# nv-nguyen/gigapose

Measured on AMD Instinct MI355X. Metric: query-crops/sec (ViT feat + template NN + 4DoF regress), 162 templates, 1/2/4/8 GPU, higher is better.
Workload: dtype f32 (ViT linear layers + attention, matcher, IST convolutions: f32 operands split into f16 hi/lo, 3 x f16 MFMA per k-block, f32 accumulate -- error vs f64 below the f32 fmaf chain's, tests/test_gpu_split.py; everything else f32); 1 GPU; BASELINE configs[1]: dinov2_vitl14 random-init, 1 object(s) x 162 templates, batch=64 crops per GPU, k=5, full path ViT->match->IST->RANSAC->pose; numerics=split, global_batch=64, parallelism=single, streams=single stream, rccl_ranks=0

## Files before the change

gigapose_amd/ae_net.py:

```python
import torch
from torch import nn

from .vit import Dinov2ViT, VARIANTS

descriptor_sizes = {"dinov2_vits14": 384, "dinov2_vitb14": 768, "dinov2_vitl14": 1024}


def as_hip_backbone(model, model_name=None):
    if isinstance(model, Dinov2ViT):
        return model
    if model is None:
        return Dinov2ViT.from_name(model_name)
    if hasattr(model, "config") and hasattr(model, "embeddings"):
        return Dinov2ViT.from_hf(model)
    sd = model.state_dict()
    if "blocks.0.attn.qkv.weight" in sd:
        dim = sd["cls_token"].shape[-1]
        depth = 1 + max(int(k.split(".")[1]) for k in sd if k.startswith("blocks."))
        vit = Dinov2ViT(dim, depth, dim // 64)
        vit.load_state_dict(sd, strict=False)
        return vit.eval()
    raise TypeError(f"cannot convert {type(model).__name__} into the HIP DINOv2 backbone")


class AENet(nn.Module):
    def __init__(self, model_name, dinov2_model, descriptor_size, max_batch_size, patch_size=14, **kwargs):
        super().__init__()
        if patch_size != 14:
            raise NotImplementedError("kernels are specialised for patch_size 14 @ 224x224")
        self.model_name = model_name
        self.dinov2_model = as_hip_backbone(dinov2_model, model_name)
        self.descriptor_size = descriptor_size
        self.max_batch_size = max_batch_size
        self.patch_size = patch_size
        assert self.dinov2_model.dim == descriptor_size

    def compute_features(self, images):
        return self.dinov2_model.forward_features(images)

    @torch.no_grad()
    def forward_by_chunk(self, processed_rgbs, patch_dim=(2, 3)):
        outs = [self.dinov2_model.patch_features(processed_rgbs[s:s + self.max_batch_size], normalize=True)
                for s in range(0, processed_rgbs.shape[0], self.max_batch_size)]
        if not outs:
            return torch.empty(0, self.descriptor_size, 16, 16, device=processed_rgbs.device)
        return outs[0] if len(outs) == 1 else torch.cat(outs, dim=0)

    def forward(self, images):
        return self.forward_by_chunk(images)
```

gigapose_amd/csrc/gp_gemm.hip:

```cpp
#include "gp_common.h"

namespace {

enum {
    EPI_NONE = 0,
    EPI_BIAS_I = 1,
    EPI_BIAS_I_GELU = 2,
    EPI_BIAS_I_SCALE_RES = 3,
    EPI_BIAS_J = 4,
    EPI_BIAS_I_RELU = 5,
};

using GM = KMajor<2, 4, 2, 1, 16>;

__device__ __forceinline__ float gelu_erf(float x)
{
    return 0.5f * x * (1.0f + erff(x * 0.70710678118654752440f));
}

constexpr int kMaxSlots = 1024;
constexpr size_t kSkHeaderBytes = 8192;
constexpr size_t kSkPartialFloats = (size_t)GM::BM * GM::BN;
constexpr int kSpinLimit = 400000;

struct GemmArgs {
    const float* A; int lda;
    const float* B; int ldb;
    float* D; int ldd;
    int K;
    const float* bias; const float* scale;
    const float* res ; int ldr;
    int tiles_i, tiles_j;
    int group;
    int* flags;
    float* partial;
    int epoch;
    int* status;
};

__device__ __forceinline__ void tile_origin(const GemmArgs& a, int q, int& i0, int& j0)
{
    const int per_band = a.group * a.tiles_j;
    const int band = q / per_band, r = q - band * per_band;
    const int first_i = band * a.group;
    const int gsz = min(a.group, a.tiles_i - first_i);
    i0 = (first_i + r % gsz) * GM::BM;
    j0 = (r / gsz) * GM::BN;
}

template <int EPI>
__device__ __forceinline__ void gemm_epilogue(const GemmArgs& a, int i0, int j0, const f32x16 (&acc)[2][1])
{
    int tid_ = threadIdx.x;
    asm volatile("" : "+v"(tid_));
    const int lane = tid_ & 63, wave = tid_ >> 6;
    const int wm = wave / GM::WN_, wn = wave % GM::WN_;
    const float* __restrict__ bias = a.bias;
    const float* __restrict__ scale = a.scale;
    const float* res = a.res;
    float* D = a.D;
    const int j = j0 + wn * 32 + (lane & 31);
#pragma unroll
    for (int mi = 0; mi < 2; ++mi) {
#pragma unroll
        for (int r = 0; r < 16; ++r) {
            const int i = i0 + wm * 64 + mi * 32 + frag_row(r, lane);
            float v = acc[mi][0][r];
            if (EPI == EPI_BIAS_I || EPI == EPI_BIAS_I_GELU || EPI == EPI_BIAS_I_SCALE_RES || EPI == EPI_BIAS_I_RELU)
                v = v + bias[i];
            if (EPI == EPI_BIAS_J) v = v + bias[j];
            if (EPI == EPI_BIAS_I_GELU) v = gelu_erf(v);
            if (EPI == EPI_BIAS_I_RELU) v = fmaxf(v, 0.f);
            if (EPI == EPI_BIAS_I_SCALE_RES) v = res[(unsigned)i * (unsigned)a.ldr + (unsigned)j] + scale[i] * v;
            D[(unsigned)i * (unsigned)a.ldd + (unsigned)j] = v;
        }
        if (EPI == EPI_BIAS_I_SCALE_RES) __builtin_amdgcn_sched_barrier(0);
    }
}

template <int EPI>
__global__ __launch_bounds__(GM::NT, 8) void gemm_kmajor_kernel(const GemmArgs a)
{
    __shared__ float smem[GM::LDS_FLOATS];
    const int q = xcd_chunked_tile(blockIdx.x, a.tiles_i * a.tiles_j);
    if (q < 0) return;
    int i0, j0;
    tile_origin(a, q, i0, j0);
    f32x16 acc[2][1];
    GM::run(a.A + i0, a.lda, a.B + j0, a.ldb, a.K, smem, acc);
    gemm_epilogue<EPI>(a, i0, j0, acc);
}

template <int EPI>
__global__ __launch_bounds__(GM::NT, 8) void gemm_streamk_kernel(const GemmArgs a)
{
    __shared__ float smem[GM::LDS_FLOATS];
    const int tid = threadIdx.x;
    const int p = blockIdx.x, x = p & 7, n = p >> 3, slots_x = gridDim.x >> 3;
    const int T = a.tiles_i * a.tiles_j;
    const int per = (T + 7) >> 3;
    const int t_lo = x * per;
    const int n_t = min(T - t_lo, per);
    const int nslab = a.K / GM::KS_;
    const long long U = (long long)n_t * nslab;
    const long long u0 = U * n / slots_x, u1 = U * (n + 1) / slots_x;
    const int ta = (int)(u0 / nslab), sa = (int)(u0 % nslab);
    const int tb = (int)(u1 / nslab), sb = (int)(u1 % nslab);
    const int n_head = sb > 0 ? 1 : 0, n_rest = sa > 0 ? 1 : 0;
    const int first_whole = ta + n_rest;
    const int n_seg = n_head + (tb - first_whole) + n_rest;
    for (int seg = 0; seg < n_seg; ++seg) {
        const bool is_head = seg < n_head;
        const bool is_rest = n_rest && seg == n_seg - 1;
        const int t = is_head ? tb : (is_rest ? ta : first_whole + seg - n_head);
        const int k0 = is_rest ? sa * GM::KS_ : 0;
        const int k1 = is_head ? sb * GM::KS_ : a.K;
        int i0, j0;
        tile_origin(a, t_lo + t, i0, j0);
        f32x16 acc[2][1];
        if (is_rest) {
            if (tid == 0) {
                int spins = 0;
                while (__hip_atomic_load(a.flags + (p - 8), __ATOMIC_RELAXED, __HIP_MEMORY_SCOPE_AGENT) != a.epoch) {
                    __builtin_amdgcn_s_sleep(16);
                    if (++spins > kSpinLimit) {
                        __hip_atomic_store(a.flags + kMaxSlots, 1, __ATOMIC_RELAXED, __HIP_MEMORY_SCOPE_AGENT);
                        gp_raise(a.status, GP_ST_HANDOFF_CHAIN);
                        break;
                    }
                }
                __builtin_amdgcn_fence(__ATOMIC_ACQUIRE, "agent");
            }
            __syncthreads();
            const f32x4* w = reinterpret_cast<const f32x4*>(a.partial + (size_t)(p - 8) * kSkPartialFloats) + tid * 8;
#pragma unroll
            for (int mi = 0; mi < 2; ++mi)
#pragma unroll
                for (int r4 = 0; r4 < 4; ++r4) {
                    const f32x4 v = w[mi * 4 + r4];
                    acc[mi][0][r4 * 4 + 0] = v[0]; acc[mi][0][r4 * 4 + 1] = v[1];
                    acc[mi][0][r4 * 4 + 2] = v[2]; acc[mi][0][r4 * 4 + 3] = v[3];
                }
        } else {
#pragma unroll
            for (int mi = 0; mi < 2; ++mi)
#pragma unroll
                for (int r = 0; r < 16; ++r) acc[mi][0][r] = 0.f;
        }
        GM::run_acc(a.A + (size_t)k0 * a.lda + i0, a.lda, a.B + (size_t)k0 * a.ldb + j0, a.ldb, k1 - k0, smem, acc);
        if (is_head) {
            f32x4* w = reinterpret_cast<f32x4*>(a.partial + (size_t)p * kSkPartialFloats) + tid * 8;
#pragma unroll
            for (int mi = 0; mi < 2; ++mi)
#pragma unroll
                for (int r4 = 0; r4 < 4; ++r4) {
                    f32x4 v;
                    v[0] = acc[mi][0][r4 * 4 + 0]; v[1] = acc[mi][0][r4 * 4 + 1];
                    v[2] = acc[mi][0][r4 * 4 + 2]; v[3] = acc[mi][0][r4 * 4 + 3];
                    w[mi * 4 + r4] = v;
                }
            asm volatile("s_waitcnt vmcnt(0)" ::: "memory");
            __syncthreads();
            if (tid == 0) {
                __builtin_amdgcn_fence(__ATOMIC_RELEASE, "agent");
                asm volatile("s_waitcnt vmcnt(0)" ::: "memory");
                __hip_atomic_store(a.flags + p, a.epoch, __ATOMIC_RELAXED, __HIP_MEMORY_SCOPE_AGENT);
            }
        } else {
            gemm_epilogue<EPI>(a, i0, j0, acc);
        }
    }
}

static int g_streamk = 1;
static int g_group = 8;
static unsigned g_epoch = 0;

template <int EPI>
int launch(const float* A, int lda, const float* B, int ldb, float* D, int ldd, int I, int J, int K,
           const float* bias, const float* scale, const float* res, int ldr, float* sk_ws, hipStream_t st)
{
    GemmArgs a{A, lda, B, ldb, D, ldd, K, bias, scale, res, ldr, I / GM::BM, J / GM::BN, g_group, nullptr, nullptr, 0, gp_status_buffer()};
    const int T = a.tiles_i * a.tiles_j;
    if (g_streamk && sk_ws && T > kMaxSlots && (T < 4 * kMaxSlots || g_streamk == 2) && T % kMaxSlots != 0) {
        const int per = (T + 7) / 8, last = T - 7 * per;
        const int slots_x = last < kMaxSlots / 8 ? last : kMaxSlots / 8;
        if (slots_x > 0) {
            a.flags = reinterpret_cast<int*>(sk_ws);
            a.partial = reinterpret_cast<float*>(reinterpret_cast<char*>(sk_ws) + kSkHeaderBytes);
            if (++g_epoch == 0) ++g_epoch;
            a.epoch = (int)g_epoch;
            hipLaunchKernelGGL((gemm_streamk_kernel<EPI>), dim3(8 * slots_x), dim3(GM::NT), 0, st, a);
            return 0;
        }
    }
    hipLaunchKernelGGL((gemm_kmajor_kernel<EPI>), dim3(xcd_chunked_grid(T)), dim3(GM::NT), 0, st, a);
    return 0;
}

}

int gp_gemm_launch(const float* A, int lda, const float* B, int ldb, float* D, int ldd, int I, int J,
                   int K, int epilogue, const float* bias, const float* scale, const float* res, int ldr,
                   float* sk_ws, hipStream_t st)
{
    GP_REQUIRE(I > 0 && J > 0 && K > 0, "gp_gemm_kmajor: empty problem (I=%d J=%d K=%d)", I, J, K);
    GP_REQUIRE(I % 128 == 0 && J % 128 == 0 && K % 16 == 0,
               "gp_gemm_kmajor: I=%d, J=%d must be multiples of 128 and K=%d of 16 (pad the operands)", I, J, K);
    GP_REQUIRE(lda % 4 == 0 && ldb % 4 == 0 && lda >= I && ldb >= J && ldd >= J,
               "gp_gemm_kmajor: bad leading dimensions lda=%d ldb=%d ldd=%d", lda, ldb, ldd);
    GP_REQUIRE((long long)I * ldd < (1ll << 31) && (long long)I * (ldr > 0 ? ldr : 1) < (1ll << 31),
               "gp_gemm_kmajor: output larger than 2^31 elements");
    GP_REQUIRE(A && B && D, "gp_gemm_kmajor: null pointer");
    GP_REQUIRE(((uintptr_t)A % 16 == 0) && ((uintptr_t)B % 16 == 0), "gp_gemm_kmajor: operands must be 16-byte aligned");
    GP_REQUIRE(((uintptr_t)sk_ws % 16 == 0), "gp_gemm_kmajor: stream-K scratch must be 16-byte aligned");
    GpProfScope prof(GP_PROF_GEMM, 2.0 * I * J * K, st);
    switch (epilogue) {
        case EPI_NONE: launch<EPI_NONE>(A, lda, B, ldb, D, ldd, I, J, K, bias, scale, res, ldr, sk_ws, st); break;
        case EPI_BIAS_I:
            GP_REQUIRE(bias, "gp_gemm_kmajor: bias required");
            launch<EPI_BIAS_I>(A, lda, B, ldb, D, ldd, I, J, K, bias, scale, res, ldr, sk_ws, st);
            break;
        case EPI_BIAS_I_GELU:
            GP_REQUIRE(bias, "gp_gemm_kmajor: bias required");
            launch<EPI_BIAS_I_GELU>(A, lda, B, ldb, D, ldd, I, J, K, bias, scale, res, ldr, sk_ws, st);
            break;
        case EPI_BIAS_I_SCALE_RES:
            GP_REQUIRE(bias && scale && res && ldr >= J, "gp_gemm_kmajor: bias/scale/residual required");
            launch<EPI_BIAS_I_SCALE_RES>(A, lda, B, ldb, D, ldd, I, J, K, bias, scale, res, ldr, sk_ws, st);
            break;
        case EPI_BIAS_J:
            GP_REQUIRE(bias, "gp_gemm_kmajor: bias required");
            launch<EPI_BIAS_J>(A, lda, B, ldb, D, ldd, I, J, K, bias, scale, res, ldr, sk_ws, st);
            break;
        case EPI_BIAS_I_RELU:
            GP_REQUIRE(bias, "gp_gemm_kmajor: bias required");
            launch<EPI_BIAS_I_RELU>(A, lda, B, ldb, D, ldd, I, J, K, bias, scale, res, ldr, sk_ws, st);
            break;
        default: GP_REQUIRE(false, "gp_gemm_kmajor: unknown epilogue %d", epilogue);
    }
    GP_CHECK_LAUNCH("gp_gemm_kmajor");
    return GP_OK;
}

size_t gp_gemm_streamk_bytes() { return kSkHeaderBytes + sizeof(float) * kSkPartialFloats * kMaxSlots; }

int gp_gemm_streamk_reset_launch(float* sk_ws, hipStream_t st)
{
    return hipMemsetAsync(sk_ws, 0, kSkHeaderBytes, st) == hipSuccess ? GP_OK : GP_ELAUNCH;
}

extern "C" int gp_gemm_kmajor(const float* A, int lda, const float* B, int ldb, float* D, int ldd, int I,
                              int J, int K, int epilogue, const float* bias, const float* scale,
                              const float* residual, int ldr, void* stream)
{
    return gp_gemm_launch(A, lda, B, ldb, D, ldd, I, J, K, epilogue, bias, scale, residual, ldr, nullptr,
                          (hipStream_t)stream);
}

extern "C" size_t gp_gemm_streamk_workspace_bytes(void) { return gp_gemm_streamk_bytes(); }

extern "C" int gp_gemm_streamk_reset(float* scratch, void* stream)
{
    GP_REQUIRE(scratch, "gp_gemm_streamk_reset: null scratch");
    return gp_gemm_streamk_reset_launch(scratch, (hipStream_t)stream);
}

#ifdef GP_PROBES
extern "C" void gp_gemm_set_streamk(int mode) { g_streamk = mode; }
extern "C" void gp_gemm_set_group(int g) { g_group = g > 0 ? g : 1; }

extern "C" int gp_gemm_streamk_error(const float* scratch, void* stream)
{
    int e = -1;
    if (hipMemcpyAsync(&e, reinterpret_cast<const int*>(scratch) + 1024, sizeof(int), hipMemcpyDeviceToHost,
                       (hipStream_t)stream) != hipSuccess ||
        hipStreamSynchronize((hipStream_t)stream) != hipSuccess)
        return -1;
    return e;
}
#endif

extern "C" int gp_gemm_kmajor_sk(const float* A, int lda, const float* B, int ldb, float* D, int ldd, int I,
                                 int J, int K, int epilogue, const float* bias, const float* scale,
                                 const float* residual, int ldr, float* scratch, size_t scratch_bytes, void* stream)
{
    GP_REQUIRE(scratch && scratch_bytes >= gp_gemm_streamk_bytes(), "gp_gemm_kmajor_sk: scratch too small");
    return gp_gemm_launch(A, lda, B, ldb, D, ldd, I, J, K, epilogue, bias, scale, residual, ldr, scratch,
                          (hipStream_t)stream);
}
```

gigapose_amd/csrc/gp_match.hip:

```cpp
#include "gp_common.h"

namespace {

__global__ __launch_bounds__(256) void l2norm_cp_kernel(const float* __restrict__ x,
                                                         float* __restrict__ out, int C)
{
    const size_t base = (size_t)blockIdx.x * C * GP_P + threadIdx.x;
    float ss = 0.f;
    for (int c = 0; c < C; ++c) {
        const float v = x[base + (size_t)c * GP_P];
        ss = __builtin_fmaf(v, v, ss);
    }
    const float d = fmaxf(__builtin_sqrtf(ss), 1e-12f);
    const int c0 = blockIdx.y * 32;
    for (int c = c0; c < c0 + 32 && c < C; ++c) out[base + (size_t)c * GP_P] = x[base + (size_t)c * GP_P] / d;
}

using MM = KMajor<4, 2, 2, 4, 16>;
static_assert(MM::BM == 256 && MM::BN == 256 && MM::NT == 512, "matcher tile must be 256x256");

struct alignas(16) MatchSmem {
    float stage[MM::LDS_FLOATS];
    float qmask[GP_P];
    float smask[GP_P];
    float rowv[2][GP_P];
    int rowi[2][GP_P];
    float colv[4][GP_P];
    int coli[4][GP_P];
    float sc_t2s[GP_P];
    int id_t2s[GP_P];
    float sc_s2t[GP_P];
    int id_s2t[GP_P];
    float contrib[GP_P];
    float maskv[GP_P];
};

template <int CNT>
__device__ __forceinline__ void rowmax_exchange(float (&rv)[32], int (&ri)[32], int lane)
{
    const bool hi = (lane & CNT) != 0;
#pragma unroll
    for (int j = 0; j < CNT; ++j) {
        const float sv = hi ? rv[j] : rv[j + CNT];
        const int si = hi ? ri[j] : ri[j + CNT];
        const float mv = hi ? rv[j + CNT] : rv[j];
        const int mj = hi ? ri[j + CNT] : ri[j];
        const float ov = __shfl_xor(sv, CNT);
        const int oi = __shfl_xor(si, CNT);
        const bool take = (ov > mv) | ((ov == mv) & (oi < mj));
        rv[j] = take ? ov : mv;
        ri[j] = take ? oi : mj;
    }
}

constexpr int kDeadPatch = 0x7fff;
#include "gp_match_rects.h"
struct MatchWaveTile {
    int r0, mi_n, c0, ni_n, rslot, cslot, active;
};
__device__ __forceinline__ MatchWaveTile match_wave_tile_grid(int wave)
{
    return MatchWaveTile{2 * (wave >> 1), 2, 4 * (wave & 1), 4, wave & 1, wave >> 1, 1};
}
__device__ __forceinline__ MatchWaveTile match_wave_tile_unpack(unsigned w)
{
    return MatchWaveTile{(int)(w & 15u), (int)((w >> 4) & 3u), (int)((w >> 6) & 15u), (int)((w >> 10) & 7u), (int)((w >> 13) & 3u), (int)((w >> 15) & 3u),
                         (int)((w >> 17) & 1u)};
}
template <bool PERM = false, class SM>
__device__ __forceinline__ void match_epilogue(SM& sm, f32x16 (&acc)[2][4], int b, int n, int N, float thr, float patch_thr,
                                               uint8_t* __restrict__ idx_t2s, float* __restrict__ score_t2s,
                                               float* __restrict__ mask_all, float* __restrict__ sim_avg,
                                               unsigned long long* trace = nullptr,
                                               int src2tar = 0,
                                               int compact = 1,
                                               MatchWaveTile wt = MatchWaveTile{0, 0, 0, 0, 0, 0, 0})
{
    const int tid = threadIdx.x, lane = tid & 63, wave = __builtin_amdgcn_readfirstlane(tid >> 6);
    if constexpr (!PERM) wt = match_wave_tile_grid(wave);
    const int s_lane = 32 * wt.c0 + (lane & 31);
    const int t_lane = 32 * wt.r0 + 4 * (lane >> 5);
    float sm_s[4];
    int s_idx[4];
#pragma unroll
    for (int ni = 0; ni < 4; ++ni) {
        sm_s[ni] = 0.f;
        s_idx[ni] = kDeadPatch;
        if (!PERM || ni < wt.ni_n) {
            if constexpr (PERM) {
                sm_s[ni] = sm.smask_p[s_lane + 32 * ni];
                s_idx[ni] = sm.s_of[s_lane + 32 * ni];
            } else {
                sm_s[ni] = sm.smask[s_lane + 32 * ni];
                s_idx[ni] = s_lane + 32 * ni;
            }
        }
    }
#pragma unroll
    for (int mi = 0; mi < 2; ++mi) {
        if (PERM && mi >= wt.mi_n) continue;
#pragma unroll
        for (int r = 0; r < 16; ++r) {
            float tm;
            if constexpr (PERM) tm = sm.qmask_p[t_lane + 32 * mi + (r & 3) + 8 * (r >> 2)];
            else tm = sm.qmask[t_lane + 32 * mi + (r & 3) + 8 * (r >> 2)];
#pragma unroll
            for (int ni = 0; ni < 4; ++ni) {
                float v = acc[mi][ni][r] * sm_s[ni];
                v = v * tm;
                acc[mi][ni][r] = (v < thr) ? 0.f : v;
            }
        }
    }

    float rv[32];
    int ri[32];
#pragma unroll
    for (int mi = 0; mi < 2; ++mi)
#pragma unroll
        for (int r = 0; r < 16; ++r) {
            float bv = acc[mi][0][r];
            int bi = s_idx[0];
#pragma unroll
            for (int ni = 1; ni < 4; ++ni) {
                const float x = acc[mi][ni][r];
                const bool take = PERM ? ((x > bv) | ((x == bv) & (s_idx[ni] < bi))) : (x > bv);
                bv = take ? x : bv;
                bi = take ? s_idx[ni] : bi;
            }
            rv[mi * 16 + r] = bv;
            ri[mi * 16 + r] = bi;
        }
    rowmax_exchange<16>(rv, ri, lane);
    rowmax_exchange<8>(rv, ri, lane);
    rowmax_exchange<4>(rv, ri, lane);
    rowmax_exchange<2>(rv, ri, lane);
    rowmax_exchange<1>(rv, ri, lane);
    {
        const int j = lane & 31;
        int t = t_lane + 32 * (j >> 4) + (j & 3) + 8 * ((j & 15) >> 2);
        const bool mine = !PERM || (wt.active && (j >> 4) < wt.mi_n);
        if constexpr (PERM) t = mine ? sm.t_of[t] : kDeadPatch;
        if (mine && (!PERM || t != kDeadPatch)) {
            sm.rowv[wt.rslot][t] = rv[0];
            sm.rowi[wt.rslot][t] = ri[0];
        }
    }

    int tp[32];
    if constexpr (PERM) {
#pragma unroll
        for (int mi = 0; mi < 2; ++mi)
#pragma unroll
            for (int r4 = 0; r4 < 4; ++r4) {
                typedef short s16x4 __attribute__((ext_vector_type(4)));
                const s16x4 q4 = *reinterpret_cast<const s16x4*>(&sm.t_of[t_lane + 32 * mi + 8 * r4]);
#pragma unroll
                for (int e = 0; e < 4; ++e) tp[mi * 16 + 4 * r4 + e] = (int)q4[e];
            }
    }
#pragma unroll
    for (int ni = 0; ni < 4; ++ni) {
        if (PERM && (ni >= wt.ni_n || !wt.active)) continue;
        float bv = acc[0][ni][0];
        int bi = PERM ? tp[0] : t_lane;
#pragma unroll
        for (int mi = 0; mi < 2; ++mi) {
            if (PERM && mi >= wt.mi_n) continue;
#pragma unroll
            for (int r = 0; r < 16; ++r) {
                const float x = acc[mi][ni][r];
                if constexpr (PERM) {
                    const int tq = tp[mi * 16 + r];
                    const bool take = (x > bv) | ((x == bv) & ((x > 0.f) | (compact == 0)) & (tq < bi));
                    bv = take ? x : bv;
                    bi = take ? tq : bi;
                } else {
                    const int row = t_lane + 32 * mi + (r & 3) + 8 * (r >> 2);
                    if (x > bv) { bv = x; bi = row; }
                }
            }
        }
        const float ov = __shfl_xor(bv, 32);
        const int oi = __shfl_xor(bi, 32);
        if (ov > bv || (ov == bv && oi < bi)) { bv = ov; bi = oi; }
        if (lane < 32 && (!PERM || s_idx[ni] != kDeadPatch)) {
            sm.colv[wt.cslot][s_idx[ni]] = bv;
            sm.coli[wt.cslot][s_idx[ni]] = bi;
        }
    }
    __syncthreads();
    if (trace && tid == 0) trace[3] = wall_clock64();

    if (tid < GP_P) {
        float bv = sm.rowv[0][tid];
        int bi = sm.rowi[0][tid];
#pragma unroll
        for (int w = 1; w < ((PERM && compact) ? 4 : 2); ++w) {
            const float v1 = sm.rowv[w][tid];
            const int i1 = sm.rowi[w][tid];
            if (v1 > bv || (PERM && v1 == bv && i1 < bi)) { bv = v1; bi = i1; }
        }
        if (PERM && compact && bv == 0.f) bi = 0;
        sm.sc_t2s[tid] = bv;
        sm.id_t2s[tid] = bi;
    } else {
        const int s = tid - GP_P;
        float bv = sm.colv[0][s];
        int bi = sm.coli[0][s];
#pragma unroll
        for (int w = 1; w < 4; ++w) {
            const float vw = sm.colv[w][s];
            const int iw = sm.coli[w][s];
            if (vw > bv || (PERM && vw == bv && iw < bi)) { bv = vw; bi = iw; }
        }
        if (PERM && compact && bv == 0.f) bi = 0;
        sm.sc_s2t[s] = bv;
        sm.id_s2t[s] = bi;
    }
    __syncthreads();
    if (trace && tid == 0) trace[4] = wall_clock64();

    if (tid < GP_P) {
        const int t = tid;
        const float* sc_a = src2tar ? sm.sc_s2t : sm.sc_t2s;
        const int* id_a = src2tar ? sm.id_s2t : sm.id_t2s;
        const float* sc_b = src2tar ? sm.sc_t2s : sm.sc_s2t;
        const int* id_b = src2tar ? sm.id_t2s : sm.id_s2t;
        const int js = id_a[t];
        const float sc = sc_a[t];
        const bool mask_sim = sc >= thr;
        bool mask_cycle = true;
        if (patch_thr > 0.f) {
            const int t2 = id_b[js];
            const float dx = (float)(t2 % GP_G) - (float)(t % GP_G);
            const float dy = (float)(t2 / GP_G) - (float)(t / GP_G);
            const float dist = __builtin_sqrtf(dx * dx + dy * dy);
            const bool mask_dist = dist <= patch_thr;
            const bool mask_sim2 = sc_b[js] >= thr;
            mask_cycle = mask_dist && mask_sim2;
        }
        float nz = sm.qmask[t] * sm.smask[js];
        nz = nz * (float)(id_b[t] != 0);
        nz = nz * (float)(js != 0);
        const float m = (float)(mask_sim && mask_cycle) * nz;
        const size_t o = ((size_t)b * N + n) * GP_P + t;
        idx_t2s[o] = (uint8_t)js;
        score_t2s[o] = sc;
        mask_all[o] = m;
        sm.contrib[t] = sc * m;
        sm.maskv[t] = m;
    }
    __syncthreads();
    if (trace && tid == 0) trace[5] = wall_clock64();
    if (tid == 0) {
        float a = 0.f, cnt = 0.f;
#pragma unroll 1
        for (int t0 = 0; t0 < GP_P; t0 += 32) {
            f32x4 c[8], m[8];
#pragma unroll
            for (int u = 0; u < 8; ++u) {
                c[u] = *reinterpret_cast<const f32x4*>(&sm.contrib[t0 + 4 * u]);
                m[u] = *reinterpret_cast<const f32x4*>(&sm.maskv[t0 + 4 * u]);
            }
#pragma unroll
            for (int u = 0; u < 8; ++u)
#pragma unroll
                for (int e = 0; e < 4; ++e) {
                    a = a + c[u][e];
                    cnt = cnt + m[u][e];
                }
        }
        sim_avg[(size_t)b * N + n] = (cnt > 0.f) ? a / 256.0f : 0.f;
        if (trace) trace[6] = wall_clock64();
    }
}

__global__ __launch_bounds__(512, 2) void match_tiles_kernel(
    const float* __restrict__ query,
    const float* __restrict__ bank,
    const float* __restrict__ qmask,
    const float* __restrict__ bmask,
    const int* __restrict__ labels,
    int B, int O, int N, int C, float thr, float patch_thr, int* __restrict__ status,
    uint8_t* __restrict__ idx_t2s,
    float* __restrict__ score_t2s,
    float* __restrict__ mask_all,
    float* __restrict__ sim_avg,
    int src2tar)
{
    __shared__ MatchSmem sm;
    const int q = xcd_chunked_tile(blockIdx.x, B * N);
    if (q < 0) return;
    const int band = q / (8 * N), r8 = q - band * (8 * N);
    const int gsz = min(8, B - band * 8);
    const int b = band * 8 + r8 % gsz, n = r8 / gsz;
    const int tid = threadIdx.x;
    int lab = labels[b];
    if ((unsigned)lab >= (unsigned)O) {
        if (tid == 0) gp_raise(status, GP_ST_LABEL_RANGE);
        lab = 0;
    }
    const size_t on = (size_t)lab * N + n;
    const float* A = query + (size_t)b * C * GP_P;
    const float* Bm = bank + on * (size_t)C * GP_P;

    if (tid < GP_P) sm.qmask[tid] = qmask[(size_t)b * GP_P + tid];
    else sm.smask[tid - GP_P] = bmask[on * GP_P + (tid - GP_P)];

    f32x16 acc[2][4];
    MM::run(A, GP_P, Bm, GP_P, C, sm.stage, acc);

    match_epilogue(sm, acc, b, n, N, thr, patch_thr, idx_t2s, score_t2s, mask_all, sim_avg, nullptr, src2tar);
}

typedef _Float16 h16x8 __attribute__((ext_vector_type(8)));
constexpr float kFeatScale = 32.0f;
constexpr int MS_BK = 32, MS_PLANE = 256 * MS_BK;

struct alignas(16) MatchSplitSmem {
    _Float16 stage[2 * 4 * MS_PLANE];
    float qmask[GP_P];
    float smask[GP_P];
    float qmask_p[GP_P];
    float smask_p[GP_P];
    short t_of[GP_P];
    short s_of[GP_P];
    int cnt[8];
    float rowv[4][GP_P];
    int rowi[4][GP_P];
    float colv[4][GP_P];
    int coli[4][GP_P];
    float sc_t2s[GP_P];
    int id_t2s[GP_P];
    float sc_s2t[GP_P];
    int id_s2t[GP_P];
    float contrib[GP_P];
    float maskv[GP_P];
};

typedef unsigned int mu32x4 __attribute__((ext_vector_type(4)));
constexpr unsigned kMatchOob = 0x80000000u;

struct MatchSplitRsrc {
    __amdgpu_buffer_rsrc_t qh, ql, bh, bl;
    unsigned va0, va1, vb0, vb1;
};

template <bool BANK_LO, int MI, int NI>
__device__ __forceinline__ void match_split_kloop(MatchSplitSmem& sm, f32x16 (&acc)[2][4], const MatchSplitRsrc& rs, int ns, int tid,
                                                  int lane, int r0, int c0, int grp)
{
    constexpr int P_AHI = 0, P_ALO = MS_PLANE, P_BHI = 2 * MS_PLANE, P_BLO = 3 * MS_PLANE, MS_BUF = 4 * MS_PLANE;
    const int wofs = (tid >> 2) * MS_BK + (((tid & 3) ^ (((tid >> 2) >> 2) & 3)) << 3);
    mu32x4 rg[8];
    auto gload = [&](int slab) {
        const unsigned so = (unsigned)slab * (MS_BK * 2u);
        rg[0] = __builtin_amdgcn_raw_buffer_load_b128(rs.qh, rs.va0, so, 0);
        rg[2] = __builtin_amdgcn_raw_buffer_load_b128(rs.ql, rs.va0, so, 0);
        rg[1] = __builtin_amdgcn_raw_buffer_load_b128(rs.qh, rs.va1, so, 0);
        rg[3] = __builtin_amdgcn_raw_buffer_load_b128(rs.ql, rs.va1, so, 0);
        rg[4] = __builtin_amdgcn_raw_buffer_load_b128(rs.bh, rs.vb0, so, 0);
        rg[5] = __builtin_amdgcn_raw_buffer_load_b128(rs.bh, rs.vb1, so, 0);
        if (BANK_LO) {
            rg[6] = __builtin_amdgcn_raw_buffer_load_b128(rs.bl, rs.vb0, so, 0);
            rg[7] = __builtin_amdgcn_raw_buffer_load_b128(rs.bl, rs.vb1, so, 0);
        }
    };
    auto stage = [&](int buf) {
        _Float16* L = sm.stage + buf * MS_BUF + wofs;
        *reinterpret_cast<mu32x4*>(L + P_AHI) = rg[0];
        *reinterpret_cast<mu32x4*>(L + P_ALO) = rg[2];
        *reinterpret_cast<mu32x4*>(L + P_AHI + 128 * MS_BK) = rg[1];
        *reinterpret_cast<mu32x4*>(L + P_ALO + 128 * MS_BK) = rg[3];
        *reinterpret_cast<mu32x4*>(L + P_BHI) = rg[4];
        *reinterpret_cast<mu32x4*>(L + P_BHI + 128 * MS_BK) = rg[5];
        if (BANK_LO) {
            *reinterpret_cast<mu32x4*>(L + P_BLO) = rg[6];
            *reinterpret_cast<mu32x4*>(L + P_BLO + 128 * MS_BK) = rg[7];
        }
    };
    const int ar_ = 32 * r0 + (lane & 31), br_ = 32 * c0 + (lane & 31), kh_ = lane >> 5;
    const int arow = ar_ * MS_BK, brow = br_ * MS_BK;
    const int ak0 = ((kh_ ^ ((ar_ >> 2) & 3)) << 3), ak1 = (((kh_ + 2) ^ ((ar_ >> 2) & 3)) << 3);
    const int bk0 = ((kh_ ^ ((br_ >> 2) & 3)) << 3), bk1 = (((kh_ + 2) ^ ((br_ >> 2) & 3)) << 3);
    gload(0);
    stage(0);
    __builtin_amdgcn_sched_barrier(0);
    if (ns > 1) gload(1);
    __syncthreads();

#define M_MFMA(A_, B_, mi, ni) acc[mi][ni] = __builtin_amdgcn_mfma_f32_32x32x16_f16(A_[mi], B_[ni], acc[mi][ni], 0, 0, 0)
#define M_ALL(A_, B_)                                       \
    _Pragma("unroll") for (int ni = 0; ni < NI; ++ni)       \
        _Pragma("unroll") for (int mi = 0; mi < MI; ++mi) M_MFMA(A_, B_, mi, ni)
    auto c_phase = [&](int s) __attribute__((always_inline)) {
        const _Float16* L = sm.stage + (s & 1) * MS_BUF;
        __builtin_amdgcn_s_setprio(1);
        h16x8 ah[MI], al[MI], bh[NI], bl[NI], ch[MI], cl[MI], dh[NI], dl[NI];
#pragma unroll
        for (int mi = 0; mi < MI; ++mi) ah[mi] = *reinterpret_cast<const h16x8*>(L + P_AHI + arow + mi * 32 * MS_BK + ak0);
#pragma unroll
        for (int ni = 0; ni < NI; ++ni) bh[ni] = *reinterpret_cast<const h16x8*>(L + P_BHI + brow + ni * 32 * MS_BK + bk0);
        if (BANK_LO) {
#pragma unroll
            for (int ni = 0; ni < NI; ++ni) bl[ni] = *reinterpret_cast<const h16x8*>(L + P_BLO + brow + ni * 32 * MS_BK + bk0);
        }
#pragma unroll
        for (int mi = 0; mi < MI; ++mi) al[mi] = *reinterpret_cast<const h16x8*>(L + P_ALO + arow + mi * 32 * MS_BK + ak0);
        M_ALL(ah, bh);
        if (BANK_LO) { M_ALL(ah, bl); }
#pragma unroll
        for (int mi = 0; mi < MI; ++mi) ch[mi] = *reinterpret_cast<const h16x8*>(L + P_AHI + arow + mi * 32 * MS_BK + ak1);
#pragma unroll
        for (int ni = 0; ni < NI; ++ni) dh[ni] = *reinterpret_cast<const h16x8*>(L + P_BHI + brow + ni * 32 * MS_BK + bk1);
        M_ALL(al, bh);
        if (BANK_LO) {
#pragma unroll
            for (int ni = 0; ni < NI; ++ni) dl[ni] = *reinterpret_cast<const h16x8*>(L + P_BLO + brow + ni * 32 * MS_BK + bk1);
        }
#pragma unroll
        for (int mi = 0; mi < MI; ++mi) cl[mi] = *reinterpret_cast<const h16x8*>(L + P_ALO + arow + mi * 32 * MS_BK + ak1);
        M_ALL(ch, dh);
        if (BANK_LO) { M_ALL(ch, dl); }
        M_ALL(cl, dh);
        __builtin_amdgcn_s_setprio(0);
    };
    auto m_phase = [&](int slab) __attribute__((always_inline)) {
        if (slab < ns) stage(slab & 1);
        __builtin_amdgcn_sched_barrier(0);
        gload(min(slab + 1, ns - 1));
    };
    if (grp) m_phase(1);
    for (int s = 0; s < ns; ++s) {
        c_phase(s);
        if (grp && s + 1 < ns) __syncthreads();
        m_phase(s + 1 + grp);
        if (!grp && s + 1 < ns) __syncthreads();
    }
#undef M_ALL
#undef M_MFMA
}

#ifndef GP_MATCH_BAND
#define GP_MATCH_BAND 8
#endif
constexpr int kSplitBand = GP_MATCH_BAND;
template <bool BANK_LO, bool TRACE = false>
__global__ __launch_bounds__(512, 2) void match_tiles_split_kernel(
    const _Float16* __restrict__ q_hi, const _Float16* __restrict__ q_lo,
    const _Float16* __restrict__ b_hi, const _Float16* __restrict__ b_lo,
    const float* __restrict__ qmask, const float* __restrict__ bmask, const int* __restrict__ labels, int B, int O, int N, int C,
    float thr, float patch_thr, int* __restrict__ status, uint8_t* __restrict__ idx_t2s, float* __restrict__ score_t2s,
    float* __restrict__ mask_all, float* __restrict__ sim_avg, unsigned long long* __restrict__ trace_all, int compact, int src2tar)
{
    __shared__ MatchSplitSmem sm;
    const unsigned long long w_in = TRACE ? wall_clock64() : 0;
    const int q = xcd_chunked_tile(blockIdx.x, B * N);
    if (q < 0) return;
    unsigned long long* trace = TRACE ? trace_all + (size_t)q * 8 : nullptr;
    if (TRACE && threadIdx.x == 0) {
        unsigned hw;
        asm volatile("s_getreg_b32 %0, hwreg(HW_REG_HW_ID)" : "=s"(hw));
        unsigned xcc;
        asm volatile("s_getreg_b32 %0, hwreg(HW_REG_XCC_ID)" : "=s"(xcc));
        trace[0] = w_in;
        trace[7] = ((unsigned long long)(xcc & 0xf) << 32) | hw;
    }
    const int band = q / (kSplitBand * N), r8 = q - band * (kSplitBand * N);
    const int gsz = min(kSplitBand, B - band * kSplitBand);
    const int b = band * kSplitBand + r8 % gsz, n = r8 / gsz;
    const int tid = threadIdx.x, lane = tid & 63;
    const int wave = __builtin_amdgcn_readfirstlane(tid >> 6);
    const int grp = wave >> 2;
    int lab = labels[b];
    if ((unsigned)lab >= (unsigned)O) {
        if (tid == 0) gp_raise(status, GP_ST_LABEL_RANGE);
        lab = 0;
    }
    const size_t on = (size_t)lab * N + n;

    const int pidx = tid & 255;
    const float mv = tid < GP_P ? qmask[(size_t)b * GP_P + pidx] : bmask[on * GP_P + pidx];
    const bool live = compact ? (mv != 0.f) : true;
    const unsigned long long bal = __ballot(live);
    const int before = __popcll(bal & ((1ull << lane) - 1ull));
    if (lane == 0) sm.cnt[wave] = __popcll(bal);
    if (tid < GP_P) {
        sm.qmask[pidx] = mv;
        sm.qmask_p[pidx] = 0.f;
        sm.t_of[pidx] = (short)kDeadPatch;
#pragma unroll
        for (int w = 0; w < 4; ++w) { sm.rowv[w][pidx] = 0.f; sm.rowi[w][pidx] = 0; }
    } else {
        sm.smask[pidx] = mv;
        sm.smask_p[pidx] = 0.f;
        sm.s_of[pidx] = (short)kDeadPatch;
#pragma unroll
        for (int w = 0; w < 4; ++w) { sm.colv[w][pidx] = 0.f; sm.coli[w][pidx] = 0; }
    }
    __syncthreads();
    int rank = before;
    for (int w = 4 * grp; w < wave; ++w) rank += sm.cnt[w];
    if (live) {
        if (tid < GP_P) {
            sm.t_of[rank] = (short)pidx;
            sm.qmask_p[rank] = mv;
        } else {
            sm.s_of[rank] = (short)pidx;
            sm.smask_p[rank] = mv;
        }
    }
    __syncthreads();
    const int live_t = sm.cnt[0] + sm.cnt[1] + sm.cnt[2] + sm.cnt[3], live_s = sm.cnt[4] + sm.cnt[5] + sm.cnt[6] + sm.cnt[7];
    const int nrb = __builtin_amdgcn_readfirstlane((live_t + 31) >> 5), ncb = __builtin_amdgcn_readfirstlane((live_s + 31) >> 5);
    const MatchWaveTile wt = match_wave_tile_unpack((unsigned)__builtin_amdgcn_readfirstlane((int)kMatchRect[nrb][ncb][wave]));

    const unsigned plane_bytes = (unsigned)GP_P * (unsigned)C * 2u;
    MatchSplitRsrc rs;
    rs.qh = __builtin_amdgcn_make_buffer_rsrc((void*)(q_hi + (size_t)b * GP_P * C), 0, plane_bytes, 0x00020000);
    rs.ql = __builtin_amdgcn_make_buffer_rsrc((void*)(q_lo + (size_t)b * GP_P * C), 0, plane_bytes, 0x00020000);
    rs.bh = __builtin_amdgcn_make_buffer_rsrc((void*)(b_hi + on * GP_P * C), 0, plane_bytes, 0x00020000);
    rs.bl = __builtin_amdgcn_make_buffer_rsrc((void*)((BANK_LO ? b_lo : b_hi) + on * GP_P * C), 0, plane_bytes, 0x00020000);
    {
        const int r0 = tid >> 2, r1 = r0 + 128;
        const unsigned ck = (unsigned)(tid & 3) * 16u, rowb = (unsigned)C * 2u;
        const int t0 = sm.t_of[r0], t1 = sm.t_of[r1], s0 = sm.s_of[r0], s1 = sm.s_of[r1];
        rs.va0 = t0 != kDeadPatch ? (unsigned)t0 * rowb + ck : kMatchOob;
        rs.va1 = t1 != kDeadPatch ? (unsigned)t1 * rowb + ck : kMatchOob;
        rs.vb0 = s0 != kDeadPatch ? (unsigned)s0 * rowb + ck : kMatchOob;
        rs.vb1 = s1 != kDeadPatch ? (unsigned)s1 * rowb + ck : kMatchOob;
    }

    f32x16 acc[2][4];
#pragma unroll
    for (int mi = 0; mi < 2; ++mi)
#pragma unroll
        for (int ni = 0; ni < 4; ++ni)
#pragma unroll
            for (int r = 0; r < 16; ++r) acc[mi][ni][r] = 0.f;
    const int ns = C / MS_BK;
    if (TRACE && tid == 0) trace[1] = wall_clock64();
    if (nrb > 0 && ncb > 0) {
        const int sel = wt.mi_n * 8 + wt.ni_n;
#define M_CASE(MI_, NI_) case MI_ * 8 + NI_: match_split_kloop<BANK_LO, MI_, NI_>(sm, acc, rs, ns, tid, lane, wt.r0, wt.c0, grp); break
        switch (sel) {
            M_CASE(1, 1); M_CASE(1, 2); M_CASE(1, 3); M_CASE(1, 4);
            M_CASE(2, 1); M_CASE(2, 2); M_CASE(2, 3);
            default: match_split_kloop<BANK_LO, 2, 4>(sm, acc, rs, ns, tid, lane, wt.r0, wt.c0, grp); break;
        }
#undef M_CASE
    }
    __syncthreads();
    if (TRACE && tid == 0) trace[2] = wall_clock64();

    constexpr float inv = 1.0f / (kFeatScale * kFeatScale);
#pragma unroll
    for (int mi = 0; mi < 2; ++mi)
#pragma unroll
        for (int ni = 0; ni < 4; ++ni)
#pragma unroll
            for (int r = 0; r < 16; ++r) acc[mi][ni][r] *= inv;
    match_epilogue<true>(sm, acc, b, n, N, thr, patch_thr, idx_t2s, score_t2s, mask_all, sim_avg, trace, src2tar, compact, wt);
}

__global__ __launch_bounds__(256) void l2norm_split_kernel(const float* __restrict__ x, _Float16* __restrict__ hi,
                                                            _Float16* __restrict__ lo, int C, int Cp,
                                                            const float* __restrict__ mask_img = nullptr, int mh = 0, int mw = 0,
                                                            float* __restrict__ patch_mask = nullptr)
{
    __shared__ float t[32][GP_P + 1];
    __shared__ float dn[GP_P];
    const int row = blockIdx.x, p = threadIdx.x;
    if (patch_mask && blockIdx.y == 0)
        patch_mask[(size_t)row * GP_P + p] = mask_img[(size_t)row * mh * mw + (size_t)((p >> 4) * (mh / GP_G)) * mw + (p & 15) * (mw / GP_G)];
    const float* xr = x + (size_t)row * C * GP_P;
    float ss = 0.f;
    int c = 0;
    for (; c + 16 <= C; c += 16) {
        float v[16];
#pragma unroll
        for (int u = 0; u < 16; ++u) v[u] = xr[(size_t)(c + u) * GP_P + p];
#pragma unroll
        for (int u = 0; u < 16; ++u) ss = __builtin_fmaf(v[u], v[u], ss);
    }
    for (; c < C; ++c) {
        const float v = xr[(size_t)c * GP_P + p];
        ss = __builtin_fmaf(v, v, ss);
    }
    dn[p] = fmaxf(__builtin_sqrtf(ss), 1e-12f);
    const int ngrp = Cp / 32, g0 = ngrp * blockIdx.y / gridDim.y, g1 = ngrp * (blockIdx.y + 1) / gridDim.y;
    for (int grp = g0; grp < g1; ++grp) {
        const int c0 = grp * 32;
        __syncthreads();
        for (int r = 0; r < 32; ++r) t[r][p] = (c0 + r < C) ? xr[(size_t)(c0 + r) * GP_P + p] : 0.f;
        __syncthreads();
#pragma unroll
        for (int u = 0; u < 4; ++u) {
            const int item = p + 256 * u, pp = item >> 2, g = item & 3;
            h16x8 h, l;
#pragma unroll
            for (int e = 0; e < 8; ++e) {
                const float v = (t[g * 8 + e][pp] / dn[pp]) * kFeatScale;
                const _Float16 hh = (_Float16)v;
                h[e] = hh;
                l[e] = (_Float16)(v - (float)hh);
            }
            const size_t o = ((size_t)row * GP_P + pp) * Cp + c0 + g * 8;
            *reinterpret_cast<h16x8*>(hi + o) = h;
            *reinterpret_cast<h16x8*>(lo + o) = l;
        }
    }
}

__global__ __launch_bounds__(64) void topk_kernel(const float* __restrict__ sim_avg, int N, int k,
                                                   int* __restrict__ ids, float* __restrict__ scores)
{
    extern __shared__ unsigned char taken[];
    const int b = blockIdx.x, lane = threadIdx.x;
    for (int n = lane; n < N; n += 64) taken[n] = 0;
    __syncthreads();
    const float* v = sim_avg + (size_t)b * N;
    for (int j = 0; j < k; ++j) {
        float bv = 0.f;
        int bi = 0x7fffffff;
        for (int n = lane; n < N; n += 64) {
            if (taken[n]) continue;
            const float x = v[n];
            if (bi == 0x7fffffff || x > bv) { bv = x; bi = n; }
        }
#pragma unroll
        for (int off = 32; off >= 1; off >>= 1) {
            const float ov = __shfl_xor(bv, off);
            const int oi = __shfl_xor(bi, off);
            if (oi != 0x7fffffff && (bi == 0x7fffffff || ov > bv || (ov == bv && oi < bi))) { bv = ov; bi = oi; }
        }
        if (lane == 0) {
            ids[(size_t)b * k + j] = bi;
            scores[(size_t)b * k + j] = bv;
            taken[bi] = 1;
        }
        __syncthreads();
    }
}

__global__ __launch_bounds__(256) void gather_records_kernel(
    const int* __restrict__ ids, const uint8_t* __restrict__ idx_t2s,
    const float* __restrict__ score_t2s, const float* __restrict__ mask_all, int N, int k,
    uint8_t* __restrict__ rec_idx, float* __restrict__ rec_score, float* __restrict__ rec_mask)
{
    const int bk = blockIdx.x, b = bk / k, t = threadIdx.x;
    const size_t src = ((size_t)b * N + ids[bk]) * GP_P + t;
    const size_t dst = (size_t)bk * GP_P + t;
    rec_idx[dst] = idx_t2s[src];
    rec_score[dst] = score_t2s[src];
    rec_mask[dst] = mask_all[src];
}

__global__ __launch_bounds__(256) void format_points_kernel(const uint8_t* __restrict__ rec_idx,
                                                             const float* __restrict__ rec_mask,
                                                             long long* __restrict__ tar_pts,
                                                             long long* __restrict__ src_pts)
{
    const size_t i = (size_t)blockIdx.x * GP_P + threadIdx.x;
    const int t = threadIdx.x;
    const bool valid = rec_mask[i] != 0.f;
    const int js = rec_idx[i];
    tar_pts[2 * i + 0] = valid ? (t % GP_G) : -1;
    tar_pts[2 * i + 1] = valid ? (t / GP_G) : -1;
    src_pts[2 * i + 0] = valid ? (js % GP_G) : -1;
    src_pts[2 * i + 1] = valid ? (js / GP_G) : -1;
}

__global__ __launch_bounds__(256) void select_topk_kernel(const float* __restrict__ sim_avg, const uint8_t* __restrict__ idx_t2s,
                                                           const float* __restrict__ score_t2s, const float* __restrict__ mask_all, int N, int k,
                                                           long long* __restrict__ ids64, float* __restrict__ scores,
                                                           float* __restrict__ rec_score, long long* __restrict__ tar_pts,
                                                           long long* __restrict__ src_pts)
{
    extern __shared__ unsigned char taken[];
    int* win = reinterpret_cast<int*>(taken + ((N + 3) & ~3));
    const int b = blockIdx.x, t = threadIdx.x, lane = t & 63;
    for (int n = t; n < N; n += 256) taken[n] = 0;
    __syncthreads();
    const float* v = sim_avg + (size_t)b * N;
    if (t < 64) {
        for (int j = 0; j < k; ++j) {
            float bv = 0.f;
            int bi = 0x7fffffff;
            for (int n = lane; n < N; n += 64) {
                if (taken[n]) continue;
                const float x = v[n];
                if (bi == 0x7fffffff || x > bv) { bv = x; bi = n; }
            }
#pragma unroll
            for (int off = 32; off >= 1; off >>= 1) {
                const float ov = __shfl_xor(bv, off);
                const int oi = __shfl_xor(bi, off);
                if (oi != 0x7fffffff && (bi == 0x7fffffff || ov > bv || (ov == bv && oi < bi))) { bv = ov; bi = oi; }
            }
            if (lane == 0) {
                ids64[(size_t)b * k + j] = bi;
                scores[(size_t)b * k + j] = bv;
                taken[bi] = 1;
                win[j] = bi;
            }
            __builtin_amdgcn_wave_barrier();
            __builtin_amdgcn_fence(__ATOMIC_ACQ_REL, "workgroup");
        }
    }
    __syncthreads();
    for (int j = 0; j < k; ++j) {
        const size_t src = ((size_t)b * N + win[j]) * GP_P + t;
        const size_t i = ((size_t)b * k + j) * GP_P + t;
        const bool valid = mask_all[src] != 0.f;
        const int js = idx_t2s[src];
        rec_score[i] = score_t2s[src];
        tar_pts[2 * i + 0] = valid ? (t % GP_G) : -1;
        tar_pts[2 * i + 1] = valid ? (t / GP_G) : -1;
        src_pts[2 * i + 0] = valid ? (js % GP_G) : -1;
        src_pts[2 * i + 1] = valid ? (js / GP_G) : -1;
    }
}

}

extern "C" {

int gp_l2norm_cp(const float* x, float* out, int rows, int C, void* stream)
{
    GP_REQUIRE(rows >= 0 && C > 0, "gp_l2norm_cp: bad arguments (rows=%d C=%d)", rows, C);
    if (rows == 0) return GP_OK;
    GP_REQUIRE(x && out, "gp_l2norm_cp: null pointer");
    hipLaunchKernelGGL(l2norm_cp_kernel, dim3(rows, (C + 31) / 32), dim3(256), 0, (hipStream_t)stream, x, out, C);
    GP_CHECK_LAUNCH("gp_l2norm_cp");
    return GP_OK;
}

int gp_match_tiles_dir(const float* query, const float* bank, const float* qmask, const float* bmask,
                       const int* labels, int B, int O, int N, int C, float sim_threshold,
                       float patch_threshold, int search_direction, uint8_t* idx_t2s, float* score_t2s, float* mask_all,
                       float* sim_avg, void* stream)
{
    GP_REQUIRE(search_direction == 0 || search_direction == 1, "gp_match_tiles: search_direction must be 0 (tar2src) or 1 (src2tar)");
    GP_REQUIRE(B >= 0 && O > 0 && N > 0, "gp_match_tiles: bad sizes B=%d O=%d N=%d", B, O, N);
    GP_REQUIRE(C > 0 && C % 16 == 0, "gp_match_tiles: C=%d must be a positive multiple of 16", C);
    if (B == 0) return GP_OK;
    GP_REQUIRE(query && bank && qmask && bmask && labels && idx_t2s && score_t2s && mask_all && sim_avg,
               "gp_match_tiles: null pointer");
    GpProfScope prof(GP_PROF_MATCH, 2.0 * B * N * 256.0 * 256.0 * C, (hipStream_t)stream);
    hipLaunchKernelGGL(match_tiles_kernel, dim3(xcd_chunked_grid(B * N)), dim3(512), 0,
                       (hipStream_t)stream, query, bank, qmask, bmask, labels, B, O, N, C, sim_threshold,
                       patch_threshold, gp_status_buffer(), idx_t2s, score_t2s, mask_all, sim_avg, search_direction);
    GP_CHECK_LAUNCH("gp_match_tiles");
    return GP_OK;
}

int gp_l2norm_split_mask(const float* x, void* hi, void* lo, int rows, int C, const float* mask_img, int mask_h, int mask_w,
                         float* patch_mask, void* stream)
{
    GP_REQUIRE(rows >= 0 && C > 0, "gp_l2norm_split: bad arguments (rows=%d C=%d)", rows, C);
    if (rows == 0) return GP_OK;
    GP_REQUIRE(x && hi && lo, "gp_l2norm_split: null pointer");
    GP_REQUIRE(!patch_mask || (mask_img && mask_h > 0 && mask_w > 0 && mask_h % GP_G == 0 && mask_w % GP_G == 0),
               "gp_l2norm_split_mask: the mask image must be (rows, H, W) f32 with H, W multiples of 16 (got %d x %d)", mask_h, mask_w);
    const int ngrp = (C + 31) / 32;
    hipLaunchKernelGGL(l2norm_split_kernel, dim3(rows, ngrp < 4 ? ngrp : 4), dim3(256), 0, (hipStream_t)stream, x, (_Float16*)hi,
                       (_Float16*)lo, C, ngrp * 32, mask_img, mask_h, mask_w, patch_mask);
    GP_CHECK_LAUNCH("gp_l2norm_split");
    return GP_OK;
}

static int g_match_compact = 1;

static int match_tiles_split_launch(const void* q_hi, const void* q_lo, const void* b_hi, const void* b_lo, const float* qmask,
                                    const float* bmask, const int* labels, int B, int O, int N, int C, float sim_threshold,
                                    float patch_threshold, uint8_t* idx_t2s, float* score_t2s, float* mask_all, float* sim_avg,
                                    unsigned long long* trace, void* stream, int search_direction = 0)
{
    GP_REQUIRE(search_direction == 0 || search_direction == 1, "gp_match_tiles_split: search_direction must be 0 (tar2src) or 1 (src2tar)");
    const int compact = (g_match_compact && sim_threshold >= 0.f) ? 1 : 0;
    GP_REQUIRE(B >= 0 && O > 0 && N > 0, "gp_match_tiles_split: bad sizes B=%d O=%d N=%d", B, O, N);
    GP_REQUIRE(C > 0 && C % 32 == 0, "gp_match_tiles_split: C=%d must be a positive multiple of 32", C);
    if (B == 0) return GP_OK;
    GP_REQUIRE(q_hi && q_lo && b_hi && qmask && bmask && labels && idx_t2s && score_t2s && mask_all && sim_avg,
               "gp_match_tiles_split: null pointer");
    GP_REQUIRE((long long)GP_P * C * 2 < (1ll << 31), "gp_match_tiles_split: C too large");
    GpProfScope prof(GP_PROF_MATCH_SPLIT, 2.0 * B * N * 256.0 * 256.0 * C, (hipStream_t)stream);
#define GP_MATCH_SPLIT_LAUNCH(LO, TR)                                                                                             \
    hipLaunchKernelGGL((match_tiles_split_kernel<LO, TR>), dim3(xcd_chunked_grid(B * N)), dim3(512), 0, (hipStream_t)stream,      \
                       (const _Float16*)q_hi, (const _Float16*)q_lo, (const _Float16*)b_hi, (const _Float16*)b_lo, qmask, bmask,  \
                       labels, B, O, N, C, sim_threshold, patch_threshold, gp_status_buffer(), idx_t2s, score_t2s, mask_all,      \
                       sim_avg, trace, compact, search_direction)
    if (trace) {
        GP_REQUIRE(b_lo, "gp_match_tiles_split_trace: the probe build takes the two-plane bank");
        GP_MATCH_SPLIT_LAUNCH(true, true);
    } else if (b_lo) {
        GP_MATCH_SPLIT_LAUNCH(true, false);
    } else {
        GP_MATCH_SPLIT_LAUNCH(false, false);
    }
#undef GP_MATCH_SPLIT_LAUNCH
    GP_CHECK_LAUNCH("gp_match_tiles_split");
    return GP_OK;
}

int gp_match_tiles_split_dir(const void* q_hi, const void* q_lo, const void* b_hi, const void* b_lo, const float* qmask,
                             const float* bmask, const int* labels, int B, int O, int N, int C, float sim_threshold,
                             float patch_threshold, int search_direction, uint8_t* idx_t2s, float* score_t2s, float* mask_all,
                             float* sim_avg, void* stream)
{
    return match_tiles_split_launch(q_hi, q_lo, b_hi, b_lo, qmask, bmask, labels, B, O, N, C, sim_threshold, patch_threshold,
                                    idx_t2s, score_t2s, mask_all, sim_avg, nullptr, stream, search_direction);
}

#ifdef GP_PROBES
int gp_match_tiles_split_trace(const void* q_hi, const void* q_lo, const void* b_hi, const void* b_lo, const float* qmask,
                               const float* bmask, const int* labels, int B, int O, int N, int C, float sim_threshold,
                               float patch_threshold, uint8_t* idx_t2s, float* score_t2s, float* mask_all, float* sim_avg,
                               unsigned long long* trace, void* stream)
{
    GP_REQUIRE(trace, "gp_match_tiles_split_trace: null trace buffer");
    return match_tiles_split_launch(q_hi, q_lo, b_hi, b_lo, qmask, bmask, labels, B, O, N, C, sim_threshold, patch_threshold,
                                    idx_t2s, score_t2s, mask_all, sim_avg, trace, stream);
}

int gp_match_split_set_compact(int on)
{
    g_match_compact = on ? 1 : 0;
    return GP_OK;
}
#endif

int gp_topk(const float* sim_avg, int B, int N, int k, int* ids, float* scores, void* stream)
{
    GP_REQUIRE(k >= 1 && k <= N, "gp_topk: selected index k out of range (k=%d, N=%d)", k, N);
    if (B == 0) return GP_OK;
    GP_REQUIRE(sim_avg && ids && scores, "gp_topk: null pointer");
    hipLaunchKernelGGL(topk_kernel, dim3(B), dim3(64), (size_t)N, (hipStream_t)stream, sim_avg, N, k, ids, scores);
    GP_CHECK_LAUNCH("gp_topk");
    return GP_OK;
}

int gp_select_topk(const float* sim_avg, const uint8_t* idx_t2s, const float* score_t2s, const float* mask_all, int B, int N, int k,
                   long long* ids, float* scores, float* rec_score, long long* tar_pts, long long* src_pts, void* stream)
{
    GP_REQUIRE(k >= 1 && k <= N, "gp_select_topk: selected index k out of range (k=%d, N=%d)", k, N);
    if (B == 0) return GP_OK;
    GP_REQUIRE(sim_avg && idx_t2s && score_t2s && mask_all && ids && scores && rec_score && tar_pts && src_pts, "gp_select_topk: null pointer");
    hipLaunchKernelGGL(select_topk_kernel, dim3(B), dim3(256), (size_t)((N + 3) & ~3) + sizeof(int) * (size_t)k, (hipStream_t)stream, sim_avg,
                       idx_t2s, score_t2s, mask_all, N, k, ids, scores, rec_score, tar_pts, src_pts);
    GP_CHECK_LAUNCH("gp_select_topk");
    return GP_OK;
}

int gp_gather_records(const int* ids, const uint8_t* idx_t2s, const float* score_t2s,
                      const float* mask_all, int B, int N, int k, uint8_t* rec_idx, float* rec_score,
                      float* rec_mask, void* stream)
{
    GP_REQUIRE(k >= 1 && N >= 1, "gp_gather_records: bad sizes");
    if (B == 0) return GP_OK;
    GP_REQUIRE(ids && idx_t2s && score_t2s && mask_all && rec_idx && rec_score && rec_mask,
               "gp_gather_records: null pointer");
    hipLaunchKernelGGL(gather_records_kernel, dim3(B * k), dim3(256), 0, (hipStream_t)stream, ids,
                       idx_t2s, score_t2s, mask_all, N, k, rec_idx, rec_score, rec_mask);
    GP_CHECK_LAUNCH("gp_gather_records");
    return GP_OK;
}

int gp_format_points(const uint8_t* rec_idx, const float* rec_mask, int rows, long long* tar_pts,
                     long long* src_pts, void* stream)
{
    if (rows <= 0) return GP_OK;
    GP_REQUIRE(rec_idx && rec_mask && tar_pts && src_pts, "gp_format_points: null pointer");
    hipLaunchKernelGGL(format_points_kernel, dim3(rows), dim3(256), 0, (hipStream_t)stream, rec_idx,
                       rec_mask, tar_pts, src_pts);
    GP_CHECK_LAUNCH("gp_format_points");
    return GP_OK;
}

}
```

gigapose_amd/csrc/gp_vit.hip:

```cpp
#include "gp_common.h"

int gp_gemm_launch(const float* A, int lda, const float* B, int ldb, float* D, int ldd, int I, int J,
                   int K, int epilogue, const float* bias, const float* scale, const float* res, int ldr,
                   float* sk_ws, hipStream_t st);
int gp_gemm_split_launch(const float* act, int ld_act, const void* whi, const void* wlo, float* D, int ldd, int I, int J,
                         int K, int act_is_b, int epilogue, const float* bias, const float* scale, const float* res, int ldr,
                         hipStream_t st);
bool gp_gemm_split256_usable(int I, int J, int K);
int gp_gemm_split256_launch(const float* act, int ld_act, const void* whi, const void* wlo, float* D, int ldd, int I, int J,
                            int K, int act_is_b, int epilogue, const float* bias, const float* scale, const float* res, int ldr,
                            float* scratch, hipStream_t st);
size_t gp_gemm_streamk_bytes();
int gp_gemm_streamk_reset_launch(float* sk_ws, hipStream_t st);
bool gp_gemm_split256_usable(int I, int J, int K);
bool gp_gemm_planes256_usable(int I, int J, int J_valid, int K);
int gp_gemm_planes256_launch(const void* ahi, const void* alo, const void* bhi, const void* blo, float* D, int ldd, void* ohi,
                             void* olo, int ldo, int I, int J, int J_valid, int K, int epilogue, const float* bias, const float* scale,
                             const float* res, int ldr, float out_scale, float* scratch, hipStream_t st, unsigned long long* trace = nullptr,
                             const GpPlaneOut* po = nullptr);

namespace {

constexpr int PATCH = 14, IMG = 224, KPE = 588, KPE_PAD = 592, T_TOK = 257;

__global__ __launch_bounds__(256) void im2col_kernel(const float* __restrict__ img, float* __restrict__ col, int B)
{
    const int k = blockIdx.x, b = blockIdx.y, p = threadIdx.x;
    float v = 0.f;
    if (k < KPE) {
        const int ci = k / 196, dy = (k % 196) / PATCH, dx = k % PATCH;
        const int py = p >> 4, px = p & 15;
        v = img[(((size_t)b * 3 + ci) * IMG + (py * PATCH + dy)) * IMG + px * PATCH + dx];
    }
    col[(size_t)k * (B * GP_P) + (size_t)b * GP_P + p] = v;
}

__global__ __launch_bounds__(320) void embed_kernel(const float* __restrict__ pe ,
                                                     const float* __restrict__ cls_pos ,
                                                     const float* __restrict__ pos_t ,
                                                     float* __restrict__ X, int B, int Mpad)
{
    const int c = blockIdx.x, b = blockIdx.y, t = threadIdx.x;
    if (b == B) {
        for (int m = B * T_TOK + t; m < Mpad; m += 320) X[(size_t)c * Mpad + m] = 0.f;
        return;
    }
    if (t >= T_TOK) return;
    float v;
    if (t == 0) v = cls_pos[c];
    else v = pe[(size_t)c * (B * GP_P) + (size_t)b * GP_P + (t - 1)] + pos_t[(size_t)c * GP_P + (t - 1)];
    X[(size_t)c * Mpad + (size_t)b * T_TOK + t] = v;
}

__global__ __launch_bounds__(1024) void layernorm_wide_kernel(const float* __restrict__ X, float* __restrict__ Y,
                                                               const float* __restrict__ gamma,
                                                               const float* __restrict__ beta, int C, int Mpad,
                                                               float eps)
{
    __shared__ float red[16][64];
    const int tok = threadIdx.x & 63, sl = threadIdx.x >> 6;
    const int per = C >> 4, c0 = sl * per;
    const float* x = X + (size_t)c0 * Mpad + (size_t)blockIdx.x * 64 + tok;
    float* y = Y + (size_t)c0 * Mpad + (size_t)blockIdx.x * 64 + tok;
    float s = 0.f;
#pragma unroll 8
    for (int i = 0; i < per; ++i) s += x[(size_t)i * Mpad];
    red[sl][tok] = s;
    __syncthreads();
    float tot = 0.f;
#pragma unroll
    for (int j = 0; j < 16; ++j) tot += red[j][tok];
    const float mean = tot / (float)C;
    __syncthreads();
    float q = 0.f;
#pragma unroll 8
    for (int i = 0; i < per; ++i) {
        const float d = x[(size_t)i * Mpad] - mean;
        q = __builtin_fmaf(d, d, q);
    }
    red[sl][tok] = q;
    __syncthreads();
    tot = 0.f;
#pragma unroll
    for (int j = 0; j < 16; ++j) tot += red[j][tok];
    const float rstd = 1.0f / __builtin_sqrtf(tot / (float)C + eps);
#pragma unroll 8
    for (int i = 0; i < per; ++i)
        y[(size_t)i * Mpad] = (x[(size_t)i * Mpad] - mean) * rstd * gamma[c0 + i] + beta[c0 + i];
}

int launch_layernorm(const float* X, float* Y, const float* g, const float* b, int C, int Mpad, float eps,
                     hipStream_t st)
{
    GpProfScope prof(GP_PROF_LN, 8.0 * C * Mpad, st);
    hipLaunchKernelGGL(layernorm_wide_kernel, dim3(Mpad / 64), dim3(1024), 0, st, X, Y, g, b, C, Mpad, eps);
    return 0;
}


typedef _Float16 v16x8 __attribute__((ext_vector_type(8)));
typedef _Float16 v16x4 __attribute__((ext_vector_type(4)));
typedef unsigned int au32x4 __attribute__((ext_vector_type(4)));
typedef float f32x2 __attribute__((ext_vector_type(2)));
constexpr float kPlaneScale = 8.0f;

__global__ __launch_bounds__(1024) void layernorm_planes_kernel(const float* __restrict__ X, _Float16* __restrict__ Yhi,
                                                                 _Float16* __restrict__ Ylo, const float* __restrict__ gamma,
                                                                 const float* __restrict__ beta, int C, int Mpad, float eps,
                                                                 int* __restrict__ status, float plane_scale, float* __restrict__ amax)
{
    __shared__ float red[16][64];
    const int tok = threadIdx.x & 63, sl = threadIdx.x >> 6;
    const int per = C >> 4, c0 = sl * per;
    const float* x = X + (size_t)c0 * Mpad + (size_t)blockIdx.x * 64 + tok;
    int bad = 0;
    float vmax = 0.f;
    float s = 0.f;
#pragma unroll 8
    for (int i = 0; i < per; ++i) s += x[(size_t)i * Mpad];
    red[sl][tok] = s;
    __syncthreads();
    float tot = 0.f;
#pragma unroll
    for (int j = 0; j < 16; ++j) tot += red[j][tok];
    const float mean = tot / (float)C;
    __syncthreads();
    float q = 0.f;
#pragma unroll 8
    for (int i = 0; i < per; ++i) {
        const float d = x[(size_t)i * Mpad] - mean;
        q = __builtin_fmaf(d, d, q);
    }
    red[sl][tok] = q;
    __syncthreads();
    tot = 0.f;
#pragma unroll
    for (int j = 0; j < 16; ++j) tot += red[j][tok];
    const float rstd = 1.0f / __builtin_sqrtf(tot / (float)C + eps);
    __shared__ unsigned int tile[2][128 * 65];
    const float* xb = X + (size_t)blockIdx.x * 64 + tok;
    const int t2 = 8 * (sl & 7) + (tok & 7), g2 = 8 * (sl >> 3) + (tok >> 3);
    const size_t row = ((size_t)blockIdx.x * 64 + t2) * C + 8 * g2;
    const int nchunk = C >> 7;
    for (int k = 0; k < nchunk; ++k) {
        unsigned int* T = tile[k & 1];
#pragma unroll
        for (int e = 0; e < 8; ++e) {
            const int cl = 8 * sl + e, c = 128 * k + cl;
            const float y = (xb[(size_t)c * Mpad] - mean) * rstd * gamma[c] + beta[c];
            const float v = y * plane_scale;
            const _Float16 hh = (_Float16)v;
            const _Float16 ll = (_Float16)(v - (float)hh);
            bad |= !(fabsf(v) <= kSplitPlaneLimit);
            vmax = __builtin_elementwise_maximum(vmax, __builtin_fabsf(v));
            T[cl * 65 + tok] = (unsigned int)__builtin_bit_cast(unsigned short, hh) |
                               ((unsigned int)__builtin_bit_cast(unsigned short, ll) << 16);
        }
        __syncthreads();
        v16x8 h, l;
#pragma unroll
        for (int e = 0; e < 8; ++e) {
            const unsigned int w = T[(8 * g2 + e) * 65 + t2];
            h[e] = __builtin_bit_cast(_Float16, (unsigned short)(w & 0xffffu));
            l[e] = __builtin_bit_cast(_Float16, (unsigned short)(w >> 16));
        }
        *reinterpret_cast<v16x8*>(Yhi + row + 128 * k) = h;
        *reinterpret_cast<v16x8*>(Ylo + row + 128 * k) = l;
    }
    if (bad) gp_raise(status, GP_ST_SPLIT_RANGE);
    if (amax) gp_record_amax(amax, vmax, 1.0f / plane_scale);
}

template <int NK, int TOK = 32>
__global__ __launch_bounds__(512) void layernorm_planes_reg_kernel(const float* __restrict__ X, _Float16* __restrict__ Yhi,
                                                                    _Float16* __restrict__ Ylo, const float* __restrict__ gamma,
                                                                    const float* __restrict__ beta, int Mpad, float eps,
                                                                    int* __restrict__ status, float plane_scale, float* __restrict__ amax)
{
    constexpr int C = 128 * NK, SL = 512 / TOK, CH = 8 * SL, NC = C / CH;
    constexpr int TP = CH + 4;
    static_assert(C % CH == 0 && (TOK == 32 || TOK == 16), "layernorm_planes_reg_kernel: C must be a multiple of the chunk width");
    __shared__ float red[SL][TOK];
    __shared__ __attribute__((aligned(16))) unsigned int tile[2][TOK * TP];
    __shared__ __attribute__((aligned(16))) float gb[2][C];
    const int tok = threadIdx.x & (TOK - 1), sl = threadIdx.x / TOK;
    const size_t tok0 = (size_t)blockIdx.x * TOK;
    float xv[NC][8];
    float s = 0.f;
#pragma unroll
    for (int k = 0; k < NC; ++k)
#pragma unroll
        for (int e = 0; e < 8; ++e) {
            xv[k][e] = X[(size_t)(CH * k + 8 * sl + e) * Mpad + tok0 + tok];
            s += xv[k][e];
        }
    for (int c = threadIdx.x; c < C; c += 512) {
        gb[0][c] = gamma[c];
        gb[1][c] = beta[c];
    }
    red[sl][tok] = s;
    __syncthreads();
    float tot = 0.f;
#pragma unroll
    for (int j = 0; j < SL; ++j) tot += red[j][tok];
    const float mean = tot / (float)C;
    __syncthreads();
    float q = 0.f;
#pragma unroll
    for (int k = 0; k < NC; ++k)
#pragma unroll
        for (int e = 0; e < 8; ++e) {
            const float d = xv[k][e] - mean;
            q = __builtin_fmaf(d, d, q);
        }
    red[sl][tok] = q;
    __syncthreads();
    tot = 0.f;
#pragma unroll
    for (int j = 0; j < SL; ++j) tot += red[j][tok];
    const float rstd = 1.0f / __builtin_sqrtf(tot / (float)C + eps);
    const int g2 = threadIdx.x & (SL - 1), t2 = threadIdx.x / SL;
    const size_t row = (tok0 + t2) * C + 8 * g2;
    int bad = 0;
    float vmax = 0.f;
#pragma unroll
    for (int k = 0; k < NC; ++k) {
        unsigned int* T = tile[k & 1];
        const int c = CH * k + 8 * sl;
        const f32x4 g0 = *reinterpret_cast<const f32x4*>(gb[0] + c), g1 = *reinterpret_cast<const f32x4*>(gb[0] + c + 4);
        const f32x4 b0 = *reinterpret_cast<const f32x4*>(gb[1] + c), b1 = *reinterpret_cast<const f32x4*>(gb[1] + c + 4);
        unsigned int w[8];
#pragma unroll
        for (int e = 0; e < 8; ++e) {
            const float y = (xv[k][e] - mean) * rstd * (e < 4 ? g0[e] : g1[e - 4]) + (e < 4 ? b0[e] : b1[e - 4]);
            const float v = y * plane_scale;
            const _Float16 hh = (_Float16)v;
            const _Float16 ll = (_Float16)(v - (float)hh);
            bad |= !(fabsf(v) <= kSplitPlaneLimit);
            if (amax) vmax = __builtin_elementwise_maximum(vmax, __builtin_fabsf(v));
            w[e] = (unsigned int)__builtin_bit_cast(unsigned short, hh) | ((unsigned int)__builtin_bit_cast(unsigned short, ll) << 16);
        }
        typedef unsigned int u4 __attribute__((ext_vector_type(4)));
        u4 w0 = {w[0], w[1], w[2], w[3]}, w1 = {w[4], w[5], w[6], w[7]};
        *reinterpret_cast<u4*>(T + tok * TP + 8 * sl) = w0;
        *reinterpret_cast<u4*>(T + tok * TP + 8 * sl + 4) = w1;
        __syncthreads();
        const u4 r0 = *reinterpret_cast<const u4*>(T + t2 * TP + 8 * g2), r1 = *reinterpret_cast<const u4*>(T + t2 * TP + 8 * g2 + 4);
        v16x8 h, l;
#pragma unroll
        for (int e = 0; e < 4; ++e) {
            h[e] = __builtin_bit_cast(_Float16, (unsigned short)(r0[e] & 0xffffu));
            l[e] = __builtin_bit_cast(_Float16, (unsigned short)(r0[e] >> 16));
            h[4 + e] = __builtin_bit_cast(_Float16, (unsigned short)(r1[e] & 0xffffu));
            l[4 + e] = __builtin_bit_cast(_Float16, (unsigned short)(r1[e] >> 16));
        }
        *reinterpret_cast<v16x8*>(Yhi + row + CH * k) = h;
        *reinterpret_cast<v16x8*>(Ylo + row + CH * k) = l;
    }
    if (bad) gp_raise(status, GP_ST_SPLIT_RANGE);
    if (amax) gp_record_amax(amax, vmax, 1.0f / plane_scale);
}


static int g_ln_planes_reg = 1;
#ifdef GP_PROBES
extern "C" void gp_vit_set_ln_reg(int on) { g_ln_planes_reg = (on >= 0 && on <= 2) ? on : 1; }
#endif

int launch_layernorm_planes(const float* X, _Float16* hi, _Float16* lo, const float* g, const float* b, int C, int Mpad, float eps,
                            hipStream_t st, float plane_scale = kPlaneScale, float* amax = nullptr)
{
    GpProfScope prof(GP_PROF_LN, 8.0 * C * Mpad, st);
    if (g_ln_planes_reg && C == 1024 && Mpad % 32 == 0 && Mpad / 32 <= 128 && g_ln_planes_reg != 2)
        hipLaunchKernelGGL((layernorm_planes_reg_kernel<8, 16>), dim3(Mpad / 16), dim3(512), 0, st, X, hi, lo, g, b, Mpad, eps, gp_status_buffer(), plane_scale, amax);
    else if (g_ln_planes_reg && C == 1024 && Mpad % 32 == 0)
        hipLaunchKernelGGL(layernorm_planes_reg_kernel<8>, dim3(Mpad / 32), dim3(512), 0, st, X, hi, lo, g, b, Mpad, eps, gp_status_buffer(), plane_scale, amax);
    else if (g_ln_planes_reg && C == 768 && Mpad % 32 == 0)
        hipLaunchKernelGGL(layernorm_planes_reg_kernel<6>, dim3(Mpad / 32), dim3(512), 0, st, X, hi, lo, g, b, Mpad, eps, gp_status_buffer(), plane_scale, amax);
    else
        hipLaunchKernelGGL(layernorm_planes_kernel, dim3(Mpad / 64), dim3(1024), 0, st, X, hi, lo, g, b, C, Mpad, eps, gp_status_buffer(), plane_scale, amax);
    return 0;
}

constexpr int NKT = 9;

__device__ __forceinline__ void attention_body(const float* __restrict__ Qp, const float* __restrict__ Kp,
                                               const float* __restrict__ Vp, float* __restrict__ Op, int q0, int C,
                                               int Mpad, float scale)
{
    const int lane = threadIdx.x, half = lane >> 5, l31 = lane & 31;
    const int tq = q0 + l31;
    const int tq_c = tq < T_TOK ? tq : T_TOK - 1;
    f32x16 o0, o1;
#pragma unroll
    for (int r = 0; r < 16; ++r) { o0[r] = 0.f; o1[r] = 0.f; }
    float m_run = -INFINITY, l_part = 0.f;

#pragma unroll 1
    for (int ch = 0; ch < 3; ++ch) {
        f32x16 s[3];
        int tk_c[3];
#pragma unroll
        for (int t = 0; t < 3; ++t) {
#pragma unroll
            for (int r = 0; r < 16; ++r) s[t][r] = 0.f;
            const int tk = (ch * 3 + t) * 32 + l31;
            tk_c[t] = tk < T_TOK ? tk : T_TOK - 1;
        }
#pragma unroll 8
        for (int kk = 0; kk < 32; ++kk) {
            const size_t drow = (size_t)(2 * kk + half) * Mpad;
            const float qv = Qp[drow + tq_c];
#pragma unroll
            for (int t = 0; t < 3; ++t) {
                const float kv = Kp[drow + tk_c[t]];
                s[t] = __builtin_amdgcn_mfma_f32_32x32x2f32(kv, qv, s[t], 0, 0, 0);
            }
        }
        float cmax = -INFINITY;
#pragma unroll
        for (int t = 0; t < 3; ++t)
#pragma unroll
            for (int r = 0; r < 16; ++r) {
                const int tk = (ch * 3 + t) * 32 + frag_row(r, lane);
                const float v = (tk < T_TOK) ? s[t][r] * scale : -INFINITY;
                s[t][r] = v;
                cmax = fmaxf(cmax, v);
            }
        cmax = fmaxf(cmax, __shfl_xor(cmax, 32));
        const float m_new = fmaxf(m_run, cmax);
        const float alpha = expf(m_run - m_new);
        float psum = 0.f;
#pragma unroll
        for (int t = 0; t < 3; ++t)
#pragma unroll
            for (int r = 0; r < 16; ++r) {
                const float p = expf(s[t][r] - m_new);
                s[t][r] = p;
                psum += p;
            }
        l_part = l_part * alpha + psum;
#pragma unroll
        for (int r = 0; r < 16; ++r) { o0[r] *= alpha; o1[r] *= alpha; }
        m_run = m_new;
#pragma unroll
        for (int t = 0; t < 3; ++t)
#pragma unroll
            for (int r = 0; r < 16; ++r) {
                int tk = (ch * 3 + t) * 32 + frag_row(r, lane);
                tk = tk < T_TOK ? tk : T_TOK - 1;
                const float* vrow = Vp + (size_t)tk * C + l31;
                const float v0 = vrow[0], v1 = vrow[32];
                o0 = __builtin_amdgcn_mfma_f32_32x32x2f32(v0, s[t][r], o0, 0, 0, 0);
                o1 = __builtin_amdgcn_mfma_f32_32x32x2f32(v1, s[t][r], o1, 0, 0, 0);
            }
    }
    const float inv = 1.0f / (l_part + __shfl_xor(l_part, 32));
    if (tq < T_TOK) {
#pragma unroll
        for (int r = 0; r < 16; ++r) {
            const int d = frag_row(r, lane);
            Op[(size_t)d * Mpad + tq] = o0[r] * inv;
            Op[(size_t)(32 + d) * Mpad + tq] = o1[r] * inv;
        }
    }
}

__global__ __launch_bounds__(64, 4) void attention_kernel(const float* __restrict__ QK ,
                                                          const float* __restrict__ Vt ,
                                                          float* __restrict__ O , int B, int H, int C,
                                                          int Mpad, float scale)
{
    const int q = xcd_chunked_tile(blockIdx.x, B * H * NKT);
    if (q < 0) return;
    const int qb = q % NKT, bh = q / NKT, h = bh % H, b = bh / H;
    const float* Qp = QK + (size_t)(h * 64) * Mpad + (size_t)b * T_TOK;
    const float* Kp = QK + (size_t)(C + h * 64) * Mpad + (size_t)b * T_TOK;
    const float* Vp = Vt + (size_t)b * T_TOK * C + h * 64;
    float* Op = O + (size_t)(h * 64) * Mpad + (size_t)b * T_TOK;
    attention_body(Qp, Kp, Vp, Op, qb * 32, C, Mpad, scale);
}

int launch_attention_f32(const float* QK, const float* Vt, float* O, int B, int heads, int C, int Mpad, hipStream_t st)
{
    GpProfScope prof(GP_PROF_ATTN, 4.0 * B * heads * 257.0 * 257.0 * 64.0, st);
    hipLaunchKernelGGL(attention_kernel, dim3(xcd_chunked_grid(B * heads * NKT)), dim3(64), 0, st, QK, Vt, O, B, heads, C, Mpad, 0.125f);
    return 0;
}

constexpr int AKS = 72;
constexpr int AVS = 292;
constexpr int AKEYS = 288;

__device__ __forceinline__ float exp_neg(float x)
{
    x = fmaxf(x, -10000.0f);
    const float t = x * 1.4426950216293335f;
    float e = __builtin_fmaf(x, 1.4426950216293335f, -t);
    e = __builtin_fmaf(x, 1.925963033500011e-08f, e);
    const float r = __builtin_amdgcn_exp2f(t);
    return __builtin_fmaf(r, e * 0.6931471824645996f, r);
}

typedef const __attribute__((address_space(3))) v16x8* lds_v16x8p;
typedef const __attribute__((address_space(3))) v16x4* lds_v16x4p;
__device__ __forceinline__ unsigned lds_addr(const _Float16* p)
{
    return (unsigned)(size_t)(const __attribute__((address_space(3))) _Float16*)p;
}

constexpr int ATH = 512;

typedef _Float16 av16x2 __attribute__((ext_vector_type(2)));
__device__ __forceinline__ unsigned attn_hi_pair(float v0, float v1)
{
    av16x2 h;
    h[0] = (_Float16)v0;
    h[1] = (_Float16)v1;
    return __builtin_bit_cast(unsigned, h);
}
__device__ __forceinline__ unsigned attn_lo_pair(float v0, float v1, unsigned hi)
{
    unsigned lo;
    asm("v_fma_mixlo_f16 %0, %1, 1.0, -%3 op_sel:[0,0,0] op_sel_hi:[0,0,1]\n\t"
        "v_fma_mixhi_f16 %0, %2, 1.0, -%3 op_sel:[0,0,1] op_sel_hi:[0,0,1]\n\t"
        "s_nop 1"
        : "=&v"(lo)
        : "v"(v0), "v"(v1), "v"(hi));
    return lo;
}
__device__ __forceinline__ float attn_max3(float a, float b, float c)
{
    return __builtin_elementwise_maximum(__builtin_elementwise_maximum(a, b), c);
}

__global__ __launch_bounds__(ATH) void attention_split_kernel(const _Float16* __restrict__ QKVhi, const _Float16* __restrict__ QKVlo,
                                                               _Float16* __restrict__ Ohi, _Float16* __restrict__ Olo, int B, int H,
                                                               int C, int Mpad, float inv_s2)
{
    __shared__ __attribute__((aligned(16))) _Float16 sm[2 * AKEYS * AKS + 2 * 64 * AVS];
    __shared__ __attribute__((aligned(16))) float xq[64], xs[T_TOK + 3], xred[2][8], xo[8][64];
    _Float16* sKh = sm;
    _Float16* sKl = sKh + AKEYS * AKS;
    _Float16* sVh = sKl + AKEYS * AKS;
    _Float16* sVl = sVh + 64 * AVS;
    const int bh = xcd_chunked_tile(blockIdx.x, B * H);
    if (bh < 0) return;
    const int h = bh % H, b = bh / H;
    const int tid = threadIdx.x, lane = tid & 63, wave = tid >> 6, half = lane >> 5, l31 = lane & 31;
    const size_t ld = 3 * (size_t)C, tok0 = (size_t)b * T_TOK;

    const int pl = tid >> 8, t8 = tid & 255;
    const _Float16* Ksrc = (pl ? QKVlo : QKVhi) + tok0 * ld + C + h * 64;
    _Float16* sKp = pl ? sKl : sKh;
    unsigned* sVp = reinterpret_cast<unsigned*>(pl ? sVl : sVh);
    const bool odd = (lane & 8) != 0;
    au32x4 kvA[3], vvA[3], kvB[3], vvB[3];
    auto load_chunk = [&](int c3, au32x4 (&kv)[3], au32x4 (&vv)[3]) __attribute__((always_inline)) {
#pragma unroll
        for (int u = 0; u < 3; ++u) {
            const int c = t8 + 256 * (3 * c3 + u), key = c >> 3, ch8 = c & 7;
            kv[u] = au32x4{0u, 0u, 0u, 0u};
            vv[u] = au32x4{0u, 0u, 0u, 0u};
            if (key < T_TOK) {
                const _Float16* src = Ksrc + (size_t)key * ld + 8 * ch8;
                kv[u] = *reinterpret_cast<const au32x4*>(src);
                vv[u] = *reinterpret_cast<const au32x4*>(src + C);
            }
        }
    };
    auto store_chunk = [&](int c3, au32x4 (&kv)[3], au32x4 (&vv)[3]) __attribute__((always_inline)) {
#pragma unroll
        for (int u = 0; u < 3; ++u) {
            const int c = t8 + 256 * (3 * c3 + u), key = c >> 3, ch8 = c & 7;
            const unsigned r0 = __shfl_xor(odd ? vv[u][0] : vv[u][2], 8), r1 = __shfl_xor(odd ? vv[u][1] : vv[u][3], 8);
            if (key < T_TOK + 1) {
                *reinterpret_cast<au32x4*>(sKp + key * AKS + 8 * ch8) = kv[u];
                const unsigned e0 = odd ? r0 : vv[u][0], e1 = odd ? r1 : vv[u][1];
                const unsigned o0 = odd ? vv[u][2] : r0, o1 = odd ? vv[u][3] : r1;
                unsigned* dst = sVp + ((8 * ch8 + (odd ? 4 : 0)) * AVS + (key & ~1)) / 2;
                dst[0 * (AVS / 2)] = (e0 & 0xffffu) | (o0 << 16);
                dst[1 * (AVS / 2)] = (e0 >> 16) | (o0 & 0xffff0000u);
                dst[2 * (AVS / 2)] = (e1 & 0xffffu) | (o1 << 16);
                dst[3 * (AVS / 2)] = (e1 >> 16) | (o1 & 0xffff0000u);
            }
        }
    };
    load_chunk(0, kvA, vvA);
    load_chunk(1, kvB, vvB);
    for (int c = tid; c < 2 * (AKEYS - T_TOK - 1) * 8; c += ATH) {
        const int plane = c >= (AKEYS - T_TOK - 1) * 8 ? 1 : 0, r = c - plane * (AKEYS - T_TOK - 1) * 8;
        *reinterpret_cast<au32x4*>((plane ? sKl : sKh) + (T_TOK + 1 + (r >> 3)) * AKS + 8 * (r & 7)) = au32x4{0u, 0u, 0u, 0u};
    }
    {
        constexpr int ZW = (AVS - T_TOK - 1) / 2;
        for (int c = tid; c < 2 * 64 * ZW; c += ATH) {
            const int plane = c >= 64 * ZW ? 1 : 0, r = c - plane * 64 * ZW;
            reinterpret_cast<unsigned*>(plane ? sVl : sVh)[((r / ZW) * AVS + T_TOK + 1) / 2 + r % ZW] = 0u;
        }
    }
    const int tq = wave * 32 + l31;
    const size_t qo = (tok0 + tq) * ld + h * 64 + 8 * half;
    if (tid < 64) {
        const size_t q256 = (tok0 + (T_TOK - 1)) * ld + h * 64 + tid;
        xq[tid] = (float)QKVhi[q256] + (float)QKVlo[q256];
    }
    store_chunk(0, kvA, vvA);
    load_chunk(2, kvA, vvA);
    store_chunk(1, kvB, vvB);
    store_chunk(2, kvA, vvA);
    __syncthreads();

    f32x16 o0, o1;
#pragma unroll
    for (int r = 0; r < 16; ++r) { o0[r] = 0.f; o1[r] = 0.f; }
    float m_run = -INFINITY, l_part = 0.f;
    const float s_scale = (0.125f * inv_s2) * 1.4426950408889634f;

#pragma unroll 1
    for (int ch = 0; ch < 3; ++ch) {
        f32x16 s[3];
        v16x8 qh[4], ql[4];
#pragma unroll
        for (int kb = 0; kb < 4; ++kb) {
            qh[kb] = *reinterpret_cast<const v16x8*>(QKVhi + qo + 16 * kb);
            ql[kb] = *reinterpret_cast<const v16x8*>(QKVlo + qo + 16 * kb);
        }
        unsigned akh = lds_addr(sKh) + 2u * ((ch * 96 + l31) * AKS + 8 * half), akl = akh + 2u * (AKEYS * AKS);
        unsigned avh = lds_addr(sVh) + 2u * (l31 * AVS + ch * 96 + 4 * half), avl = avh + 2u * (64 * AVS);
        asm volatile("" : "+v"(akh), "+v"(akl), "+v"(avh), "+v"(avl));
#pragma unroll
        for (int t = 0; t < 3; ++t) {
#pragma unroll
            for (int r = 0; r < 16; ++r) s[t][r] = 0.f;
#pragma unroll
            for (int kb = 0; kb < 4; ++kb) {
                const v16x8 kh = *(lds_v16x8p)(size_t)(akh + 2u * (t * 32 * AKS + 16 * kb));
                const v16x8 kl = *(lds_v16x8p)(size_t)(akl + 2u * (t * 32 * AKS + 16 * kb));
                s[t] = __builtin_amdgcn_mfma_f32_32x32x16_f16(kh, qh[kb], s[t], 0, 0, 0);
                s[t] = __builtin_amdgcn_mfma_f32_32x32x16_f16(kh, ql[kb], s[t], 0, 0, 0);
                s[t] = __builtin_amdgcn_mfma_f32_32x32x16_f16(kl, qh[kb], s[t], 0, 0, 0);
            }
        }
        float cmax = -INFINITY;
        if (ch == 2) {
#pragma unroll
            for (int r = 0; r < 16; ++r) s[2][r] = (256 + frag_row(r, lane) < T_TOK) ? s[2][r] : -INFINITY;
        }
#pragma unroll
        for (int t = 0; t < 3; ++t)
#pragma unroll
            for (int r = 0; r < 16; r += 2) cmax = attn_max3(cmax, s[t][r], s[t][r + 1]);
        cmax = fmaxf(cmax, __shfl_xor(cmax, 32)) * s_scale;
        const float mb = fmaxf(m_run, cmax - 15.0f);
        const float alpha = __builtin_amdgcn_exp2f(m_run - mb);
        const float nmb = -mb;
        float psum = 0.f;
#pragma unroll
        for (int t = 0; t < 3; ++t)
#pragma unroll
            for (int r = 0; r < 16; ++r) {
                const float pp = __builtin_amdgcn_exp2f(__builtin_fmaf(s[t][r], s_scale, nmb));
                s[t][r] = pp;
                psum += pp;
            }
        l_part = l_part * alpha + psum;
#pragma unroll
        for (int r = 0; r < 16; ++r) { o0[r] *= alpha; o1[r] *= alpha; }
        m_run = mb;
#pragma unroll
        for (int t = 0; t < 3; ++t)
#pragma unroll
            for (int m = 0; m < 2; ++m) {
                au32x4 phu, plu;
#pragma unroll
                for (int e = 0; e < 8; e += 2) {
                    const float px = s[t][8 * m + e], py = s[t][8 * m + e + 1];
                    const unsigned hp = attn_hi_pair(px, py);
                    phu[e >> 1] = hp;
                    plu[e >> 1] = attn_lo_pair(px, py, hp);
                }
                const v16x8 ph = __builtin_bit_cast(v16x8, phu), pl = __builtin_bit_cast(v16x8, plu);
#pragma unroll
                for (int dh = 0; dh < 2; ++dh) {
                    const unsigned vo = 2u * (32 * dh * AVS + t * 32 + 16 * m);
                    const v16x4 a0 = *(lds_v16x4p)(size_t)(avh + vo), a1 = *(lds_v16x4p)(size_t)(avh + vo + 16u);
                    const v16x4 b0 = *(lds_v16x4p)(size_t)(avl + vo), b1 = *(lds_v16x4p)(size_t)(avl + vo + 16u);
                    v16x8 vh, vl;
#pragma unroll
                    for (int e = 0; e < 4; ++e) { vh[e] = a0[e]; vh[4 + e] = a1[e]; vl[e] = b0[e]; vl[4 + e] = b1[e]; }
                    if (dh == 0) {
                        o0 = __builtin_amdgcn_mfma_f32_32x32x16_f16(vh, ph, o0, 0, 0, 0);
                        o0 = __builtin_amdgcn_mfma_f32_32x32x16_f16(vh, pl, o0, 0, 0, 0);
                        o0 = __builtin_amdgcn_mfma_f32_32x32x16_f16(vl, ph, o0, 0, 0, 0);
                    } else {
                        o1 = __builtin_amdgcn_mfma_f32_32x32x16_f16(vh, ph, o1, 0, 0, 0);
                        o1 = __builtin_amdgcn_mfma_f32_32x32x16_f16(vh, pl, o1, 0, 0, 0);
                        o1 = __builtin_amdgcn_mfma_f32_32x32x16_f16(vl, ph, o1, 0, 0, 0);
                    }
                }
            }
    }
    const float sc = 1.0f / (l_part + __shfl_xor(l_part, 32));
    {
        const size_t row = (tok0 + tq) * C + h * 64;
#pragma unroll
        for (int dh = 0; dh < 2; ++dh)
#pragma unroll
            for (int r4 = 0; r4 < 4; ++r4) {
                typedef unsigned int au32x2 __attribute__((ext_vector_type(2)));
                au32x2 hv, lv;
#pragma unroll
                for (int e = 0; e < 4; e += 2) {
                    float v0 = (dh ? o1[4 * r4 + e] : o0[4 * r4 + e]) * sc, v1 = (dh ? o1[4 * r4 + e + 1] : o0[4 * r4 + e + 1]) * sc;
                    asm volatile("" : "+v"(v0), "+v"(v1));
                    const unsigned hp = attn_hi_pair(v0, v1);
                    hv[e >> 1] = hp;
                    lv[e >> 1] = attn_lo_pair(v0, v1, hp);
                }
                const size_t o = row + 32 * dh + frag_row(4 * r4, lane);
                *reinterpret_cast<au32x2*>(Ohi + o) = hv;
                *reinterpret_cast<au32x2*>(Olo + o) = lv;
            }
    }
    {
        float sv = -INFINITY;
        if (tid < T_TOK) {
            const _Float16* kh = sKh + tid * AKS;
            const _Float16* kl = sKl + tid * AKS;
            float a = 0.f;
#pragma unroll
            for (int c8 = 0; c8 < 8; ++c8) {
                const v16x8 h8 = *reinterpret_cast<const v16x8*>(kh + 8 * c8), l8 = *reinterpret_cast<const v16x8*>(kl + 8 * c8);
#pragma unroll
                for (int e = 0; e < 8; ++e) {
                    a = __builtin_fmaf((float)h8[e], xq[8 * c8 + e], a);
                    a = __builtin_fmaf((float)l8[e], xq[8 * c8 + e], a);
                }
            }
            sv = a * (0.125f * inv_s2);
        }
        float mx = sv;
#pragma unroll
        for (int off = 32; off >= 1; off >>= 1) mx = fmaxf(mx, __shfl_xor(mx, off));
        if (lane == 0) xred[0][wave] = mx;
        __syncthreads();
        mx = xred[0][0];
#pragma unroll
        for (int w = 1; w < 8; ++w) mx = fmaxf(mx, xred[0][w]);
        const float pr = tid < T_TOK ? exp_neg(sv - mx) : 0.f;
        if (tid < T_TOK) xs[tid] = pr;
        float ps = pr;
#pragma unroll
        for (int off = 32; off >= 1; off >>= 1) ps += __shfl_xor(ps, off);
        if (lane == 0) xred[1][wave] = ps;
        __syncthreads();
        {
            const _Float16* vh = sVh + lane * AVS + 32 * wave;
            const _Float16* vl = sVl + lane * AVS + 32 * wave;
            v16x4 h4[8], l4[8];
            f32x4 p4[8];
#pragma unroll
            for (int u = 0; u < 8; ++u) {
                h4[u] = *reinterpret_cast<const v16x4*>(vh + 4 * u);
                l4[u] = *reinterpret_cast<const v16x4*>(vl + 4 * u);
                p4[u] = *reinterpret_cast<const f32x4*>(xs + 32 * wave + 4 * u);
            }
            float a = 0.f;
#pragma unroll
            for (int u = 0; u < 8; ++u)
#pragma unroll
                for (int e = 0; e < 4; ++e) {
                    a = __builtin_fmaf((float)h4[u][e], p4[u][e], a);
                    a = __builtin_fmaf((float)l4[u][e], p4[u][e], a);
                }
            if (wave == 0) {
                a = __builtin_fmaf((float)sVh[lane * AVS + T_TOK - 1], xs[T_TOK - 1], a);
                a = __builtin_fmaf((float)sVl[lane * AVS + T_TOK - 1], xs[T_TOK - 1], a);
            }
            xo[wave][lane] = a;
        }
        __syncthreads();
        if (tid < 64) {
            float l = xred[1][0], a = xo[0][tid];
#pragma unroll
            for (int w = 1; w < 8; ++w) { l += xred[1][w]; a += xo[w][tid]; }
            float v = a * (1.0f / l);
            asm volatile("" : "+v"(v));
            const _Float16 hh = (_Float16)v;
            const size_t o = (tok0 + (T_TOK - 1)) * C + h * 64 + tid;
            Ohi[o] = hh;
            Olo[o] = (_Float16)(v - (float)hh);
        }
    }
}

static bool g_vit_planes = true;
#ifdef GP_PROBES
extern "C" void gp_vit_set_planes(int on) { g_vit_planes = on != 0; }
#endif

__global__ __launch_bounds__(256) void features_kernel(const float* __restrict__ X, float* __restrict__ out,
                                                        int C, int Mpad, int normalize, int* __restrict__ status)
{
    const int b = blockIdx.x, p = threadIdx.x;
    const int c0 = (int)((long long)C * blockIdx.y / gridDim.y), c1 = (int)((long long)C * (blockIdx.y + 1) / gridDim.y);
    const float* x = X + (size_t)b * T_TOK + 1 + p;
    float d = 1.f;
    if (normalize) {
        float ss = 0.f;
        int c = 0;
        for (; c + 16 <= C; c += 16) {
            float v[16];
#pragma unroll
            for (int u = 0; u < 16; ++u) v[u] = x[(size_t)(c + u) * Mpad];
#pragma unroll
            for (int u = 0; u < 16; ++u) ss = __builtin_fmaf(v[u], v[u], ss);
        }
        for (; c < C; ++c) {
            const float v = x[(size_t)c * Mpad];
            ss = __builtin_fmaf(v, v, ss);
        }
        d = fmaxf(__builtin_sqrtf(ss), 1e-12f);
        if (blockIdx.y == 0 && !(ss <= 3.0e38f)) gp_raise(status, GP_ST_SPLIT_RANGE);
    }
    float* o = out + (size_t)b * C * GP_P + p;
    for (int c = c0; c < c1; ++c) o[(size_t)c * GP_P] = normalize ? x[(size_t)c * Mpad] / d : x[(size_t)c * Mpad];
}

int launch_features(const float* X, float* out, int B, int C, int Mpad, int normalize, hipStream_t st)
{
    hipLaunchKernelGGL(features_kernel, dim3(B, B >= 64 ? 4 : (B >= 16 ? 16 : 32)), dim3(256), 0, st, X, out, C, Mpad, normalize,
                       gp_status_buffer());
    return 0;
}

inline int round_up(int x, int m) { return (x + m - 1) / m * m; }

}

enum { W_PATCH_WT = 0, W_PATCH_B, W_CLS_POS, W_POS_T, W_HEADER = 4 };
enum { L_LN1_G = 0, L_LN1_B, L_QK_WT, L_QK_B, L_V_WT, L_V_B, L_PROJ_WT, L_PROJ_B, L_LS1, L_LN2_G, L_LN2_B,
       L_FC1_WT, L_FC1_B, L_FC2_WT, L_FC2_B, L_LS2, L_PER_LAYER = 16 };

extern "C" {

size_t gp_vit_workspace_bytes(int B, int dim, int mlp_dim)
{
    if (B <= 0 || dim <= 0 || mlp_dim <= 0) return 0;
    const size_t Mpad = (size_t)round_up(B * T_TOK, 256);
    size_t f = (size_t)mlp_dim * Mpad;
    const size_t pe_need = (size_t)KPE_PAD * B * GP_P + (size_t)dim * B * GP_P;
    if (pe_need > f) f = pe_need;
    return sizeof(float) * ((size_t)5 * dim * Mpad + f) + gp_gemm_streamk_bytes();
}

enum { S_QK_HI = 0, S_QK_LO, S_V_HI, S_V_LO, S_PROJ_HI, S_PROJ_LO, S_FC1_HI, S_FC1_LO, S_FC2_HI, S_FC2_LO, S_PER_LAYER = 10 };
int gp_vit_forward_split2(const float* images, int B, int dim, int depth, int heads, int mlp_dim, float ln_eps,
                          const float* const* weights, int n_weights, const void* const* split, int n_split,
                          float* workspace, size_t workspace_bytes, float* out_features, int normalize,
                          int stop_after_layers, const float* plane_scales, float* plane_amax, void* stream);

int gp_attention_split_scaled(const void* qkv_hi, const void* qkv_lo, void* out_hi, void* out_lo, int B, int heads, int dim, int Mpad,
                              float qkv_scale, void* stream);
int gp_attention_split_scaled(const void* qkv_hi, const void* qkv_lo, void* out_hi, void* out_lo, int B, int heads, int dim, int Mpad,
                              float qkv_scale, void* stream)
{
    GP_REQUIRE(qkv_scale > 0.f, "gp_attention_split: bad plane scale");
    GP_REQUIRE(qkv_hi && qkv_lo && out_hi && out_lo && B > 0 && heads > 0 && dim == heads * 64 && Mpad >= B * T_TOK,
               "gp_attention_split: bad arguments");
    hipLaunchKernelGGL(attention_split_kernel, dim3(xcd_chunked_grid(B * heads)), dim3(ATH), 0, (hipStream_t)stream,
                       (const _Float16*)qkv_hi, (const _Float16*)qkv_lo, (_Float16*)out_hi, (_Float16*)out_lo, B, heads, dim, Mpad, 1.0f / (qkv_scale * qkv_scale));
    GP_CHECK_LAUNCH("gp_attention_split");
    return GP_OK;
}

int gp_layernorm_planes(const float* X, void* out_hi, void* out_lo, const float* gamma, const float* beta, int C, int Mpad, float eps,
                        void* stream)
{
    GP_REQUIRE(X && out_hi && out_lo && gamma && beta && C > 0 && C % 128 == 0 && Mpad > 0 && Mpad % 64 == 0, "gp_layernorm_planes: bad arguments");
    launch_layernorm_planes(X, (_Float16*)out_hi, (_Float16*)out_lo, gamma, beta, C, Mpad, eps, (hipStream_t)stream);
    GP_CHECK_LAUNCH("gp_layernorm_planes");
    return GP_OK;
}

#ifdef GP_PROBES
int gp_vit_attention_f32(const float* qk, const float* vt, float* out, int B, int heads, int dim, int Mpad, void* stream)
{
    GP_REQUIRE(qk && vt && out && B > 0 && heads > 0 && dim == heads * 64 && Mpad > 0 && Mpad % 256 == 0 && (long long)Mpad >= (long long)B * T_TOK,
               "gp_vit_attention_f32: bad arguments");
    launch_attention_f32(qk, vt, out, B, heads, dim, Mpad, (hipStream_t)stream);
    GP_CHECK_LAUNCH("gp_vit_attention_f32");
    return GP_OK;
}

int gp_vit_layernorm_f32(const float* X, float* Y, const float* gamma, const float* beta, int C, int Mpad, float eps, void* stream)
{
    GP_REQUIRE(X && Y && gamma && beta && C > 0 && C % 16 == 0 && Mpad > 0 && Mpad % 64 == 0, "gp_vit_layernorm_f32: bad arguments");
    launch_layernorm(X, Y, gamma, beta, C, Mpad, eps, (hipStream_t)stream);
    GP_CHECK_LAUNCH("gp_vit_layernorm_f32");
    return GP_OK;
}

int gp_vit_features(const float* X, float* out, int B, int C, int Mpad, int normalize, void* stream)
{
    GP_REQUIRE(X && out && B > 0 && C > 0 && Mpad > 0 && (long long)Mpad >= (long long)B * T_TOK, "gp_vit_features: bad arguments");
    launch_features(X, out, B, C, Mpad, normalize, (hipStream_t)stream);
    GP_CHECK_LAUNCH("gp_vit_features");
    return GP_OK;
}
#endif

int gp_vit_forward(const float* images, int B, int dim, int depth, int heads, int mlp_dim, float ln_eps,
                   const float* const* weights, int n_weights, float* workspace, size_t workspace_bytes,
                   float* out_features, int normalize, int stop_after_layers, void* stream)
{
    return gp_vit_forward_split2(images, B, dim, depth, heads, mlp_dim, ln_eps, weights, n_weights, nullptr, 0, workspace,
                                 workspace_bytes, out_features, normalize, stop_after_layers, nullptr, nullptr, stream);
}

int gp_vit_forward_split2(const float* images, int B, int dim, int depth, int heads, int mlp_dim, float ln_eps,
                          const float* const* weights, int n_weights, const void* const* split, int n_split,
                          float* workspace, size_t workspace_bytes, float* out_features, int normalize,
                          int stop_after_layers, const float* plane_scales, float* plane_amax, void* stream)
{
    hipStream_t st = (hipStream_t)stream;
    enum { PS_LN1 = 0, PS_QKV, PS_LN2, PS_GELU, PS_PER_LAYER = 4 };
    if (plane_scales)
        for (int i = 0; i < depth * PS_PER_LAYER; ++i) {
            int ex = 0;
            GP_REQUIRE(plane_scales[i] > 0.f && frexpf(plane_scales[i], &ex) == 0.5f && plane_scales[i] <= 64.f && plane_scales[i] >= 1.0f / 1024.0f,
                       "gp_vit_forward_split2: plane scale %d = %g is not a power of two in [2^-10, 64]", i, (double)plane_scales[i]);
        }
    GP_REQUIRE(B >= 0 && dim > 0 && depth > 0 && heads > 0, "gp_vit_forward: bad config");
    if (B == 0) return GP_OK;
    GP_REQUIRE(dim == heads * 64, "gp_vit_forward: head dim must be 64 (dim=%d heads=%d)", dim, heads);
    GP_REQUIRE(dim % 128 == 0 && mlp_dim % 128 == 0, "gp_vit_forward: dim/mlp_dim must be multiples of 128");
    GP_REQUIRE(n_weights == W_HEADER + depth * L_PER_LAYER, "gp_vit_forward: expected %d weight pointers, got %d",
               W_HEADER + depth * L_PER_LAYER, n_weights);
    GP_REQUIRE(images && weights && workspace && out_features, "gp_vit_forward: null pointer");
    GP_REQUIRE(workspace_bytes >= gp_vit_workspace_bytes(B, dim, mlp_dim), "gp_vit_forward: workspace too small");
    for (int i = 0; i < n_weights; ++i) GP_REQUIRE(weights[i], "gp_vit_forward: weight pointer %d is null", i);
    GP_REQUIRE(split == nullptr || n_split == depth * S_PER_LAYER || n_split == 2 * depth * S_PER_LAYER,
               "gp_vit_forward_split: expected %d (or %d) split planes, got %d", depth * S_PER_LAYER, 2 * depth * S_PER_LAYER, n_split);
    const int sp_stride = (split && n_split == 2 * depth * S_PER_LAYER) ? 2 * S_PER_LAYER : S_PER_LAYER;
    const bool have_x64 = split && sp_stride >= 2 * S_PER_LAYER;
    if (split) {
        GP_REQUIRE(dim % 32 == 0 && mlp_dim % 32 == 0, "gp_vit_forward_split: dim / mlp_dim must be multiples of 32");
        for (int i = 0; i < n_split; ++i) GP_REQUIRE(split[i], "gp_vit_forward_split: split plane %d is null", i);
    }

    const int C = dim, Mpad = round_up(B * T_TOK, 256), BP = B * GP_P;
    float* X = workspace;
    float* Hn = X + (size_t)C * Mpad;
    float* QK = Hn + (size_t)C * Mpad;
    float* Vt = QK + (size_t)2 * C * Mpad;
    float* F = Vt + (size_t)C * Mpad;
    size_t f_floats = (size_t)mlp_dim * Mpad;
    if ((size_t)KPE_PAD * B * GP_P + (size_t)dim * B * GP_P > f_floats) f_floats = (size_t)KPE_PAD * B * GP_P + (size_t)dim * B * GP_P;
    float* SK = F + f_floats;
    float* col = F;
    float* pe = F + (size_t)KPE_PAD * BP;
    int rc;

    if ((rc = gp_gemm_streamk_reset_launch(SK, st))) return rc;
    hipLaunchKernelGGL(im2col_kernel, dim3(KPE_PAD, B), dim3(256), 0, st, images, col, B);
    GP_CHECK_LAUNCH("gp_vit_forward/im2col");
    if ((rc = gp_gemm_launch(weights[W_PATCH_WT], C, col, BP, pe, BP, C, BP, KPE_PAD, 1 ,
                             weights[W_PATCH_B], nullptr, nullptr, 0, SK, st)))
        return rc;
    hipLaunchKernelGGL(embed_kernel, dim3(C, B + 1), dim3(320), 0, st, pe, weights[W_CLS_POS], weights[W_POS_T],
                       X, B, Mpad);
    GP_CHECK_LAUNCH("gp_vit_forward/embed");

    const int nl = (stop_after_layers >= 0 && stop_after_layers < depth) ? stop_after_layers : depth;
    const int Mtok = B * T_TOK;
    const bool planes = have_x64 && g_vit_planes && gp_gemm_planes256_usable(2 * C, Mpad, Mtok, C) &&
                        gp_gemm_planes256_usable(C, Mpad, Mtok, C) && gp_gemm_planes256_usable(mlp_dim, Mpad, Mtok, C) &&
                        gp_gemm_planes256_usable(C, Mpad, Mtok, mlp_dim);
    if (planes) {
        _Float16* Hhi = reinterpret_cast<_Float16*>(Hn);
        _Float16* Hlo = Hhi + (size_t)C * Mpad;
        _Float16* Fhi = reinterpret_cast<_Float16*>(F);
        _Float16* Flo = Fhi + (size_t)mlp_dim * Mpad;
        const float ps_default[PS_PER_LAYER] = {kPlaneScale, kPlaneScale, kPlaneScale, kPlaneScale};
        for (int l = 0; l < nl; ++l) {
            const float* const* w = weights + W_HEADER + l * L_PER_LAYER;
            const void* const* sq = split + l * sp_stride + S_PER_LAYER;
            const float* ps = plane_scales ? plane_scales + l * PS_PER_LAYER : ps_default;
            float* am = plane_amax ? plane_amax + l * PS_PER_LAYER : nullptr;
            const float os_ln1 = 1.0f / (ps[PS_LN1] * 64.0f), os_qkv = 1.0f / (ps[PS_QKV] * 64.0f), os_ln2 = 1.0f / (ps[PS_LN2] * 64.0f),
                        os_gelu = 1.0f / (ps[PS_GELU] * 64.0f);
            const GpPlaneOut po_qkv{ps[PS_QKV], am ? am + PS_QKV : nullptr}, po_gelu{ps[PS_GELU], am ? am + PS_GELU : nullptr};
            launch_layernorm_planes(X, Hhi, Hlo, w[L_LN1_G], w[L_LN1_B], C, Mpad, ln_eps, st, ps[PS_LN1], am ? am + PS_LN1 : nullptr);
            GP_CHECK_LAUNCH("gp_vit_forward/layernorm_planes");
            _Float16* Ahi = reinterpret_cast<_Float16*>(QK);
            _Float16* Alo = Ahi + (size_t)3 * C * Mpad;
            const bool fused_qkv = (const char*)sq[S_V_HI] == (const char*)sq[S_QK_HI] + (size_t)2 * C * C * 2 &&
                                   (const char*)sq[S_V_LO] == (const char*)sq[S_QK_LO] + (size_t)2 * C * C * 2 && w[L_V_B] == w[L_QK_B] + 2 * C &&
                                   gp_gemm_planes256_usable(3 * C, Mpad, Mtok, C);
            if (fused_qkv) {
                if ((rc = gp_gemm_planes256_launch(sq[S_QK_HI], sq[S_QK_LO], Hhi, Hlo, nullptr, 0, Ahi, Alo, 3 * C, 3 * C, Mpad, Mtok, C,
                                                   7 , w[L_QK_B], nullptr, nullptr, 0, os_ln1, SK, st, nullptr, &po_qkv)))
                    return rc;
            } else {
                if ((rc = gp_gemm_planes256_launch(sq[S_QK_HI], sq[S_QK_LO], Hhi, Hlo, nullptr, 0, Ahi, Alo, 3 * C, 2 * C, Mpad, Mtok, C,
                                                   7 , w[L_QK_B], nullptr, nullptr, 0, os_ln1, SK, st, nullptr, &po_qkv)))
                    return rc;
                if ((rc = gp_gemm_planes256_launch(sq[S_V_HI], sq[S_V_LO], Hhi, Hlo, nullptr, 0, Ahi + 2 * C, Alo + 2 * C, 3 * C, C, Mpad, Mtok, C,
                                                   7 , w[L_V_B], nullptr, nullptr, 0, os_ln1, SK, st, nullptr, &po_qkv)))
                    return rc;
            }
            {
                GpProfScope prof(GP_PROF_ATTN, 4.0 * B * heads * 257.0 * 257.0 * 64.0, st);
                hipLaunchKernelGGL(attention_split_kernel, dim3(xcd_chunked_grid(B * heads)), dim3(ATH), 0, st, Ahi, Alo, Hhi, Hlo, B,
                                   heads, C, Mpad, 1.0f / (ps[PS_QKV] * ps[PS_QKV]));
            }
            GP_CHECK_LAUNCH("gp_vit_forward/attention_split");
            if ((rc = gp_gemm_planes256_launch(sq[S_PROJ_HI], sq[S_PROJ_LO], Hhi, Hlo, X, Mpad, nullptr, nullptr, 0, C, Mpad, Mtok, C,
                                               3 , w[L_PROJ_B], w[L_LS1], X, Mpad, os_qkv, SK, st)))
                return rc;
            launch_layernorm_planes(X, Hhi, Hlo, w[L_LN2_G], w[L_LN2_B], C, Mpad, ln_eps, st, ps[PS_LN2], am ? am + PS_LN2 : nullptr);
            GP_CHECK_LAUNCH("gp_vit_forward/layernorm_planes");
            if ((rc = gp_gemm_planes256_launch(sq[S_FC1_HI], sq[S_FC1_LO], Hhi, Hlo, nullptr, 0, Fhi, Flo, mlp_dim, mlp_dim, Mpad, Mtok, C,
                                               6 , w[L_FC1_B], nullptr, nullptr, 0, os_ln2, SK, st, nullptr, &po_gelu)))
                return rc;
            if ((rc = gp_gemm_planes256_launch(sq[S_FC2_HI], sq[S_FC2_LO], Fhi, Flo, X, Mpad, nullptr, nullptr, 0, C, Mpad, Mtok, mlp_dim,
                                               3 , w[L_FC2_B], w[L_LS2], X, Mpad, os_gelu, SK, st)))
                return rc;
        }
    }
    for (int l = planes ? nl : 0; l < nl; ++l) {
        const float* const* w = weights + W_HEADER + l * L_PER_LAYER;
        launch_layernorm(X, Hn, w[L_LN1_G], w[L_LN1_B], C, Mpad, ln_eps, st);
        GP_CHECK_LAUNCH("gp_vit_forward/layernorm");
        const void* const* sp = split ? split + l * sp_stride : nullptr;
        const void* const* sq = (sp && have_x64) ? sp + S_PER_LAYER : nullptr;
        auto sgemm = [&](const float* act, int ld_act, int which, float* D, int ldd, int I, int J, int K, int act_is_b, int epi,
                         const float* bias, const float* scale, const float* res, int ldr) -> int {
            if (sq && gp_gemm_split256_usable(I, J, K))
                return gp_gemm_split256_launch(act, ld_act, sq[which], sq[which + 1], D, ldd, I, J, K, act_is_b, epi, bias, scale, res,
                                               ldr, SK, st);
            return gp_gemm_split_launch(act, ld_act, sp[which], sp[which + 1], D, ldd, I, J, K, act_is_b, epi, bias, scale, res, ldr, st);
        };
        if (sp) rc = sgemm(Hn, Mpad, S_QK_HI, QK, Mpad, 2 * C, Mpad, C, 1, 1, w[L_QK_B], nullptr, nullptr, 0);
        else rc = gp_gemm_launch(w[L_QK_WT], 2 * C, Hn, Mpad, QK, Mpad, 2 * C, Mpad, C, 1, w[L_QK_B], nullptr, nullptr, 0, SK, st);
        if (rc) return rc;
        if (sp) rc = sgemm(Hn, Mpad, S_V_HI, Vt, C, Mpad, C, C, 0, 4 , w[L_V_B], nullptr, nullptr, 0);
        else rc = gp_gemm_launch(Hn, Mpad, w[L_V_WT], C, Vt, C, Mpad, C, C, 4 , w[L_V_B], nullptr, nullptr, 0, SK, st);
        if (rc) return rc;
        launch_attention_f32(QK, Vt, Hn, B, heads, C, Mpad, st);
        GP_CHECK_LAUNCH("gp_vit_forward/attention");
        if (sp) rc = sgemm(Hn, Mpad, S_PROJ_HI, X, Mpad, C, Mpad, C, 1, 3, w[L_PROJ_B], w[L_LS1], X, Mpad);
        else rc = gp_gemm_launch(w[L_PROJ_WT], C, Hn, Mpad, X, Mpad, C, Mpad, C, 3, w[L_PROJ_B], w[L_LS1], X, Mpad, SK, st);
        if (rc) return rc;
        launch_layernorm(X, Hn, w[L_LN2_G], w[L_LN2_B], C, Mpad, ln_eps, st);
        GP_CHECK_LAUNCH("gp_vit_forward/layernorm");
        if (sp) rc = sgemm(Hn, Mpad, S_FC1_HI, F, Mpad, mlp_dim, Mpad, C, 1, 2 , w[L_FC1_B], nullptr, nullptr, 0);
        else rc = gp_gemm_launch(w[L_FC1_WT], mlp_dim, Hn, Mpad, F, Mpad, mlp_dim, Mpad, C, 2 , w[L_FC1_B], nullptr,
                                 nullptr, 0, SK, st);
        if (rc) return rc;
        if (sp) rc = sgemm(F, Mpad, S_FC2_HI, X, Mpad, C, Mpad, mlp_dim, 1, 3, w[L_FC2_B], w[L_LS2], X, Mpad);
        else rc = gp_gemm_launch(w[L_FC2_WT], C, F, Mpad, X, Mpad, C, Mpad, mlp_dim, 3, w[L_FC2_B], w[L_LS2], X, Mpad, SK, st);
        if (rc) return rc;
    }
    launch_features(X, out_features, B, C, Mpad, normalize, st);
    GP_CHECK_LAUNCH("gp_vit_forward/features");
    return GP_OK;
}

}
```

gigapose_amd/gigaPose.py:

```python
import os
import ctypes
import os.path as osp
import time

import numpy as np
import pandas as pd
import torch
from torch import nn

from . import _lib
from .matching import MatchBank
from .poses import ObjectPoseRecovery
from .tensor_collection import PandasTensorCollection

try:
    import pytorch_lightning as pl

    _Base = pl.LightningModule
except Exception:
    class _Base(nn.Module):
        global_rank = 0
        logger = None

        @property
        def device(self):
            try:
                return next(self.parameters()).device
            except StopIteration:
                return torch.device("cpu")


def stable_argsort_desc(score):
    return torch.sort(score, dim=1, descending=True, stable=True).indices


def rank_hypotheses(pred, sort=True):
    isc = pred.ransac_scores.contiguous()
    B, k, num_patches = isc.shape
    dev = isc.device
    if not isc.is_cuda or isc.dtype != torch.int64:
        raise _lib.GigaPoseHipError(f"rank_hypotheses needs the int64 device tensor gp_ransac writes, got {isc.dtype} on {isc.device}")
    score = torch.empty(B, k, dtype=torch.float32, device=dev)
    order = torch.empty(B, k, dtype=torch.int64, device=dev)
    names = list(pred.tensors) if sort else []
    srcs = [pred.tensors[n].contiguous() for n in names]
    for v in srcs:
        if v.shape[:2] != (B, k):
            raise ValueError(f"per-hypothesis tensors must be (B, k, ...), got {tuple(v.shape)}")
    dsts = [torch.empty_like(v) for v in srcs]
    for s0 in range(0, max(len(srcs), 1), 16):
        a, b = srcs[s0:s0 + 16], dsts[s0:s0 + 16]
        n = len(a)
        src_t = (ctypes.c_void_p * max(n, 1))(*[v.data_ptr() for v in a])
        dst_t = (ctypes.c_void_p * max(n, 1))(*[v.data_ptr() for v in b])
        rb_t = (ctypes.c_int * max(n, 1))(*[v[0, 0].numel() * v.element_size() if B else 1 for v in a])
        _lib.call("gp_rank_hypotheses", _lib.ptr(isc), _lib.i(B), _lib.i(k), _lib.i(num_patches), _lib.i(1 if sort else 0),
                  _lib.ptr(score), _lib.ptr(order), _lib.i(n), src_t, dst_t, rb_t, _lib.stream_ptr())
    for name, v in zip(names, dsts):
        pred.register_tensor(name, v)
    pred.register_tensor("scores", score)
    return order


class GigaPose(_Base):
    def __init__(self, model_name, ae_net, ist_net, training_loss, testing_metric, optim_config, log_interval,
                 log_dir, max_num_dets_per_forward=None, test_setting="localization", **kwargs):
        super().__init__()
        numerics = kwargs.pop("numerics", None)
        accumulate = kwargs.pop("accumulate_crops", None)
        ownership = kwargs.pop("image_ownership", None)
        self.model_name = model_name
        self.ae_net = ae_net
        self.ist_net = ist_net
        self.training_loss = training_loss
        self.testing_metric = testing_metric
        self.max_num_dets_per_forward = max_num_dets_per_forward
        self.test_setting = test_setting
        self.log_interval = log_interval
        self.log_dir = log_dir
        os.makedirs(osp.join(self.log_dir, "predictions"), exist_ok=True)
        self.optim_config = optim_config
        self.template_datas = {}
        self.match_banks = {}
        self.pose_recovery = {}
        self.run_id = None
        self.template_datasets = None
        self.test_dataset_name = None
        self.last_predictions = None
        self.template_shard = None
        env = os.environ.get("GIGAPOSE_OVERLAP_IST", "auto").strip().lower()
        self.overlap_ist = "auto" if env == "auto" else env in ("1", "true", "on")
        self._side_stream = None
        self.accumulate_crops = int(os.environ.get("GIGAPOSE_ACCUMULATE_CROPS", "64")) if accumulate is None else int(accumulate)
        self._pending = []
        self._pending_crops = 0
        self._in_flight = None
        self._feat_shapes = {}
        self._sharded_flow = None
        self.image_ownership = (os.environ.get("GIGAPOSE_IMAGE_OWNERSHIP") or None) if ownership is None else (ownership or None)
        if self.image_ownership not in (None, "round_robin"):
            raise ValueError("image_ownership must be None or 'round_robin'")
        if numerics is not None:
            self.set_numerics(numerics)

    def set_numerics(self, mode):
        if mode not in _lib.NUMERICS:
            raise ValueError(f"numerics must be one of {_lib.NUMERICS}")
        self.ae_net.dinov2_model.set_numerics(mode)
        self.testing_metric.numerics = mode
        self.ist_net.backbone.set_numerics(mode)
        self.template_datas, self.match_banks, self.pose_recovery = {}, {}, {}
        return self

    def _widen_split_range(self, bits):
        import warnings

        changed = []
        vit = getattr(self.ae_net, "dinov2_model", None)
        if bits & 4 and vit is not None and getattr(vit, "numerics", None) == "split" and getattr(vit, "split_gemm", "128") != "128":
            vit.set_split_gemm("128")
            changed.append("ViT linear layers -> 128 x 128 two-accumulator kernels (Dinov2ViT.set_split_gemm('128'))")
        ist = getattr(self.ist_net, "backbone", None)
        if bits & 16 and ist is not None and getattr(ist, "numerics", None) == "split" and getattr(ist, "conv_kernel", "128") != "128":
            ist.conv_kernel = "128"
            ist.invalidate()
            changed.append("IST convolutions -> 128 x 128 two-accumulator kernel (ResNet.conv_kernel = '128')")
        if changed:
            warnings.warn("split numerics: an activation left the range of the f16 planes (|x| >= 8190); falling back for this model: "
                          + "; ".join(changed) + ".  Template banks are rebuilt.", RuntimeWarning)
            names = [n for n in self.template_datas if n in (self.template_datasets or {})]
            self.template_datas, self.match_banks, self.pose_recovery = {}, {}, {}
            for name in names:
                self.set_template_data(name)
        return bool(changed)

    def _calibrate_planes(self, images):
        vit = getattr(self.ae_net, "dinov2_model", None)
        if vit is None or not hasattr(vit, "calibrate_plane_scales"):
            return False
        sharded = self.template_shard is not None
        group = self.template_shard[2] if sharded else None
        changed = False
        for x in ([images] if torch.is_tensor(images) else images):
            changed = vit.calibrate_plane_scales(x.to(self.device), group=group, sync_ranks=sharded) or changed
        _lib.raise_status(_lib.take_status() & ~_lib.SPLIT_RANGE_BITS)
        return changed

    def _needs_calibration(self):
        vit = getattr(self.ae_net, "dinov2_model", None)
        return (vit is not None and getattr(vit, "numerics", None) == "split" and getattr(vit, "split_gemm", "128") != "128"
                and hasattr(vit, "calibrate_plane_scales") and vit.plane_amax is None)

    def _recover_range(self, bits, images):
        import warnings

        if bits & 4 and images is not None:
            vit = self.ae_net.dinov2_model
            if getattr(vit, "numerics", None) == "split" and getattr(vit, "split_gemm", "128") != "128" and self._calibrate_planes(images):
                warnings.warn("split numerics: a ViT activation left the range of its f16 planes; plane scales re-calibrated on the offending "
                              f"inputs: {vit.plane_scale_report()} (tensor: (max |x|, scale)); all GEMMs stay on the 256 x 256 kernels.", RuntimeWarning)
                return "recalibrated"
        return "widened" if self._widen_split_range(bits) else False

    def _collect_status(self):
        bits = _lib.take_status()
        if self.template_shard is not None:
            import torch.distributed as dist

            _, world, group = self.template_shard
            if world > 1:
                dev = self.device if dist.get_backend(group) != "gloo" else torch.device("cpu")
                flags = torch.tensor([(bits >> b) & 1 for b in range(16)], dtype=torch.int32, device=dev)
                dist.all_reduce(flags, op=dist.ReduceOp.MAX, group=group)
                bits = sum(int(f) << b for b, f in enumerate(flags.tolist()))
        return bits

    def enable_template_sharding(self, group=None):
        import torch.distributed as dist

        self.template_shard = (dist.get_rank(group), dist.get_world_size(group), group)

    @torch.no_grad()
    def set_template_data(self, dataset_name):
        t0 = time.time()
        template_dataset = self.template_datasets[dataset_name]
        dev = self.device
        if torch.device(dev).type == "cuda":
            _lib.status_word(dev)
        if self._needs_calibration() and len(template_dataset):
            self._calibrate_planes(template_dataset[idx].rgb for idx in range(len(template_dataset)))
        cols = {n: [] for n in ["mask", "K", "M", "poses", "ae_features", "ist_features"]}
        lo, hi = 0, None
        if self.template_shard is not None:
            from .sharding import ShardedMatcher, shard_bounds

            rank, world, group = self.template_shard
        for idx in range(len(template_dataset)):
            item = template_dataset[idx]
            templates = item.rgb.to(dev)
            if self.template_shard is not None:
                lo, hi = shard_bounds(templates.shape[0], world, rank)
            cols["ae_features"].append(self.ae_net(templates)[lo:hi].contiguous())
            cols["ist_features"].append(self.ist_net.forward_by_chunk(templates))
            for n in ["mask", "K", "M", "poses"]:
                cols[n].append(getattr(item, n).to(dev))
        data = {n: torch.stack(v, dim=0) for n, v in cols.items()}
        self.template_datas[dataset_name] = PandasTensorCollection(infos=pd.DataFrame(), **data)
        if self.template_shard is None:
            self.match_banks[dataset_name] = MatchBank(data["ae_features"], data["mask"], self.testing_metric.numerics,
                                                       self.testing_metric.bank_dtype)
        else:
            shard = MatchBank(data["ae_features"], data["mask"][:, lo:hi].contiguous(), self.testing_metric.numerics,
                              self.testing_metric.bank_dtype)
            self.match_banks[dataset_name] = ShardedMatcher(self.testing_metric, shard, lo, group)
        self.pose_recovery[dataset_name] = ObjectPoseRecovery(template_K=data["K"], template_Ms=data["M"],
                                                              template_poses=data["poses"])
        torch.cuda.synchronize()
        bits = self._collect_status()
        if bits & _lib.SPLIT_RANGE_BITS:
            how = self._recover_range(bits, (template_dataset[idx].rgb for idx in range(len(template_dataset))))
            if how == "widened" and dataset_name in self.template_datas:
                return
            if how:
                self.template_datas.pop(dataset_name, None)
                return self.set_template_data(dataset_name)
        _lib.raise_status(bits)
        self.onboarding_time = (time.time() - t0) / max(1, len(template_dataset))

    @torch.no_grad()
    def predict(self, tar_img, tar_mask, tar_K, tar_M, labels, dataset_name, sort_pred_by_inliers=True, exchange_aux=None, live_rows=None):
        bank = self.match_banks[dataset_name]
        template_data = self.template_datas[dataset_name]
        n_obj = template_data.ist_features.shape[0]
        if not labels.is_cuda and labels.numel() and (int(labels.min()) < 1 or int(labels.max()) > n_obj):
            raise IndexError(f"detection label outside 1..{n_obj} (the reference indexes ae_features[label - 1], gigaPose.py:520)")
        if tar_img.is_cuda:
            _lib.status_word(tar_img.device)
        if not labels.is_cuda and tar_img.is_cuda:
            labels0 = (labels.to(torch.int64) - 1).to(torch.int32).contiguous().pin_memory().to(tar_img.device, non_blocking=True)
        else:
            labels0 = (labels.to(tar_img.device) - 1).to(torch.int32).contiguous()
        side = None
        if tar_img.is_cuda and (self.overlap_ist is True or (self.overlap_ist == "auto" and tar_img.shape[0] <= 32)):
            main = torch.cuda.current_stream()
            if self._side_stream is None:
                self._side_stream = torch.cuda.Stream(device=tar_img.device)
            side = self._side_stream
            side.wait_stream(main)
            with torch.cuda.stream(side):
                tar_ist = self._backbone_rows("ist", self.ist_net.forward_by_chunk, tar_img, live_rows)
        tar_ae = self._backbone_rows("ae", self.ae_net, tar_img, live_rows)
        if self.template_shard is None:
            pred = self.testing_metric.test_bank(bank, tar_ae, tar_mask, labels0)
            if side is None:
                tar_ist = self._backbone_rows("ist", self.ist_net.forward_by_chunk, tar_img, live_rows)
        else:
            pending = bank.start_exchange(tar_ae, tar_mask, labels0, exchange_aux)
            if side is None:
                tar_ist = self._backbone_rows("ist", self.ist_net.forward_by_chunk, tar_img, live_rows)
            pred = bank.finish(pending)
        if side is not None:
            torch.cuda.current_stream().wait_stream(side)
            tar_ist.record_stream(torch.cuda.current_stream())
        rel_scale, rel_inplane = self.ist_net.regress_bank(template_data.ist_features, labels0, pred.id_src,
                                                           tar_ist, pred.src_pts, pred.tar_pts)
        pred.register_tensor("relScale", rel_scale)
        pred.register_tensor("relInplane", rel_inplane)
        pred = self.pose_recovery[dataset_name].forward_ransac(predictions=pred)
        rank_hypotheses(pred, sort_pred_by_inliers)
        poses = self.pose_recovery[dataset_name].forward_recovery(
            tar_label=labels, tar_K=tar_K, tar_M=tar_M, pred_src_views=pred.id_src, pred_M=pred.M, labels0=labels0)
        pred.register_tensor("pred_poses", poses)
        return pred

    def _backbone_rows(self, key, net, tar_img, live_rows):
        B = tar_img.shape[0]
        if live_rows is None or live_rows >= B:
            out = net(tar_img)
            self._feat_shapes[key] = (tuple(out.shape[1:]), out.dtype)
            return out
        if live_rows == 0 and key in self._feat_shapes:
            shape, dtype = self._feat_shapes[key]
            return torch.zeros((B,) + shape, dtype=dtype, device=tar_img.device)
        feat = net(tar_img[:max(live_rows, 1)])
        self._feat_shapes[key] = (tuple(feat.shape[1:]), feat.dtype)
        out = feat.new_zeros((B,) + tuple(feat.shape[1:]))
        if live_rows > 0:
            out[:live_rows] = feat[:live_rows]
        return out

    def eval_retrieval(self, batch, idx_batch, dataset_name, sort_pred_by_inliers=True):
        if dataset_name not in self.template_datas:
            self.set_template_data(dataset_name)
        labels_np = np.asarray(batch.infos.label).astype(np.int32)
        if self.template_shard is not None:
            from .sharding import require_same_batch

            require_same_batch(len(labels_np), batch.tar_img.device, self.template_shard[2])
        t0 = time.time()
        labels = torch.from_numpy(labels_np)
        predictions = self.predict(batch.tar_img, batch.tar_mask, batch.tar_K, batch.tar_M, labels, dataset_name,
                                   sort_pred_by_inliers)
        torch.cuda.synchronize()
        bits = self._collect_status()
        if bits & _lib.SPLIT_RANGE_BITS and self._recover_range(bits, batch.tar_img):
            return self.eval_retrieval(batch, idx_batch, dataset_name, sort_pred_by_inliers)
        _lib.raise_status(bits)
        predictions.infos = batch.infos
        total_time = time.time() - t0
        self.last_predictions = predictions
        save_path = osp.join(self.log_dir, "predictions", f"{idx_batch}.npz")
        if getattr(batch, "test_list", None) is not None:
            return self.filter_and_save(predictions, test_list=batch.test_list, time=total_time, save_path=save_path,
                                        keep_only_testing_instances=(self.test_setting == "localization"))
        return None, predictions

    def filter_and_save(self, predictions, test_list, time, save_path, keep_only_testing_instances=True):
        labels = np.asarray(predictions.infos.label).astype(np.int32)
        assert len(np.unique(labels)) == len(np.unique(test_list.infos.obj_id))
        top_scores = predictions.scores[:, 0].cpu().numpy()
        selected, detection_times = list(range(len(labels))), [0.0] * len(labels)
        if keep_only_testing_instances:
            selected, detection_times = [], []
            for row, obj_id in enumerate(test_list.infos.obj_id):
                num_inst = int(test_list.infos.inst_count[row])
                cand = np.flatnonzero(labels == obj_id)
                best = cand[np.argsort(-top_scores[cand], kind="stable")[:num_inst]]
                selected.extend(best.tolist())
                detection_times.extend([test_list.infos.detection_time[row]] * num_inst)
        predictions = predictions[selected]
        det_t = torch.from_numpy(np.asarray(detection_times, dtype=np.float64)).to(predictions.scores.device)
        predictions.register_tensor("detection_time", det_t)
        predictions.register_tensor("time", torch.ones_like(det_t) * time)
        np.savez(save_path,
                 scene_id=np.asarray(predictions.infos.scene_id).astype(np.int32),
                 im_id=np.asarray(predictions.infos.view_id).astype(np.int32),
                 object_id=np.asarray(predictions.infos.label).astype(np.int32),
                 time=predictions.time.cpu().numpy(), detection_time=predictions.detection_time.cpu().numpy(),
                 poses=predictions.pred_poses.cpu().numpy(), scores=predictions.scores.cpu().numpy())
        return selected, predictions

    @torch.no_grad()
    def test_step(self, batch, idx_batch):
        if self.image_ownership == "round_robin":
            rank, world = self._image_ranks()
            if idx_batch % world != rank:
                return 0
        if self.template_shard is not None and self._flushable(batch):
            self._flow().push(batch, idx_batch)
            return 0
        if not self._accumulating(batch):
            if self.template_shard is None:
                self.flush_pending()
            if self.accumulate_crops == 0 and self.template_shard is None and self._flushable(batch):
                if self.test_dataset_name not in self.template_datas:
                    self.set_template_data(self.test_dataset_name)
                t0 = time.time()
                job = self._run_flush([(batch, idx_batch, self._bind())], self.test_dataset_name)
                job["ev"][1].synchronize()
                job["wall_s"] = time.time() - t0
                self._finish_flush(job)
                return 0
            self.eval_retrieval(batch, idx_batch=idx_batch, dataset_name=self.test_dataset_name)
            return 0
        bound = self._bind()
        if self._pending and self._pending[-1][2] != bound:
            self.flush_pending()
        self._pending.append((batch, idx_batch, bound))
        self._pending_crops += len(batch.infos)
        if self._pending_crops >= self.accumulate_crops:
            self._launch_flush()
        return 0

    def _flushable(self, batch):
        return getattr(batch, "test_list", None) is not None and batch.tar_img.is_cuda

    def _accumulating(self, batch):
        return self.accumulate_crops > 0 and self.template_shard is None and self._flushable(batch)

    def _bind(self):
        return (self.test_dataset_name, self.log_dir, self.test_setting)

    def _flow(self):
        if self._sharded_flow is None:
            from .sharded_flow import ShardedFlow

            self._sharded_flow = ShardedFlow(self)
        return self._sharded_flow

    def _image_ranks(self):
        import torch.distributed as dist

        if self.template_shard is not None:
            return self.template_shard[0], self.template_shard[1]
        if dist.is_available() and dist.is_initialized():
            return dist.get_rank(), dist.get_world_size()
        return 0, 1

    @torch.no_grad()
    def _launch_flush(self):
        dataset_name = self._pending[0][2][0] if self._pending else self.test_dataset_name
        if dataset_name not in self.template_datas:
            self.set_template_data(dataset_name)
        take, n = [], 0
        while self._pending and (not take or n + len(self._pending[0][0].infos) <= max(self.accumulate_crops, 1)):
            take.append(self._pending.pop(0))
            n += len(take[-1][0].infos)
        self._pending_crops -= n
        job = self._run_flush(take, dataset_name)
        prev, self._in_flight = self._in_flight, job
        if prev is not None:
            self._finish_flush(prev)

    def _run_flush(self, images, dataset_name):
        batches = [im[0] for im in images]
        cat = (lambda name: batches[0].tensors[name]) if len(batches) == 1 else (lambda name: torch.cat([b.tensors[name] for b in batches], dim=0))
        labels_np = np.concatenate([np.asarray(b.infos.label).astype(np.int32) for b in batches])
        job = self._run_rows({n: cat(n) for n in ("tar_img", "tar_mask", "tar_K", "tar_M")}, labels_np, dataset_name)
        job["images"] = images
        return job

    def _run_rows(self, inputs, labels_np, dataset_name, aux=None, live_rows=None):
        dev = inputs["tar_img"].device
        n = len(labels_np)
        ev0, ev1 = torch.cuda.Event(enable_timing=True), torch.cuda.Event(enable_timing=True)
        ev0.record()
        recovery = self.pose_recovery[dataset_name]
        keep_asserts, recovery.check_asserts = recovery.check_asserts, ("deferred" if recovery.check_asserts else False)
        sharded = self.template_shard is not None
        aux_t = None
        if sharded:
            aux_t = torch.full((n,), int(aux or 0), dtype=torch.int32).pin_memory().to(dev, non_blocking=True)
        try:
            pred = self.predict(inputs["tar_img"], inputs["tar_mask"], inputs["tar_K"], inputs["tar_M"], torch.from_numpy(labels_np), dataset_name,
                                exchange_aux=aux_t, live_rows=live_rows)
        finally:
            recovery.check_asserts = keep_asserts
        word = _lib.status_word(dev)
        flag = recovery.deferred_flag if keep_asserts else None
        host = {"scores": torch.empty(pred.scores.shape, dtype=pred.scores.dtype, pin_memory=True),
                "pred_poses": torch.empty(pred.pred_poses.shape, dtype=pred.pred_poses.dtype, pin_memory=True),
                "bad_crop_M": torch.zeros(1, dtype=torch.int32, pin_memory=True)}
        host["scores"].copy_(pred.scores, non_blocking=True)
        host["pred_poses"].copy_(pred.pred_poses, non_blocking=True)
        if sharded:
            from .sharding import all_gather_rows

            words, _ = all_gather_rows(word.view(1, 1), self.template_shard[2])
            host["status"] = torch.zeros(words.shape[0], dtype=torch.int32, pin_memory=True)
            host["status"].copy_(words.reshape(-1), non_blocking=True)
            aux_all = self.match_banks[dataset_name].last_aux
            host["aux_all"] = torch.zeros(aux_all.shape[0], dtype=torch.int32, pin_memory=True)
            host["aux_all"].copy_(aux_all, non_blocking=True)
        else:
            host["status"] = torch.zeros(1, dtype=torch.int32, pin_memory=True)
            host["status"].copy_(word, non_blocking=True)
        word.zero_()
        if flag is not None:
            host["bad_crop_M"].copy_(flag, non_blocking=True)
        ev1.record()
        return dict(inputs=inputs, labels=labels_np, pred=pred, host=host, ev=(ev0, ev1), dataset_name=dataset_name, device=dev)

    def _clear_crop_flag(self, dataset_name):
        flag = self.pose_recovery[dataset_name]._flag
        if flag is not None:
            flag.zero_()

    def _finish_flush(self, job):
        job["ev"][1].synchronize()
        bits = int(job["host"]["status"][0])
        redone = False
        while bits & _lib.SPLIT_RANGE_BITS and self._recover_range(bits, [im[0].tar_img for im in job["images"]]):
            if not redone:
                nxt, self._in_flight = self._in_flight, None
                self._drain_device()
                redone = True
            wall = "wall_s" in job
            t0 = time.time()
            job = self._run_flush(job["images"], job["dataset_name"])
            job["ev"][1].synchronize()
            if wall:
                job["wall_s"] = time.time() - t0
            bits = int(job["host"]["status"][0])
        _lib.raise_status(bits)
        if redone and nxt is not None:
            self._in_flight = self._run_flush(nxt["images"], nxt["dataset_name"])
        if int(job["host"]["bad_crop_M"][0]) != 0:
            self._clear_crop_flag(job["dataset_name"])
            raise AssertionError("tar_M must be an isotropic scale + translation")
        total_ms = 1e3 * job["wall_s"] if "wall_s" in job else job["ev"][0].elapsed_time(job["ev"][1])
        scores, poses = job["host"]["scores"].numpy(), job["host"]["pred_poses"].numpy()
        n_all, a = len(job["labels"]), 0
        for batch, idx_batch, (_, log_dir, test_setting) in job["images"]:
            n = len(batch.infos)
            save_path = osp.join(log_dir, "predictions", f"{idx_batch}.npz")
            self._save_image(batch.infos, batch.test_list, scores[a:a + n], poses[a:a + n], 1e-3 * total_ms * n / max(n_all, 1), save_path,
                             test_setting == "localization")
            a += n
        pred = job["pred"]
        pred.infos = pd.concat([im[0].infos for im in job["images"]], axis=0, sort=False).reset_index(drop=True)
        self.last_predictions = pred

    @staticmethod
    def _drain_device():
        torch.cuda.synchronize()
        _lib.take_status()

    @staticmethod
    def _save_image(infos, test_list, scores, poses, time, save_path, keep_only_testing_instances):
        labels = np.asarray(infos.label).astype(np.int32)
        assert len(np.unique(labels)) == len(np.unique(test_list.infos.obj_id))
        selected, detection_times = list(range(len(labels))), [0.0] * len(labels)
        if keep_only_testing_instances:
            selected, detection_times = [], []
            for row, obj_id in enumerate(test_list.infos.obj_id):
                num_inst = int(test_list.infos.inst_count[row])
                cand = np.flatnonzero(labels == obj_id)
                best = cand[np.argsort(-scores[cand, 0], kind="stable")[:num_inst]]
                selected.extend(best.tolist())
                detection_times.extend([test_list.infos.detection_time[row]] * num_inst)
        det_t = np.asarray(detection_times, dtype=np.float64)
        sel = np.asarray(selected, dtype=np.int64)
        np.savez(save_path,
                 scene_id=np.asarray(infos.scene_id).astype(np.int32)[sel], im_id=np.asarray(infos.view_id).astype(np.int32)[sel],
                 object_id=labels[sel], time=np.ones_like(det_t) * time, detection_time=det_t,
                 poses=poses[sel], scores=scores[sel])
        return selected

    def flush_pending(self):
        if self.template_shard is not None:
            if self._sharded_flow is not None or self.test_dataset_name is not None:
                self._flow().drain()
            return
        while self._pending:
            self._launch_flush()
        if self._in_flight is not None:
            job, self._in_flight = self._in_flight, None
            self._finish_flush(job)
            if self._in_flight is not None:
                job, self._in_flight = self._in_flight, None
                self._finish_flush(job)

    def on_test_epoch_end(self):
        self.flush_pending()
        import torch.distributed as dist

        if dist.is_available() and dist.is_initialized():
            group = self.template_shard[2] if self.template_shard is not None else None
            if dist.get_world_size(group) > 1:
                dist.barrier(group=group)
        if self.global_rank != 0:
            return
        from .inout import save_predictions_from_batched_predictions

        save_predictions_from_batched_predictions(osp.join(self.log_dir, "predictions"),
                                                  dataset_name=self.test_dataset_name, model_name=self.model_name,
                                                  run_id=self.run_id, is_refined=False)
```

gigapose_amd/matching.py:

```python
import os

import pandas as pd
import torch

from . import _lib
from .tensor_collection import PandasTensorCollection

P = 256


def patch_grid_mask(mask224):
    assert mask224.shape[-1] % 16 == 0 and mask224.shape[-2] % 16 == 0
    sy, sx = mask224.shape[-2] // 16, mask224.shape[-1] // 16
    m = mask224[..., ::sy, ::sx].to(torch.float32)
    return m.reshape(*m.shape[:-2], P).contiguous()


default_numerics = _lib.default_numerics


def _l2norm_split(x, hi, lo, rows, C):
    _lib.call("gp_l2norm_split_mask", _lib.ptr(x), _lib.ptr(hi), _lib.ptr(lo), _lib.i(rows), _lib.i(C), _lib.ptr(None), _lib.i(0), _lib.i(0),
              _lib.ptr(None), _lib.stream_ptr())


def normalize_split(feats, mask224=None):
    rows, C = feats.shape[:2]
    x = feats.reshape(rows, C, P).contiguous().float()
    hi = torch.empty(rows, P, (C + 31) // 32 * 32, dtype=torch.float16, device=x.device)
    lo = torch.empty_like(hi)
    if mask224 is None:
        _l2norm_split(x, hi, lo, rows, C)
        return hi, lo
    fused = (mask224.dtype == torch.float32 and mask224.is_contiguous() and mask224.dim() == 3 and mask224.shape[0] == rows
             and mask224.shape[1] % 16 == 0 and mask224.shape[2] % 16 == 0)
    if not fused:
        _l2norm_split(x, hi, lo, rows, C)
        return hi, lo, patch_grid_mask(mask224)
    qmask = torch.empty(rows, P, dtype=torch.float32, device=x.device)
    _lib.call("gp_l2norm_split_mask", _lib.ptr(x), _lib.ptr(hi), _lib.ptr(lo), _lib.i(rows), _lib.i(C), _lib.ptr(mask224),
              _lib.i(mask224.shape[1]), _lib.i(mask224.shape[2]), _lib.ptr(qmask), _lib.stream_ptr())
    return hi, lo, qmask


class MatchBank:

    def __init__(self, ae_features, masks224, numerics=None, bank_dtype=None):
        self.numerics = numerics or default_numerics()
        self.bank_dtype = bank_dtype or os.environ.get("GIGAPOSE_BANK_DTYPE", "f32")
        if self.bank_dtype not in ("f32", "f16") or (self.bank_dtype == "f16" and self.numerics != "split"):
            raise ValueError("bank_dtype must be 'f32' or 'f16' ('f16' needs numerics='split')")
        O, N, C = ae_features.shape[:3]
        feats = ae_features.reshape(O * N, C, P).contiguous().float()
        self.features = self.hi = self.lo = None
        if self.numerics == "split":
            hi, lo = normalize_split(feats)
            self.hi = hi.view(O, N, P, -1)
            self.lo = lo.view(O, N, P, -1) if self.bank_dtype == "f32" else None
        else:
            self.features = torch.empty_like(feats)
            _lib.call("gp_l2norm_cp", _lib.ptr(feats), _lib.ptr(self.features), _lib.i(O * N), _lib.i(C),
                      _lib.stream_ptr())
            self.features = self.features.view(O, N, C, P)
        self.masks = patch_grid_mask(masks224)
        self.O, self.N, self.C = O, N, C


class LocalSimilarity(torch.nn.Module):
    def __init__(self, k, sim_threshold, patch_threshold, search_direction="tar2src",
                 image_size=224, patch_size=14, max_batch_size=32):
        super().__init__()
        if search_direction not in ("tar2src", "src2tar"):
            raise ValueError(f"search_direction must be 'tar2src' or 'src2tar', got {search_direction!r}")
        self.max_batch_size = max_batch_size
        self.k = k
        self.sim_threshold = sim_threshold
        self.patch_threshold = patch_threshold
        self.search_direction = search_direction
        self.num_patches = image_size // patch_size
        self.numerics = default_numerics()
        self.bank_dtype = None
        if self.num_patches != 16:
            raise NotImplementedError("kernels are specialised for a 16x16 patch grid (224/14)")

    def normalize(self, feats):
        if self.numerics == "split":
            return normalize_split(feats.reshape(feats.shape[0], feats.shape[1], P))
        rows, C = feats.shape[:2]
        x = feats.reshape(rows, C, P).contiguous().float()
        out = torch.empty_like(x)
        _lib.call("gp_l2norm_cp", _lib.ptr(x), _lib.ptr(out), _lib.i(rows), _lib.i(C), _lib.stream_ptr())
        return out

    def match_tiles(self, query, qmask, bank, labels0, search_direction=None, out=None):
        split = isinstance(query, (tuple, list))
        if split != (getattr(bank, "numerics", "chain") == "split"):
            raise ValueError(f"query numerics and bank numerics ({bank.numerics}) differ")
        B, C = (query[0].shape[0], query[0].shape[2]) if split else query.shape[:2]
        N = bank.N
        dev = qmask.device
        if out is not None:
            idx, sc, ma, avg = out
            want = [((B, N, P), torch.uint8), ((B, N, P), torch.float32), ((B, N, P), torch.float32), ((B, N), torch.float32)]
            if any(tuple(t.shape) != shp or t.dtype != dt or t.device != dev for t, (shp, dt) in zip(out, want)):
                raise ValueError("match_tiles: out must be (idx u8, score f32, mask f32) of shape (B, N, 256) and sim_avg f32 (B, N) on the masks' device")
        else:
            idx = torch.empty(B, N, P, dtype=torch.uint8, device=dev)
            sc = torch.empty(B, N, P, dtype=torch.float32, device=dev)
            ma = torch.empty(B, N, P, dtype=torch.float32, device=dev)
            avg = torch.empty(B, N, dtype=torch.float32, device=dev)
        direction = 1 if (search_direction or self.search_direction) == "src2tar" else 0
        if split:
            _lib.call("gp_match_tiles_split_dir", _lib.ptr(query[0]), _lib.ptr(query[1]), _lib.ptr(bank.hi), _lib.ptr(bank.lo),
                      _lib.ptr(qmask), _lib.ptr(bank.masks), _lib.ptr(labels0), _lib.i(B), _lib.i(bank.O), _lib.i(N),
                      _lib.i(C), _lib.f(self.sim_threshold), _lib.f(self.patch_threshold), _lib.i(direction), _lib.ptr(idx),
                      _lib.ptr(sc), _lib.ptr(ma), _lib.ptr(avg), _lib.stream_ptr())
            return idx, sc, ma, avg
        _lib.call("gp_match_tiles_dir", _lib.ptr(query), _lib.ptr(bank.features), _lib.ptr(qmask),
                  _lib.ptr(bank.masks), _lib.ptr(labels0), _lib.i(B), _lib.i(bank.O), _lib.i(N), _lib.i(C),
                  _lib.f(self.sim_threshold), _lib.f(self.patch_threshold), _lib.i(direction), _lib.ptr(idx), _lib.ptr(sc),
                  _lib.ptr(ma), _lib.ptr(avg), _lib.stream_ptr())
        return idx, sc, ma, avg

    def topk(self, sim_avg, k=None):
        k = self.k if k is None else k
        B, N = sim_avg.shape
        if k > N:
            raise RuntimeError("selected index k out of range")
        ids = torch.empty(B, k, dtype=torch.int32, device=sim_avg.device)
        scores = torch.empty(B, k, dtype=torch.float32, device=sim_avg.device)
        _lib.call("gp_topk", _lib.ptr(sim_avg), _lib.i(B), _lib.i(N), _lib.i(k), _lib.ptr(ids),
                  _lib.ptr(scores), _lib.stream_ptr())
        return ids, scores

    def gather_records(self, ids, idx, sc, ma):
        B, k = ids.shape
        N = idx.shape[1]
        dev = ids.device
        rec_idx = torch.empty(B, k, P, dtype=torch.uint8, device=dev)
        rec_score = torch.empty(B, k, P, dtype=torch.float32, device=dev)
        rec_mask = torch.empty(B, k, P, dtype=torch.float32, device=dev)
        _lib.call("gp_gather_records", _lib.ptr(ids), _lib.ptr(idx), _lib.ptr(sc), _lib.ptr(ma), _lib.i(B),
                  _lib.i(N), _lib.i(k), _lib.ptr(rec_idx), _lib.ptr(rec_score), _lib.ptr(rec_mask),
                  _lib.stream_ptr())
        return rec_idx, rec_score, rec_mask

    def format_points(self, rec_idx, rec_mask):
        B, k = rec_idx.shape[:2]
        tar_pts = torch.empty(B, k, P, 2, dtype=torch.int64, device=rec_idx.device)
        src_pts = torch.empty(B, k, P, 2, dtype=torch.int64, device=rec_idx.device)
        _lib.call("gp_format_points", _lib.ptr(rec_idx), _lib.ptr(rec_mask), _lib.i(B * k), _lib.ptr(tar_pts),
                  _lib.ptr(src_pts), _lib.stream_ptr())
        return tar_pts, src_pts

    def select_topk(self, sim_avg, idx, sc, ma, k=None):
        k = self.k if k is None else k
        B, N = sim_avg.shape
        if k > N:
            raise RuntimeError("selected index k out of range")
        dev = sim_avg.device
        ids = torch.empty(B, k, dtype=torch.int64, device=dev)
        scores = torch.empty(B, k, dtype=torch.float32, device=dev)
        rec_score = torch.empty(B, k, P, dtype=torch.float32, device=dev)
        tar_pts = torch.empty(B, k, P, 2, dtype=torch.int64, device=dev)
        src_pts = torch.empty(B, k, P, 2, dtype=torch.int64, device=dev)
        _lib.call("gp_select_topk", _lib.ptr(sim_avg), _lib.ptr(idx), _lib.ptr(sc), _lib.ptr(ma), _lib.i(B), _lib.i(N), _lib.i(k), _lib.ptr(ids),
                  _lib.ptr(scores), _lib.ptr(rec_score), _lib.ptr(tar_pts), _lib.ptr(src_pts), _lib.stream_ptr())
        return ids, scores, rec_score, tar_pts, src_pts

    def test_bank(self, bank, tar_feat, tar_mask, labels0):
        if self.numerics == "split":
            hi, lo, qmask = normalize_split(tar_feat.reshape(tar_feat.shape[0], tar_feat.shape[1], P), tar_mask)
            query = (hi, lo)
        else:
            query = self.normalize(tar_feat)
            qmask = patch_grid_mask(tar_mask)
        idx, sc, ma, avg = self.match_tiles(query, qmask, bank, labels0.to(torch.int32).contiguous())
        ids, score_src, rec_score, tar_pts, src_pts = self.select_topk(avg, idx, sc, ma)
        return PandasTensorCollection(infos=pd.DataFrame(), id_src=ids, score_src=score_src,
                                      score_pts=rec_score, tar_pts=tar_pts, src_pts=src_pts)

    def val(self, src_feat, tar_feat, src_mask, tar_mask):
        if self.patch_threshold <= 0:
            raise ValueError("patch_threshold must be greater than 0")
        B = tar_feat.shape[0]
        dev = tar_feat.device
        bank = MatchBank(src_feat.unsqueeze(1), src_mask.unsqueeze(1), self.numerics)
        labels0 = torch.arange(B, dtype=torch.int32, device=dev)
        idx, sc, ma, _ = self.match_tiles(self.normalize(tar_feat), patch_grid_mask(tar_mask), bank, labels0, "tar2src")
        tar_pts, src_pts = self.format_points(idx.contiguous(), ma.contiguous())
        return PandasTensorCollection(infos=pd.DataFrame(), src_pts=src_pts[:, 0], tar_pts=tar_pts[:, 0], score=sc[:, 0])

    def test(self, src_feats, tar_feat, src_masks, tar_mask, max_batch_size=None):
        if max_batch_size is None:
            max_batch_size = self.max_batch_size
        B = tar_feat.shape[0]
        outs = []
        for s in range(0, B, max_batch_size):
            e = min(B, s + max_batch_size)
            bank = MatchBank(src_feats[s:e], src_masks[s:e], self.numerics)
            labels0 = torch.arange(e - s, dtype=torch.int32, device=tar_feat.device)
            outs.append(self.test_bank(bank, tar_feat[s:e], tar_mask[s:e], labels0))
        out = outs[0]
        for o in outs[1:]:
            out.cat_df(o)
        return PandasTensorCollection(infos=pd.DataFrame(), **out.tensors)
```

gigapose_amd/vit.py:

```python
import ctypes
import math
import os

import torch
from torch import nn

from . import _lib

VARIANTS = {
    "dinov2_vits14": (384, 12, 6),
    "dinov2_vitb14": (768, 12, 12),
    "dinov2_vitl14": (1024, 24, 16),
}
T = 257
NUMERICS = ("chain", "split")


def split_planes(w):
    w = w.detach().float().contiguous()
    hi = w.half()
    lo = ((w - hi.float()) * 2048.0).half()
    return hi.contiguous(), lo.contiguous()


def split_planes_x64(w):
    w = w.detach().float().contiguous()
    hi = torch.empty(w.shape, dtype=torch.float16, device=w.device)
    lo = torch.empty_like(hi)
    _lib.call("gp_split256_weights", _lib.ptr(w), ctypes.c_size_t(w.numel()), _lib.ptr(hi), _lib.ptr(lo), _lib.stream_ptr())
    return hi, lo


class _Block(nn.Module):
    def __init__(self, dim, mlp_dim):
        super().__init__()
        self.norm1 = nn.LayerNorm(dim, eps=1e-6)
        self.attn = nn.Module()
        self.attn.qkv = nn.Linear(dim, 3 * dim)
        self.attn.proj = nn.Linear(dim, dim)
        self.ls1 = nn.Module()
        self.ls1.gamma = nn.Parameter(torch.ones(dim))
        self.norm2 = nn.LayerNorm(dim, eps=1e-6)
        self.mlp = nn.Module()
        self.mlp.fc1 = nn.Linear(dim, mlp_dim)
        self.mlp.fc2 = nn.Linear(mlp_dim, dim)
        self.ls2 = nn.Module()
        self.ls2.gamma = nn.Parameter(torch.ones(dim))


class Dinov2ViT(nn.Module):

    def __init__(self, dim=1024, depth=24, heads=16, mlp_ratio=4, num_pos=T):
        super().__init__()
        assert dim == heads * 64, "kernels are specialised for head dim 64"
        self.dim, self.depth, self.heads, self.mlp_dim = dim, depth, heads, dim * mlp_ratio
        self.cls_token = nn.Parameter(torch.zeros(1, 1, dim))
        self.pos_embed = nn.Parameter(torch.zeros(1, num_pos, dim))
        self.mask_token = nn.Parameter(torch.zeros(1, dim))
        self.patch_embed = nn.Module()
        self.patch_embed.proj = nn.Conv2d(3, dim, kernel_size=14, stride=14)
        self.blocks = nn.ModuleList([_Block(dim, self.mlp_dim) for _ in range(depth)])
        self.norm = nn.LayerNorm(dim, eps=1e-6)
        self._packed = None
        self._ws = None
        self.numerics = _lib.default_numerics()
        self.split_gemm = "256"
        self.plane_scales = None
        self.plane_amax = None
        self.plane_headroom = 4.0

    def set_split_gemm(self, mode):
        if mode not in ("256", "128"):
            raise ValueError("split_gemm must be '256' or '128'")
        if mode != self.split_gemm:
            self.split_gemm = mode
            self._packed = None
        return self

    def set_numerics(self, mode):
        if mode not in NUMERICS:
            raise ValueError(f"numerics must be one of {NUMERICS}")
        if mode != self.numerics:
            self.numerics = mode
            self._packed = None
        return self

    @classmethod
    def from_name(cls, name):
        dim, depth, heads = VARIANTS[name]
        return cls(dim, depth, heads)

    @classmethod
    def from_hf(cls, hf_model):
        cfg = hf_model.config
        m = cls(cfg.hidden_size, cfg.num_hidden_layers, cfg.num_attention_heads, int(cfg.mlp_ratio))
        sd = hf_model.state_dict()
        out = {
            "cls_token": sd["embeddings.cls_token"],
            "pos_embed": sd["embeddings.position_embeddings"],
            "mask_token": sd["embeddings.mask_token"],
            "patch_embed.proj.weight": sd["embeddings.patch_embeddings.projection.weight"],
            "patch_embed.proj.bias": sd["embeddings.patch_embeddings.projection.bias"],
            "norm.weight": sd["layernorm.weight"],
            "norm.bias": sd["layernorm.bias"],
        }
        for i in range(m.depth):
            p = f"encoder.layer.{i}."
            a = p + "attention.attention."
            out[f"blocks.{i}.norm1.weight"] = sd[p + "norm1.weight"]
            out[f"blocks.{i}.norm1.bias"] = sd[p + "norm1.bias"]
            out[f"blocks.{i}.attn.qkv.weight"] = torch.cat([sd[a + "query.weight"], sd[a + "key.weight"], sd[a + "value.weight"]])
            out[f"blocks.{i}.attn.qkv.bias"] = torch.cat([sd[a + "query.bias"], sd[a + "key.bias"], sd[a + "value.bias"]])
            out[f"blocks.{i}.attn.proj.weight"] = sd[p + "attention.output.dense.weight"]
            out[f"blocks.{i}.attn.proj.bias"] = sd[p + "attention.output.dense.bias"]
            out[f"blocks.{i}.ls1.gamma"] = sd[p + "layer_scale1.lambda1"]
            out[f"blocks.{i}.norm2.weight"] = sd[p + "norm2.weight"]
            out[f"blocks.{i}.norm2.bias"] = sd[p + "norm2.bias"]
            out[f"blocks.{i}.mlp.fc1.weight"] = sd[p + "mlp.fc1.weight"]
            out[f"blocks.{i}.mlp.fc1.bias"] = sd[p + "mlp.fc1.bias"]
            out[f"blocks.{i}.mlp.fc2.weight"] = sd[p + "mlp.fc2.weight"]
            out[f"blocks.{i}.mlp.fc2.bias"] = sd[p + "mlp.fc2.bias"]
            out[f"blocks.{i}.ls2.gamma"] = sd[p + "layer_scale2.lambda1"]
        m.load_state_dict(out)
        return m.eval()

    interpolate_offset = 0.1
    interpolate_antialias = False

    def resample_pos_embed(self, pe):
        pe = pe.float()
        n = int(round(math.sqrt(pe.shape[1] - 1)))
        if n * n != pe.shape[1] - 1:
            raise ValueError(f"pos_embed with {pe.shape[1]} entries is not 1 + a square grid")
        grid = pe[:, 1:].reshape(1, n, n, -1).permute(0, 3, 1, 2)
        if self.interpolate_offset:
            sf = float(16 + self.interpolate_offset) / n
            grid = nn.functional.interpolate(grid, scale_factor=(sf, sf), mode="bicubic", antialias=self.interpolate_antialias)
        else:
            grid = nn.functional.interpolate(grid, size=(16, 16), mode="bicubic", antialias=self.interpolate_antialias)
        if tuple(grid.shape[-2:]) != (16, 16):
            raise ValueError(f"pos_embed resampling produced {tuple(grid.shape[-2:])}, expected (16, 16)")
        return torch.cat([pe[:, :1], grid.permute(0, 2, 3, 1).reshape(1, 256, -1)], dim=1)

    def _load_from_state_dict(self, state_dict, prefix, *args, **kwargs):
        key = prefix + "pos_embed"
        if key in state_dict and state_dict[key].shape[1] != self.pos_embed.shape[1]:
            state_dict[key] = self.resample_pos_embed(state_dict[key])
        self._packed = None
        self.plane_scales = self.plane_amax = None
        return super()._load_from_state_dict(state_dict, prefix, *args, **kwargs)

    def _apply(self, fn, *a, **k):
        self._packed = None
        return super()._apply(fn, *a, **k)

    def invalidate(self):
        self._packed = None
        self.plane_scales = self.plane_amax = None

    @torch.no_grad()
    def _pack(self, device):
        def dev(t):
            return t.detach().to(device=device, dtype=torch.float32).contiguous()

        C = self.dim
        w = self.patch_embed.proj.weight.detach().float().reshape(C, 588).t()
        patch_wt = torch.zeros(592, C)
        patch_wt[:588] = w.cpu()
        tensors = [dev(patch_wt), dev(self.patch_embed.proj.bias),
                   dev((self.cls_token[0, 0] + self.pos_embed[0, 0])),
                   dev(self.pos_embed[0, 1:].t())]
        for blk in self.blocks:
            qkv_w, qkv_b = blk.attn.qkv.weight, blk.attn.qkv.bias
            qkv_bd = dev(qkv_b)
            tensors += [dev(blk.norm1.weight), dev(blk.norm1.bias),
                        dev(qkv_w[:2 * C].t()), qkv_bd[:2 * C],
                        dev(qkv_w[2 * C:].t()), qkv_bd[2 * C:],
                        dev(blk.attn.proj.weight.t()), dev(blk.attn.proj.bias), dev(blk.ls1.gamma),
                        dev(blk.norm2.weight), dev(blk.norm2.bias),
                        dev(blk.mlp.fc1.weight.t()), dev(blk.mlp.fc1.bias),
                        dev(blk.mlp.fc2.weight.t()), dev(blk.mlp.fc2.bias), dev(blk.ls2.gamma)]
        table = (ctypes.c_void_p * len(tensors))(*[t.data_ptr() for t in tensors])
        split, split_table = [], None
        if self.numerics == "split":
            for blk in self.blocks:
                qkv_w = blk.attn.qkv.weight.detach().to(device)
                ws = (qkv_w[:2 * C], qkv_w[2 * C:], blk.attn.proj.weight.to(device), blk.mlp.fc1.weight.to(device),
                      blk.mlp.fc2.weight.to(device))
                for w in ws:
                    split += list(split_planes(w))
                if self.split_gemm != "128":
                    qkv_hi, qkv_lo = split_planes_x64(qkv_w)
                    split += [qkv_hi[:2 * C], qkv_lo[:2 * C], qkv_hi[2 * C:], qkv_lo[2 * C:]]
                    for w in ws[2:]:
                        split += list(split_planes_x64(w))
            split_table = (ctypes.c_void_p * len(split))(*[t.data_ptr() for t in split])
        self._packed = (device, tensors, table, split, split_table)

    def _workspace(self, B, device):
        lib = _lib.lib()
        lib.gp_vit_workspace_bytes.restype = ctypes.c_size_t
        need = lib.gp_vit_workspace_bytes(_lib.i(B), _lib.i(self.dim), _lib.i(self.mlp_dim))
        if self._ws is None or self._ws.numel() * 4 < need or self._ws.device != device:
            self._ws = torch.empty((need + 3) // 4, dtype=torch.float32, device=device)
        return self._ws, need

    PLANE_TENSORS = ("ln1", "qkv", "ln2", "gelu")
    CALIBRATION_SCALE = 2.0 ** -4

    def reset_plane_scales(self):
        self.plane_scales, self.plane_amax = None, None

    @staticmethod
    def scale_for(amax, headroom):
        if not amax > 0.0:
            return 8.0
        return float(min(8.0, max(2.0 ** -10, 2.0 ** math.floor(math.log2(65504.0 / (amax * headroom))))))

    @torch.no_grad()
    def calibrate_plane_scales(self, images, group=None, chunk=64, sync_ranks=False):
        active = self.numerics == "split" and self.split_gemm != "128"
        if not sync_ranks and (not active or images.shape[0] == 0):
            return False
        device = images.device
        amax = torch.zeros(self.depth * 4, dtype=torch.float32, device=device)
        keep = self.plane_scales
        self.plane_scales = [self.CALIBRATION_SCALE] * (self.depth * 4)
        try:
            for s0 in range(0, images.shape[0] if active else 0, chunk):
                self.patch_features(images[s0:s0 + chunk], plane_amax=amax)
        finally:
            self.plane_scales = keep
        if sync_ranks:
            import torch.distributed as dist

            if dist.is_initialized() and dist.get_world_size(group) > 1:
                if dist.get_backend(group) == "gloo":
                    host = amax.cpu()
                    dist.all_reduce(host, op=dist.ReduceOp.MAX, group=group)
                    amax = host
                else:
                    dist.all_reduce(amax, op=dist.ReduceOp.MAX, group=group)
        if not active:
            return False
        seen = amax.double().cpu().numpy().reshape(self.depth, 4)
        if not bool((seen == seen).all()) or not bool((seen < float("inf")).all()):
            raise _lib.GigaPoseHipError("plane-scale calibration: a ViT activation is not finite (NaN / inf input or weights)")
        self.plane_amax = seen if self.plane_amax is None else __import__("numpy").maximum(self.plane_amax, seen)
        new = [self.scale_for(float(a), self.plane_headroom) for a in self.plane_amax.reshape(-1)]
        old = self.plane_scales or [8.0] * (self.depth * 4)
        changed = new != old
        self.plane_scales = None if all(v == 8.0 for v in new) else new
        return changed

    def adopt_plane_amax(self, amax):
        import numpy as np

        amax = np.asarray(amax, dtype=np.float64).reshape(self.depth, 4)
        if not np.isfinite(amax).all() or (amax < 0).any():
            raise ValueError("plane-scale calibration: the adopted maxima must be finite and non-negative")
        self.plane_amax = amax.copy() if self.plane_amax is None else np.maximum(self.plane_amax, amax)
        new = [self.scale_for(float(a), self.plane_headroom) for a in self.plane_amax.reshape(-1)]
        old = self.plane_scales or [8.0] * (self.depth * 4)
        self.plane_scales = None if all(v == 8.0 for v in new) else new
        return new != old

    def plane_scale_report(self):
        if self.plane_scales is None or self.plane_amax is None:
            return {}
        out = {}
        for l in range(self.depth):
            for t, name in enumerate(self.PLANE_TENSORS):
                if self.plane_scales[4 * l + t] != 8.0:
                    out[f"L{l}.{name}"] = (float(self.plane_amax[l, t]), self.plane_scales[4 * l + t])
        return out

    @torch.no_grad()
    def patch_features(self, images, normalize=True, stop_after_layers=-1, plane_amax=None):
        if images.shape[1:] != (3, 224, 224):
            raise ValueError(f"expected (B,3,224,224) crops, got {tuple(images.shape)}")
        device = images.device
        if device.type == "cuda":
            _lib.status_word(device)
        if self._packed is None or self._packed[0] != device:
            self._pack(device)
        B = images.shape[0]
        x = images.contiguous().float()
        out = torch.empty(B, self.dim, 16, 16, dtype=torch.float32, device=device)
        if B == 0:
            return out
        ws, need = self._workspace(B, device)
        _, tensors, table, split, split_table = self._packed
        scales = None
        if self.plane_scales is not None and self.numerics == "split":
            scales = (ctypes.c_float * len(self.plane_scales))(*self.plane_scales)
        _lib.call("gp_vit_forward_split2", _lib.ptr(x), _lib.i(B), _lib.i(self.dim), _lib.i(self.depth),
                  _lib.i(self.heads), _lib.i(self.mlp_dim), _lib.f(1e-6), table, _lib.i(len(tensors)),
                  split_table, _lib.i(len(split)), _lib.ptr(ws), ctypes.c_size_t(need), _lib.ptr(out),
                  _lib.i(1 if normalize else 0), _lib.i(stop_after_layers), scales, _lib.ptr(plane_amax), _lib.stream_ptr())
        return out

    @torch.no_grad()
    def forward_features(self, images):
        B = images.shape[0]
        self.patch_features(images, normalize=False)
        mpad = (B * T + 255) // 256 * 256
        xt = self._ws[: self.dim * mpad].view(self.dim, mpad)[:, : B * T]
        return {"x_prenorm": xt.t().reshape(B, T, self.dim).contiguous()}
```

include/gigapose_hip_probe.h:

```cpp
#ifndef GIGAPOSE_HIP_PROBE_H
#define GIGAPOSE_HIP_PROBE_H
#include "gigapose_hip.h"
#ifdef __cplusplus
extern "C" {
#endif

int gp_match_tiles_split_trace(const void* q_hi, const void* q_lo, const void* b_hi, const void* b_lo, const float* qmask,
                               const float* bmask, const int* labels, int B, int O, int N, int C, float sim_threshold,
                               float patch_threshold, uint8_t* idx_t2s, float* score_t2s, float* mask_all, float* sim_avg,
                               unsigned long long* trace, void* stream);
int gp_match_split_set_compact(int on);

void gp_gemm_set_streamk(int mode);
void gp_gemm_set_group(int g);
int gp_gemm_streamk_error(const float* scratch, void* stream);

int gp_gemm_split_set_trace(unsigned long long* dev_buf);
int gp_gemm_split_timing(const float* act, int ld_act, const void* whi, const void* wlo, float* D, int ldd, int I, int J, int K,
                         unsigned long long* out20 , void* stream);
int gp_gemm_split256_error(const float* scratch, void* stream);
int gp_gemm_planes256_set_dp(int mode);
int gp_gemm_planes256_set_par(int on);
int gp_gemm_planes256_set_half_tiles(int on);
int gp_gemm_planes256_trace(const void* a_hi, const void* a_lo, const void* b_hi, const void* b_lo, float* D, int ldd, void* out_hi,
                            void* out_lo, int ldo, int I, int J, int J_valid, int K, int epilogue, const float* bias, const float* scale,
                            const float* residual, int ldr, float out_scale, float* scratch, unsigned long long* trace, void* stream);
int gp_gemm_planes256_timing(const void* a_hi, const void* a_lo, const void* b_hi, const void* b_lo, float* D, int ldd, int I, int J,
                             int K, float* scratch, unsigned long long* out8, void* stream);

void gp_vit_set_ln_reg(int mode);
void gp_vit_set_planes(int on);
int gp_vit_attention_f32(const float* qk, const float* vt, float* out, int B, int heads, int dim, int Mpad, void* stream);
int gp_vit_layernorm_f32(const float* X, float* Y, const float* gamma, const float* beta, int C, int Mpad, float eps, void* stream);
int gp_vit_features(const float* X, float* out, int B, int C, int Mpad, int normalize, void* stream);

void gp_conv_set_direct(int on);
void gp_conv2d_planes_set_trace(unsigned long long* device_buf);
int gp_conv2d_planes_set_halo(int on);

#ifdef __cplusplus
}
#endif
#endif
```

Before: 1571 query-crops/sec.

## Emit matcher f16 planes from ViT and fuse embedding, LN tail and zeroing

The ViT forward can now write L2-normalised hi/lo f16 query planes straight into the matcher layout, so the separate l2norm split pass over the f32 features is skipped and only a small patch-mask kernel runs. The patch-embedding add of class token, position table and padding zeroing moves into a GEMM epilogue, which removes embed_kernel. The stream-K header reset is folded into im2col. LayerNorm launches only cover live tokens, and a few leftover tokens are folded into existing blocks to avoid a partial wave. This cuts launches and memory passes but adds epilogue complexity and layout coupling between the ViT and the matcher.

```diff
diff --git a/gigapose_amd/ae_net.py b/gigapose_amd/ae_net.py
--- a/gigapose_amd/ae_net.py
+++ b/gigapose_amd/ae_net.py
@@ -48,3 +48,11 @@
 
     def forward(self, images):
         return self.forward_by_chunk(images)
+
+    @torch.no_grad()
+    def forward_planes(self, processed_rgbs):
+        outs = [self.dinov2_model.patch_features(processed_rgbs[s:s + self.max_batch_size], matcher_planes=True)
+                for s in range(0, processed_rgbs.shape[0], self.max_batch_size)]
+        if not outs:
+            return torch.empty(2, 0, 256, self.descriptor_size, dtype=torch.float16, device=processed_rgbs.device)
+        return outs[0] if len(outs) == 1 else torch.cat(outs, dim=1)
diff --git a/gigapose_amd/csrc/gp_gemm.hip b/gigapose_amd/csrc/gp_gemm.hip
--- a/gigapose_amd/csrc/gp_gemm.hip
+++ b/gigapose_amd/csrc/gp_gemm.hip
@@ -9,6 +9,7 @@
     EPI_BIAS_I_SCALE_RES = 3,
     EPI_BIAS_J = 4,
     EPI_BIAS_I_RELU = 5,
+    EPI_EMBED = 8,
 };
 
 using GM = KMajor<2, 4, 2, 1, 16>;
@@ -21,6 +22,7 @@
 constexpr int kMaxSlots = 1024;
 constexpr size_t kSkHeaderBytes = 8192;
 constexpr size_t kSkPartialFloats = (size_t)GM::BM * GM::BN;
+constexpr int T_EMB = GP_P + 1;
 constexpr int kSpinLimit = 400000;
 
 struct GemmArgs {
@@ -66,15 +68,29 @@
         for (int r = 0; r < 16; ++r) {
             const int i = i0 + wm * 64 + mi * 32 + frag_row(r, lane);
             float v = acc[mi][0][r];
-            if (EPI == EPI_BIAS_I || EPI == EPI_BIAS_I_GELU || EPI == EPI_BIAS_I_SCALE_RES || EPI == EPI_BIAS_I_RELU)
+            if (EPI == EPI_BIAS_I || EPI == EPI_BIAS_I_GELU || EPI == EPI_BIAS_I_SCALE_RES || EPI == EPI_BIAS_I_RELU || EPI == EPI_EMBED)
                 v = v + bias[i];
             if (EPI == EPI_BIAS_J) v = v + bias[j];
             if (EPI == EPI_BIAS_I_GELU) v = gelu_erf(v);
             if (EPI == EPI_BIAS_I_RELU) v = fmaxf(v, 0.f);
             if (EPI == EPI_BIAS_I_SCALE_RES) v = res[(unsigned)i * (unsigned)a.ldr + (unsigned)j] + scale[i] * v;
-            D[(unsigned)i * (unsigned)a.ldd + (unsigned)j] = v;
+            if (EPI == EPI_EMBED) v = v + scale[(unsigned)i * GP_P + (unsigned)(j & (GP_P - 1))];
+            D[(unsigned)i * (unsigned)a.ldd + (unsigned)(EPI == EPI_EMBED ? j + (j >> 8) + 1 : j)] = v;
         }
         if (EPI == EPI_BIAS_I_SCALE_RES) __builtin_amdgcn_sched_barrier(0);
+    }
+    if (EPI == EPI_EMBED) {
+        static_assert(GM::BN == 128 && GM::BM <= GM::NT, "EPI_EMBED: one crop start per two j tiles, one class-token row per thread");
+        int t2 = threadIdx.x;
+        asm volatile("" : "+v"(t2));
+        if ((j0 & (GP_P - 1)) == 0 && t2 < GM::BM) D[(unsigned)(i0 + t2) * (unsigned)a.ldd + (unsigned)(j0 + (j0 >> 8))] = res[i0 + t2];
+        if (j0 + GM::BN == a.tiles_j * GM::BN) {
+            const int m0 = a.tiles_j * GM::BN / GP_P * T_EMB, npad = a.ldr - m0;
+            for (int idx = t2; idx < GM::BM * npad; idx += GM::NT) {
+                const int r = idx / npad;
+                D[(unsigned)(i0 + r) * (unsigned)a.ldd + (unsigned)(m0 + idx - r * npad)] = 0.f;
+            }
+        }
     }
 }
 
@@ -237,6 +253,11 @@
             GP_REQUIRE(bias, "gp_gemm_kmajor: bias required");
             launch<EPI_BIAS_I_RELU>(A, lda, B, ldb, D, ldd, I, J, K, bias, scale, res, ldr, sk_ws, st);
             break;
+        case EPI_EMBED:
+            GP_REQUIRE(bias && scale && res && J % GP_P == 0 && ldr == ldd && ldd >= J / GP_P * T_EMB && ldd - J / GP_P * T_EMB < GP_P,
+                       "gp_gemm_kmajor: bias / position table / class token and a (257 B + padding)-column output required");
+            launch<EPI_EMBED>(A, lda, B, ldb, D, ldd, I, J, K, bias, scale, res, ldr, sk_ws, st);
+            break;
         default: GP_REQUIRE(false, "gp_gemm_kmajor: unknown epilogue %d", epilogue);
     }
     GP_CHECK_LAUNCH("gp_gemm_kmajor");
@@ -244,6 +265,8 @@
 }
 
 size_t gp_gemm_streamk_bytes() { return kSkHeaderBytes + sizeof(float) * kSkPartialFloats * kMaxSlots; }
+
+size_t gp_gemm_streamk_header_bytes() { return kSkHeaderBytes; }
 
 int gp_gemm_streamk_reset_launch(float* sk_ws, hipStream_t st)
 {
diff --git a/gigapose_amd/csrc/gp_match.hip b/gigapose_amd/csrc/gp_match.hip
--- a/gigapose_amd/csrc/gp_match.hip
+++ b/gigapose_amd/csrc/gp_match.hip
@@ -613,6 +613,12 @@
     }
 }
 
+__global__ __launch_bounds__(256) void patch_mask_kernel(const float* __restrict__ mask_img, int mh, int mw, float* __restrict__ patch_mask)
+{
+    const int row = blockIdx.x, p = threadIdx.x;
+    patch_mask[(size_t)row * GP_P + p] = mask_img[(size_t)row * mh * mw + (size_t)((p >> 4) * (mh / GP_G)) * mw + (p & 15) * (mw / GP_G)];
+}
+
 __global__ __launch_bounds__(64) void topk_kernel(const float* __restrict__ sim_avg, int N, int k,
                                                    int* __restrict__ ids, float* __restrict__ scores)
 {
@@ -761,10 +767,15 @@
 {
     GP_REQUIRE(rows >= 0 && C > 0, "gp_l2norm_split: bad arguments (rows=%d C=%d)", rows, C);
     if (rows == 0) return GP_OK;
-    GP_REQUIRE(x && hi && lo, "gp_l2norm_split: null pointer");
+    GP_REQUIRE((x && hi && lo) || (!x && patch_mask), "gp_l2norm_split: null pointer");
     GP_REQUIRE(!patch_mask || (mask_img && mask_h > 0 && mask_w > 0 && mask_h % GP_G == 0 && mask_w % GP_G == 0),
                "gp_l2norm_split_mask: the mask image must be (rows, H, W) f32 with H, W multiples of 16 (got %d x %d)", mask_h, mask_w);
     const int ngrp = (C + 31) / 32;
+    if (!x) {
+        hipLaunchKernelGGL(patch_mask_kernel, dim3(rows), dim3(256), 0, (hipStream_t)stream, mask_img, mask_h, mask_w, patch_mask);
+        GP_CHECK_LAUNCH("gp_l2norm_split");
+        return GP_OK;
+    }
     hipLaunchKernelGGL(l2norm_split_kernel, dim3(rows, ngrp < 4 ? ngrp : 4), dim3(256), 0, (hipStream_t)stream, x, (_Float16*)hi,
                        (_Float16*)lo, C, ngrp * 32, mask_img, mask_h, mask_w, patch_mask);
     GP_CHECK_LAUNCH("gp_l2norm_split");
diff --git a/gigapose_amd/csrc/gp_vit.hip b/gigapose_amd/csrc/gp_vit.hip
--- a/gigapose_amd/csrc/gp_vit.hip
+++ b/gigapose_amd/csrc/gp_vit.hip
@@ -11,7 +11,7 @@
                             int K, int act_is_b, int epilogue, const float* bias, const float* scale, const float* res, int ldr,
                             float* scratch, hipStream_t st);
 size_t gp_gemm_streamk_bytes();
-int gp_gemm_streamk_reset_launch(float* sk_ws, hipStream_t st);
+size_t gp_gemm_streamk_header_bytes();
 bool gp_gemm_split256_usable(int I, int J, int K);
 bool gp_gemm_planes256_usable(int I, int J, int J_valid, int K);
 int gp_gemm_planes256_launch(const void* ahi, const void* alo, const void* bhi, const void* blo, float* D, int ldd, void* ohi,
@@ -23,9 +23,12 @@
 
 constexpr int PATCH = 14, IMG = 224, KPE = 588, KPE_PAD = 592, T_TOK = 257;
 
-__global__ __launch_bounds__(256) void im2col_kernel(const float* __restrict__ img, float* __restrict__ col, int B)
+__global__ __launch_bounds__(256) void im2col_kernel(const float* __restrict__ img, float* __restrict__ col, int B,
+                                                      int* __restrict__ sk_header, int sk_words)
 {
     const int k = blockIdx.x, b = blockIdx.y, p = threadIdx.x;
+    if (k == 0 && b == 0)
+        for (int w = p; w < sk_words; w += 256) sk_header[w] = 0;
     float v = 0.f;
     if (k < KPE) {
         const int ci = k / 196, dy = (k % 196) / PATCH, dx = k % PATCH;
@@ -35,22 +38,6 @@
     col[(size_t)k * (B * GP_P) + (size_t)b * GP_P + p] = v;
 }
 
-__global__ __launch_bounds__(320) void embed_kernel(const float* __restrict__ pe ,
-                                                     const float* __restrict__ cls_pos ,
-                                                     const float* __restrict__ pos_t ,
-                                                     float* __restrict__ X, int B, int Mpad)
-{
-    const int c = blockIdx.x, b = blockIdx.y, t = threadIdx.x;
-    if (b == B) {
-        for (int m = B * T_TOK + t; m < Mpad; m += 320) X[(size_t)c * Mpad + m] = 0.f;
-        return;
-    }
-    if (t >= T_TOK) return;
-    float v;
-    if (t == 0) v = cls_pos[c];
-    else v = pe[(size_t)c * (B * GP_P) + (size_t)b * GP_P + (t - 1)] + pos_t[(size_t)c * GP_P + (t - 1)];
-    X[(size_t)c * Mpad + (size_t)b * T_TOK + t] = v;
-}
 
 __global__ __launch_bounds__(1024) void layernorm_wide_kernel(const float* __restrict__ X, float* __restrict__ Y,
                                                                const float* __restrict__ gamma,
@@ -171,15 +158,32 @@
     if (amax) gp_record_amax(amax, vmax, 1.0f / plane_scale);
 }
 
-template <int NK, int TOK = 32>
+struct LnTail { int n_extra, extra_tok0, zero_row0, zero_rows; };
+
+template <int NK, int TOK = 32, bool FOLD = false>
 __global__ __launch_bounds__(512) void layernorm_planes_reg_kernel(const float* __restrict__ X, _Float16* __restrict__ Yhi,
                                                                     _Float16* __restrict__ Ylo, const float* __restrict__ gamma,
                                                                     const float* __restrict__ beta, int Mpad, float eps,
-                                                                    int* __restrict__ status, float plane_scale, float* __restrict__ amax)
+                                                                    int* __restrict__ status, float plane_scale, float* __restrict__ amax,
+                                                                    const LnTail tail)
 {
     constexpr int C = 128 * NK, SL = 512 / TOK, CH = 8 * SL, NC = C / CH;
     constexpr int TP = CH + 4;
     static_assert(C % CH == 0 && (TOK == 32 || TOK == 16), "layernorm_planes_reg_kernel: C must be a multiple of the chunk width");
+    static_assert(!FOLD || TOK == 32, "layernorm_planes_reg_kernel: extra tokens are summed as 16 slices");
+    constexpr int EV = (C + 511) / 512;
+    __shared__ __attribute__((aligned(16))) float xe[FOLD ? C : 4];
+    __shared__ float rede[2][16];
+    const bool fold = FOLD && (int)blockIdx.x < tail.n_extra;
+    const size_t etok = FOLD ? (size_t)(tail.extra_tok0 + (int)blockIdx.x) : 0;
+    float ev[EV] = {};
+    if (fold) {
+#pragma unroll
+        for (int u = 0; u < EV; ++u) {
+            const int c = threadIdx.x + 512 * u;
+            ev[u] = c < C ? X[(size_t)c * Mpad + etok] : 0.f;
+        }
+    }
     __shared__ float red[SL][TOK];
     __shared__ __attribute__((aligned(16))) unsigned int tile[2][TOK * TP];
     __shared__ __attribute__((aligned(16))) float gb[2][C];
@@ -198,12 +202,27 @@
         gb[0][c] = gamma[c];
         gb[1][c] = beta[c];
     }
+    if (fold) {
+#pragma unroll
+        for (int u = 0; u < EV; ++u)
+            if (threadIdx.x + 512 * u < C) xe[threadIdx.x + 512 * u] = ev[u];
+    }
     red[sl][tok] = s;
     __syncthreads();
     float tot = 0.f;
 #pragma unroll
     for (int j = 0; j < SL; ++j) tot += red[j][tok];
     const float mean = tot / (float)C;
+    if (fold && threadIdx.x < 16) {
+        float se = 0.f;
+#pragma unroll
+        for (int k = 0; k < NC; ++k) {
+            const f32x4 a0 = *reinterpret_cast<const f32x4*>(xe + CH * k + 8 * threadIdx.x), a1 = *reinterpret_cast<const f32x4*>(xe + CH * k + 8 * threadIdx.x + 4);
+#pragma unroll
+            for (int e = 0; e < 8; ++e) se += e < 4 ? a0[e] : a1[e - 4];
+        }
+        rede[0][threadIdx.x] = se;
+    }
     __syncthreads();
     float q = 0.f;
 #pragma unroll
@@ -214,15 +233,53 @@
             q = __builtin_fmaf(d, d, q);
         }
     red[sl][tok] = q;
+    if (fold && threadIdx.x < 16) {
+        float te = 0.f;
+#pragma unroll
+        for (int j = 0; j < 16; ++j) te += rede[0][j];
+        const float me = te / (float)C;
+        float qe = 0.f;
+#pragma unroll
+        for (int k = 0; k < NC; ++k) {
+            const f32x4 a0 = *reinterpret_cast<const f32x4*>(xe + CH * k + 8 * threadIdx.x), a1 = *reinterpret_cast<const f32x4*>(xe + CH * k + 8 * threadIdx.x + 4);
+#pragma unroll
+            for (int e = 0; e < 8; ++e) {
+                const float d = (e < 4 ? a0[e] : a1[e - 4]) - me;
+                qe = __builtin_fmaf(d, d, qe);
+            }
+        }
+        rede[1][threadIdx.x] = qe;
+    }
     __syncthreads();
     tot = 0.f;
 #pragma unroll
     for (int j = 0; j < SL; ++j) tot += red[j][tok];
     const float rstd = 1.0f / __builtin_sqrtf(tot / (float)C + eps);
+    int bad = 0;
+    float vmax = 0.f;
+    if (fold) {
+        float te = 0.f, tq = 0.f;
+#pragma unroll
+        for (int j = 0; j < 16; ++j) te += rede[0][j];
+#pragma unroll
+        for (int j = 0; j < 16; ++j) tq += rede[1][j];
+        const float me = te / (float)C, re = 1.0f / __builtin_sqrtf(tq / (float)C + eps);
+#pragma unroll
+        for (int u = 0; u < EV; ++u) {
+            const int c = threadIdx.x + 512 * u;
+            if (c < C) {
+                const float y = (ev[u] - me) * re * gb[0][c] + gb[1][c];
+                const float v = y * plane_scale;
+                const _Float16 hh = (_Float16)v;
+                bad |= !(fabsf(v) <= kSplitPlaneLimit);
+                if (amax) vmax = __builtin_elementwise_maximum(vmax, __builtin_fabsf(v));
+                Yhi[etok * C + c] = hh;
+                Ylo[etok * C + c] = (_Float16)(v - (float)hh);
+            }
+        }
+    }
     const int g2 = threadIdx.x & (SL - 1), t2 = threadIdx.x / SL;
     const size_t row = (tok0 + t2) * C + 8 * g2;
-    int bad = 0;
-    float vmax = 0.f;
 #pragma unroll
     for (int k = 0; k < NC; ++k) {
         unsigned int* T = tile[k & 1];
@@ -259,6 +316,11 @@
     }
     if (bad) gp_raise(status, GP_ST_SPLIT_RANGE);
     if (amax) gp_record_amax(amax, vmax, 1.0f / plane_scale);
+    const v16x8 z = {};
+    for (int w = blockIdx.x * 512 + threadIdx.x; w < tail.zero_rows * (C / 8); w += gridDim.x * 512) {
+        *reinterpret_cast<v16x8*>(Yhi + (size_t)tail.zero_row0 * C + (size_t)w * 8) = z;
+        *reinterpret_cast<v16x8*>(Ylo + (size_t)tail.zero_row0 * C + (size_t)w * 8) = z;
+    }
 }
 
 
@@ -266,17 +328,60 @@
 #ifdef GP_PROBES
 extern "C" void gp_vit_set_ln_reg(int on) { g_ln_planes_reg = (on >= 0 && on <= 2) ? on : 1; }
 #endif
+static int g_ln_live = -1;
+#ifdef GP_PROBES
+extern "C" void gp_vit_set_ln_live(int tokens) { g_ln_live = tokens > 0 ? tokens : -1; }
+#endif
+
+template <int NK>
+int ln_fold_slots()
+{
+    static int cache[64] = {};
+    int dev = 0, per_cu = 0, cus = 0;
+    if (hipGetDevice(&dev) != hipSuccess || dev < 0 || dev >= 64) return 0;
+    if (cache[dev] == 0) {
+        if (hipOccupancyMaxActiveBlocksPerMultiprocessor(&per_cu, layernorm_planes_reg_kernel<NK, 32, true>, 512, 0) != hipSuccess ||
+            hipDeviceGetAttribute(&cus, hipDeviceAttributeMultiprocessorCount, dev) != hipSuccess)
+            return 0;
+        cache[dev] = per_cu * cus > 0 ? per_cu * cus : -1;
+    }
+    return cache[dev] > 0 ? cache[dev] : 0;
+}
+
+constexpr int kLnFoldMaxBlocks = 4;
+
+template <int NK>
+void launch_ln_reg32(const float* X, _Float16* hi, _Float16* lo, const float* g, const float* b, int Mpad, int live, float eps, hipStream_t st,
+                     float plane_scale, float* amax)
+{
+    const int nblk = (live + 31) / 32;
+    const int slots = ln_fold_slots<NK>();
+    const int rem = slots > 0 ? nblk % slots : 0;
+    const int n_extra = live - (nblk - rem) * 32;
+    if (rem >= 1 && rem <= kLnFoldMaxBlocks && nblk > rem && n_extra <= nblk - rem) {
+        const LnTail tail{n_extra, (nblk - rem) * 32, live, Mpad - live};
+        hipLaunchKernelGGL((layernorm_planes_reg_kernel<NK, 32, true>), dim3(nblk - rem), dim3(512), 0, st, X, hi, lo, g, b, Mpad, eps, gp_status_buffer(),
+                           plane_scale, amax, tail);
+    } else {
+        const LnTail tail{0, 0, nblk * 32, Mpad - nblk * 32};
+        hipLaunchKernelGGL((layernorm_planes_reg_kernel<NK, 32, false>), dim3(nblk), dim3(512), 0, st, X, hi, lo, g, b, Mpad, eps, gp_status_buffer(),
+                           plane_scale, amax, tail);
+    }
+}
 
 int launch_layernorm_planes(const float* X, _Float16* hi, _Float16* lo, const float* g, const float* b, int C, int Mpad, float eps,
-                            hipStream_t st, float plane_scale = kPlaneScale, float* amax = nullptr)
+                            hipStream_t st, float plane_scale = kPlaneScale, float* amax = nullptr, int Mtok = -1)
 {
     GpProfScope prof(GP_PROF_LN, 8.0 * C * Mpad, st);
-    if (g_ln_planes_reg && C == 1024 && Mpad % 32 == 0 && Mpad / 32 <= 128 && g_ln_planes_reg != 2)
-        hipLaunchKernelGGL((layernorm_planes_reg_kernel<8, 16>), dim3(Mpad / 16), dim3(512), 0, st, X, hi, lo, g, b, Mpad, eps, gp_status_buffer(), plane_scale, amax);
-    else if (g_ln_planes_reg && C == 1024 && Mpad % 32 == 0)
-        hipLaunchKernelGGL(layernorm_planes_reg_kernel<8>, dim3(Mpad / 32), dim3(512), 0, st, X, hi, lo, g, b, Mpad, eps, gp_status_buffer(), plane_scale, amax);
+    const int live = (Mtok > 0 && Mtok < Mpad) ? Mtok : Mpad;
+    if (g_ln_planes_reg && C == 1024 && Mpad % 32 == 0 && Mpad / 32 <= 128 && g_ln_planes_reg != 2) {
+        const int nblk = (live + 15) / 16;
+        const LnTail tail{0, 0, nblk * 16, Mpad - nblk * 16};
+        hipLaunchKernelGGL((layernorm_planes_reg_kernel<8, 16>), dim3(nblk), dim3(512), 0, st, X, hi, lo, g, b, Mpad, eps, gp_status_buffer(), plane_scale, amax, tail);
+    } else if (g_ln_planes_reg && C == 1024 && Mpad % 32 == 0)
+        launch_ln_reg32<8>(X, hi, lo, g, b, Mpad, live, eps, st, plane_scale, amax);
     else if (g_ln_planes_reg && C == 768 && Mpad % 32 == 0)
-        hipLaunchKernelGGL(layernorm_planes_reg_kernel<6>, dim3(Mpad / 32), dim3(512), 0, st, X, hi, lo, g, b, Mpad, eps, gp_status_buffer(), plane_scale, amax);
+        launch_ln_reg32<6>(X, hi, lo, g, b, Mpad, live, eps, st, plane_scale, amax);
     else
         hipLaunchKernelGGL(layernorm_planes_kernel, dim3(Mpad / 64), dim3(1024), 0, st, X, hi, lo, g, b, C, Mpad, eps, gp_status_buffer(), plane_scale, amax);
     return 0;
@@ -735,6 +840,82 @@
     return 0;
 }
 
+constexpr float kMatchFeatScale = 32.0f;
+constexpr int FP_PT = 16;
+
+__global__ __launch_bounds__(256) void features_planes_kernel(const float* __restrict__ X, _Float16* __restrict__ hi,
+                                                               _Float16* __restrict__ lo, int C, int Mpad, int* __restrict__ status)
+{
+    extern __shared__ __attribute__((aligned(16))) float fp_lds[];
+    const int pitch = C + 4;
+    float* xs = fp_lds;
+    float* dn = fp_lds + FP_PT * pitch;
+    const int b = blockIdx.x / (GP_P / FP_PT), p0 = (blockIdx.x % (GP_P / FP_PT)) * FP_PT, t = threadIdx.x;
+    const int pl = t & (FP_PT - 1), cs = t / FP_PT;
+    const float* x = X + (size_t)cs * Mpad + (size_t)b * T_TOK + 1 + p0 + pl;
+    float* xl = xs + pl * pitch + cs;
+    for (int i = 0; i < C / 16; i += 8) {
+        float v[8];
+#pragma unroll
+        for (int u = 0; u < 8; ++u) v[u] = x[(size_t)(16 * (i + u)) * Mpad];
+#pragma unroll
+        for (int u = 0; u < 8; ++u) xl[16 * (i + u)] = v[u];
+    }
+    __syncthreads();
+    for (int pass = 0; pass < 2; ++pass) {
+        if (t < FP_PT) {
+            const f32x4* r = reinterpret_cast<const f32x4*>(xs + t * pitch);
+            float ss = 0.f;
+#pragma unroll 8
+            for (int c4 = 0; c4 < C / 4; ++c4) {
+                const f32x4 v = r[c4];
+                ss = __builtin_fmaf(v[0], v[0], ss);
+                ss = __builtin_fmaf(v[1], v[1], ss);
+                ss = __builtin_fmaf(v[2], v[2], ss);
+                ss = __builtin_fmaf(v[3], v[3], ss);
+            }
+            if (pass == 0 && !(ss <= 3.0e38f)) gp_raise(status, GP_ST_SPLIT_RANGE);
+            dn[t] = fmaxf(__builtin_sqrtf(ss), 1e-12f);
+        }
+        __syncthreads();
+        if (pass == 0) {
+            const float d = dn[pl];
+#pragma unroll 8
+            for (int i = 0; i < C / 16; ++i) xl[16 * i] = xl[16 * i] / d;
+            __syncthreads();
+        }
+    }
+    const int G = C >> 3;
+    for (int item = t; item < FP_PT * G; item += 256) {
+        const int pp = item / G, g = item - pp * G;
+        const float d = dn[pp];
+        const f32x4 a0 = *reinterpret_cast<const f32x4*>(xs + pp * pitch + 8 * g), a1 = *reinterpret_cast<const f32x4*>(xs + pp * pitch + 8 * g + 4);
+        v16x8 h, l;
+#pragma unroll
+        for (int e = 0; e < 8; ++e) {
+            const float v = ((e < 4 ? a0[e] : a1[e - 4]) / d) * kMatchFeatScale;
+            const _Float16 hh = (_Float16)v;
+            h[e] = hh;
+            l[e] = (_Float16)(v - (float)hh);
+        }
+        const size_t o = ((size_t)b * GP_P + p0 + pp) * C + 8 * g;
+        *reinterpret_cast<v16x8*>(hi + o) = h;
+        *reinterpret_cast<v16x8*>(lo + o) = l;
+    }
+}
+
+int launch_features_planes(const float* X, float* out, int B, int C, int Mpad, hipStream_t st)
+{
+    const size_t lds = sizeof(float) * ((size_t)FP_PT * (C + 4) + FP_PT);
+    GP_REQUIRE(lds <= 160 * 1024, "gp_vit_forward: dim=%d is too wide for the features-to-planes kernel", C);
+    if (lds > 48 * 1024)
+        (void)hipFuncSetAttribute(reinterpret_cast<const void*>(&features_planes_kernel), hipFuncAttributeMaxDynamicSharedMemorySize, (int)lds);
+    _Float16* hi = reinterpret_cast<_Float16*>(out);
+    hipLaunchKernelGGL(features_planes_kernel, dim3(B * (GP_P / FP_PT)), dim3(256), lds, st, X, hi, hi + (size_t)B * GP_P * C, C, Mpad,
+                       gp_status_buffer());
+    return GP_OK;
+}
+
 inline int round_up(int x, int m) { return (x + m - 1) / m * m; }
 
 }
@@ -779,7 +960,7 @@
                         void* stream)
 {
     GP_REQUIRE(X && out_hi && out_lo && gamma && beta && C > 0 && C % 128 == 0 && Mpad > 0 && Mpad % 64 == 0, "gp_layernorm_planes: bad arguments");
-    launch_layernorm_planes(X, (_Float16*)out_hi, (_Float16*)out_lo, gamma, beta, C, Mpad, eps, (hipStream_t)stream);
+    launch_layernorm_planes(X, (_Float16*)out_hi, (_Float16*)out_lo, gamma, beta, C, Mpad, eps, (hipStream_t)stream, kPlaneScale, nullptr, g_ln_live);
     GP_CHECK_LAUNCH("gp_layernorm_planes");
     return GP_OK;
 }
@@ -860,18 +1041,14 @@
     if ((size_t)KPE_PAD * B * GP_P + (size_t)dim * B * GP_P > f_floats) f_floats = (size_t)KPE_PAD * B * GP_P + (size_t)dim * B * GP_P;
     float* SK = F + f_floats;
     float* col = F;
-    float* pe = F + (size_t)KPE_PAD * BP;
     int rc;
 
-    if ((rc = gp_gemm_streamk_reset_launch(SK, st))) return rc;
-    hipLaunchKernelGGL(im2col_kernel, dim3(KPE_PAD, B), dim3(256), 0, st, images, col, B);
+    hipLaunchKernelGGL(im2col_kernel, dim3(KPE_PAD, B), dim3(256), 0, st, images, col, B, reinterpret_cast<int*>(SK),
+                       (int)(gp_gemm_streamk_header_bytes() / sizeof(int)));
     GP_CHECK_LAUNCH("gp_vit_forward/im2col");
-    if ((rc = gp_gemm_launch(weights[W_PATCH_WT], C, col, BP, pe, BP, C, BP, KPE_PAD, 1 ,
-                             weights[W_PATCH_B], nullptr, nullptr, 0, SK, st)))
+    if ((rc = gp_gemm_launch(weights[W_PATCH_WT], C, col, BP, X, Mpad, C, BP, KPE_PAD, 8 ,
+                             weights[W_PATCH_B], weights[W_POS_T], weights[W_CLS_POS], Mpad, SK, st)))
         return rc;
-    hipLaunchKernelGGL(embed_kernel, dim3(C, B + 1), dim3(320), 0, st, pe, weights[W_CLS_POS], weights[W_POS_T],
-                       X, B, Mpad);
-    GP_CHECK_LAUNCH("gp_vit_forward/embed");
 
     const int nl = (stop_after_layers >= 0 && stop_after_layers < depth) ? stop_after_layers : depth;
     const int Mtok = B * T_TOK;
@@ -892,7 +1069,7 @@
             const float os_ln1 = 1.0f / (ps[PS_LN1] * 64.0f), os_qkv = 1.0f / (ps[PS_QKV] * 64.0f), os_ln2 = 1.0f / (ps[PS_LN2] * 64.0f),
                         os_gelu = 1.0f / (ps[PS_GELU] * 64.0f);
             const GpPlaneOut po_qkv{ps[PS_QKV], am ? am + PS_QKV : nullptr}, po_gelu{ps[PS_GELU], am ? am + PS_GELU : nullptr};
-            launch_layernorm_planes(X, Hhi, Hlo, w[L_LN1_G], w[L_LN1_B], C, Mpad, ln_eps, st, ps[PS_LN1], am ? am + PS_LN1 : nullptr);
+            launch_layernorm_planes(X, Hhi, Hlo, w[L_LN1_G], w[L_LN1_B], C, Mpad, ln_eps, st, ps[PS_LN1], am ? am + PS_LN1 : nullptr, Mtok);
             GP_CHECK_LAUNCH("gp_vit_forward/layernorm_planes");
             _Float16* Ahi = reinterpret_cast<_Float16*>(QK);
             _Float16* Alo = Ahi + (size_t)3 * C * Mpad;
@@ -920,7 +1097,7 @@
             if ((rc = gp_gemm_planes256_launch(sq[S_PROJ_HI], sq[S_PROJ_LO], Hhi, Hlo, X, Mpad, nullptr, nullptr, 0, C, Mpad, Mtok, C,
                                                3 , w[L_PROJ_B], w[L_LS1], X, Mpad, os_qkv, SK, st)))
                 return rc;
-            launch_layernorm_planes(X, Hhi, Hlo, w[L_LN2_G], w[L_LN2_B], C, Mpad, ln_eps, st, ps[PS_LN2], am ? am + PS_LN2 : nullptr);
+            launch_layernorm_planes(X, Hhi, Hlo, w[L_LN2_G], w[L_LN2_B], C, Mpad, ln_eps, st, ps[PS_LN2], am ? am + PS_LN2 : nullptr, Mtok);
             GP_CHECK_LAUNCH("gp_vit_forward/layernorm_planes");
             if ((rc = gp_gemm_planes256_launch(sq[S_FC1_HI], sq[S_FC1_LO], Hhi, Hlo, nullptr, 0, Fhi, Flo, mlp_dim, mlp_dim, Mpad, Mtok, C,
                                                6 , w[L_FC1_B], nullptr, nullptr, 0, os_ln2, SK, st, nullptr, &po_gelu)))
@@ -964,7 +1141,11 @@
         else rc = gp_gemm_launch(w[L_FC2_WT], C, F, Mpad, X, Mpad, C, Mpad, mlp_dim, 3, w[L_FC2_B], w[L_LS2], X, Mpad, SK, st);
         if (rc) return rc;
     }
-    launch_features(X, out_features, B, C, Mpad, normalize, st);
+    if (normalize == 2) {
+        if ((rc = launch_features_planes(X, out_features, B, C, Mpad, st))) return rc;
+    } else {
+        launch_features(X, out_features, B, C, Mpad, normalize, st);
+    }
     GP_CHECK_LAUNCH("gp_vit_forward/features");
     return GP_OK;
 }
diff --git a/gigapose_amd/gigaPose.py b/gigapose_amd/gigaPose.py
--- a/gigapose_amd/gigaPose.py
+++ b/gigapose_amd/gigaPose.py
@@ -249,7 +249,10 @@
             side.wait_stream(main)
             with torch.cuda.stream(side):
                 tar_ist = self._backbone_rows("ist", self.ist_net.forward_by_chunk, tar_img, live_rows)
-        tar_ae = self._backbone_rows("ae", self.ae_net, tar_img, live_rows)
+        if self.template_shard is None and self.testing_metric.numerics == "split" and hasattr(self.ae_net, "forward_planes"):
+            tar_ae = self._backbone_rows("ae_planes", self.ae_net.forward_planes, tar_img, live_rows, row_dim=1)
+        else:
+            tar_ae = self._backbone_rows("ae", self.ae_net, tar_img, live_rows)
         if self.template_shard is None:
             pred = self.testing_metric.test_bank(bank, tar_ae, tar_mask, labels0)
             if side is None:
@@ -273,20 +276,24 @@
         pred.register_tensor("pred_poses", poses)
         return pred
 
-    def _backbone_rows(self, key, net, tar_img, live_rows):
+    def _backbone_rows(self, key, net, tar_img, live_rows, row_dim=0):
         B = tar_img.shape[0]
+
+        def shape_for(rows, other):
+            return other[:row_dim] + (rows,) + other[row_dim:]
+
         if live_rows is None or live_rows >= B:
             out = net(tar_img)
-            self._feat_shapes[key] = (tuple(out.shape[1:]), out.dtype)
+            self._feat_shapes[key] = (tuple(out.shape[:row_dim]) + tuple(out.shape[row_dim + 1:]), out.dtype)
             return out
         if live_rows == 0 and key in self._feat_shapes:
             shape, dtype = self._feat_shapes[key]
-            return torch.zeros((B,) + shape, dtype=dtype, device=tar_img.device)
+            return torch.zeros(shape_for(B, shape), dtype=dtype, device=tar_img.device)
         feat = net(tar_img[:max(live_rows, 1)])
-        self._feat_shapes[key] = (tuple(feat.shape[1:]), feat.dtype)
-        out = feat.new_zeros((B,) + tuple(feat.shape[1:]))
+        self._feat_shapes[key] = (tuple(feat.shape[:row_dim]) + tuple(feat.shape[row_dim + 1:]), feat.dtype)
+        out = feat.new_zeros(shape_for(B, self._feat_shapes[key][0]))
         if live_rows > 0:
-            out[:live_rows] = feat[:live_rows]
+            out.narrow(row_dim, 0, live_rows).copy_(feat.narrow(row_dim, 0, live_rows))
         return out
 
     def eval_retrieval(self, batch, idx_batch, dataset_name, sort_pred_by_inliers=True):
diff --git a/gigapose_amd/matching.py b/gigapose_amd/matching.py
--- a/gigapose_amd/matching.py
+++ b/gigapose_amd/matching.py
@@ -41,6 +41,18 @@
     _lib.call("gp_l2norm_split_mask", _lib.ptr(x), _lib.ptr(hi), _lib.ptr(lo), _lib.i(rows), _lib.i(C), _lib.ptr(mask224),
               _lib.i(mask224.shape[1]), _lib.i(mask224.shape[2]), _lib.ptr(qmask), _lib.stream_ptr())
     return hi, lo, qmask
+
+
+def patch_masks(mask224):
+    rows = mask224.shape[0]
+    fused = (mask224.is_cuda and mask224.dtype == torch.float32 and mask224.is_contiguous() and mask224.dim() == 3 and rows > 0
+             and mask224.shape[1] % 16 == 0 and mask224.shape[2] % 16 == 0)
+    if not fused:
+        return patch_grid_mask(mask224)
+    qmask = torch.empty(rows, P, dtype=torch.float32, device=mask224.device)
+    _lib.call("gp_l2norm_split_mask", _lib.ptr(None), _lib.ptr(None), _lib.ptr(None), _lib.i(rows), _lib.i(32), _lib.ptr(mask224),
+              _lib.i(mask224.shape[1]), _lib.i(mask224.shape[2]), _lib.ptr(qmask), _lib.stream_ptr())
+    return qmask
 
 
 class MatchBank:
@@ -169,7 +181,12 @@
         return ids, scores, rec_score, tar_pts, src_pts
 
     def test_bank(self, bank, tar_feat, tar_mask, labels0):
-        if self.numerics == "split":
+        if self.numerics == "split" and tar_feat.dtype == torch.float16:
+            if tar_feat.dim() != 4 or tar_feat.shape[0] != 2 or tar_feat.shape[2] != P or not tar_feat.is_contiguous():
+                raise ValueError(f"query planes must be a contiguous (2, B, 256, Cp) f16 tensor, got {tuple(tar_feat.shape)}")
+            query = (tar_feat[0], tar_feat[1])
+            qmask = patch_masks(tar_mask)
+        elif self.numerics == "split":
             hi, lo, qmask = normalize_split(tar_feat.reshape(tar_feat.shape[0], tar_feat.shape[1], P), tar_mask)
             query = (hi, lo)
         else:
diff --git a/gigapose_amd/vit.py b/gigapose_amd/vit.py
--- a/gigapose_amd/vit.py
+++ b/gigapose_amd/vit.py
@@ -276,7 +276,7 @@
         return out
 
     @torch.no_grad()
-    def patch_features(self, images, normalize=True, stop_after_layers=-1, plane_amax=None):
+    def patch_features(self, images, normalize=True, stop_after_layers=-1, plane_amax=None, matcher_planes=False):
         if images.shape[1:] != (3, 224, 224):
             raise ValueError(f"expected (B,3,224,224) crops, got {tuple(images.shape)}")
         device = images.device
@@ -286,7 +286,10 @@
             self._pack(device)
         B = images.shape[0]
         x = images.contiguous().float()
-        out = torch.empty(B, self.dim, 16, 16, dtype=torch.float32, device=device)
+        if matcher_planes:
+            out = torch.empty(2, B, 256, self.dim, dtype=torch.float16, device=device)
+        else:
+            out = torch.empty(B, self.dim, 16, 16, dtype=torch.float32, device=device)
         if B == 0:
             return out
         ws, need = self._workspace(B, device)
@@ -297,7 +300,8 @@
         _lib.call("gp_vit_forward_split2", _lib.ptr(x), _lib.i(B), _lib.i(self.dim), _lib.i(self.depth),
                   _lib.i(self.heads), _lib.i(self.mlp_dim), _lib.f(1e-6), table, _lib.i(len(tensors)),
                   split_table, _lib.i(len(split)), _lib.ptr(ws), ctypes.c_size_t(need), _lib.ptr(out),
-                  _lib.i(1 if normalize else 0), _lib.i(stop_after_layers), scales, _lib.ptr(plane_amax), _lib.stream_ptr())
+                  _lib.i(2 if matcher_planes else (1 if normalize else 0)), _lib.i(stop_after_layers), scales, _lib.ptr(plane_amax),
+                  _lib.stream_ptr())
         return out
 
     @torch.no_grad()
diff --git a/include/gigapose_hip_probe.h b/include/gigapose_hip_probe.h
--- a/include/gigapose_hip_probe.h
+++ b/include/gigapose_hip_probe.h
@@ -29,6 +29,7 @@
                              int K, float* scratch, unsigned long long* out8, void* stream);
 
 void gp_vit_set_ln_reg(int mode);
+void gp_vit_set_ln_live(int tokens);
 void gp_vit_set_planes(int on);
 int gp_vit_attention_f32(const float* qk, const float* vt, float* out, int B, int heads, int dim, int Mpad, void* stream);
 int gp_vit_layernorm_f32(const float* X, float* Y, const float* gamma, const float* beta, int C, int Mpad, float eps, void* stream);
```

Result: faster. 1590 query-crops/sec, median of 6 (+1.2%).
